# facebookresearch/NasRec

Measured on AMD Instinct MI355X. Metric: supernet samples/sec at batch 256 (Criteo-shape), 1/2/4/8 MI355X, higher is better.
Workload: dtype f32

## Files before the change

include/nasrec_hip.h:

```cpp
#ifndef NASREC_HIP_H
#define NASREC_HIP_H

#include <stdint.h>

#ifdef __cplusplus
extern "C" {
#endif

#define NASREC_MAX_SEGS 8
#define NASREC_MAX_TABLES 32
#define NASREC_EMB_DIM 16
#define NASREC_MHA_PARAMS 1696
#define NASREC_MHA_SAVED 36

enum {
  NASREC_AM_KC = 0,
  NASREC_AM_RC = 1,
  NASREC_AM_TOKR = 2,
  NASREC_AM_TOKK = 3
};
enum { NASREC_CM_PLAIN = 0,
       NASREC_CM_TOKJ = 1    };
enum { NASREC_ACT_NONE = 0, NASREC_ACT_RELU = 1, NASREC_ACT_SILU = 2, NASREC_ACT_SIGMOID = 3 };

enum {
  NASREC_OP_GEMM = 1,
  NASREC_OP_EMBED_GATHER = 2,
  NASREC_OP_DOT_TRI_FWD = 3,
  NASREC_OP_DOT_TRI_BWD = 4,
  NASREC_OP_FM_FWD = 5,
  NASREC_OP_FM_BWD = 6,
  NASREC_OP_MHA_FWD = 7,
  NASREC_OP_MHA_BWD = 8,
  NASREC_OP_REDUCE_ROWS = 9,
  NASREC_OP_COPY_SEGS = 10,
  NASREC_OP_GATE_BWD = 11,
  NASREC_OP_ROWSUM = 12,
  NASREC_OP_FINAL_FWD = 13,
  NASREC_OP_BCE = 14,
  NASREC_OP_FINAL_BWD = 15,
  NASREC_OP_EMB_DEDUP = 16,
  NASREC_OP_SUMSQ = 17,
  NASREC_OP_CLIP_COEF = 18,
  NASREC_OP_ADAGRAD_DENSE = 19,
  NASREC_OP_ADAGRAD_ROWS = 20,
  NASREC_OP_MEMSET = 21,
  NASREC_OP_LAYERNORM_FWD = 22,
  NASREC_OP_LAYERNORM_BWD = 23,
  NASREC_OP_ADD_SEGS = 24,
  NASREC_OP_SCALE = 25,
  NASREC_OP_ACT_BWD = 26,
  NASREC_OP_STAGE_INPUTS = 27,
  NASREC_OP_OPT_REDUCE = 28,
  NASREC_OP_OPT_APPLY = 29,
  NASREC_OP_WORKLIST = 30,
  NASREC_OP_CONST_I64 = 31,
  NASREC_OP_SPLITK_EPILOGUES = 32,
  NASREC_OP_DEDUP_IDS = 33,
  NASREC_OP_OPT_REDUCE2 = 34,
  NASREC_OP_FINAL_FUSED = 35,
  NASREC_OP_PERSIST = 36,
  NASREC_OP_WORKLIST_DEV = 38,
  NASREC_OP_WEIGHT_DECAY = 39,
  NASREC_OP_OPT_MOMENTS = 40,
  NASREC_OP_LAST_LAYER_STEP = 41,
  NASREC_OP_ROC_AUC = 42
};

enum { NASREC_OPTIM_ADAGRAD = 0, NASREC_OPTIM_ADAM = 1, NASREC_OPTIM_SGD = 2 };

typedef struct nasrec_gemm_seg {
  const float* A;
  const float* B;
  float* C;
  const float* Aaux;
  const float* Baux;
  float* rowsum;
  int32_t M, N, K;
  int32_t lda, ldb, ldc;
  int32_t Mvalid;
  int32_t accumulate;
  int32_t ones_col;
  int32_t _pad;
} nasrec_gemm_seg_t;

typedef struct nasrec_gemm_desc {
  int32_t kind;
  int32_t amode, bmode, cmode;
  int32_t nseg;
  int32_t zmode;
  int32_t act;
  int32_t bias_on_rows;
  int32_t mask_on_rows;
  int32_t dims_in_use;
  int32_t beta;
  int32_t splitk;
  const float* bias;
  float* save_z;
  float* save_act;
  const float* mul_ptr[NASREC_MAX_SEGS];
  int32_t mul_off[NASREC_MAX_SEGS], mul_width[NASREC_MAX_SEGS], mul_ld[NASREC_MAX_SEGS];
  int32_t mul_nseg;
  int32_t defer_second_pass;
  float* workspace;
  int32_t* counters;
  float* rowsum_out;
  const float* pre_add;
  nasrec_gemm_seg_t seg[NASREC_MAX_SEGS];
} nasrec_gemm_desc_t;

typedef struct nasrec_embed_desc {
  int32_t kind;
  int32_t B, Fs;
  int32_t _pad;
  const int64_t* idx;
  const float* table[NASREC_MAX_TABLES];
  int64_t rows[NASREC_MAX_TABLES];
  float* out;
  int32_t* oob;
} nasrec_embed_desc_t;

typedef struct nasrec_emb_dedup_desc {
  int32_t kind;
  int32_t B, Fs;
  int32_t _pad;
  const int64_t* idx;
  const float* dout;
  int32_t* leader;
  float* gsum;
  float* sumsq_partial;
  int32_t* overflow;
  int32_t rank_B;
  int32_t _pad2;
  int64_t rank_stride;
} nasrec_emb_dedup_desc_t;

typedef struct nasrec_dot_tri_desc {
  int32_t kind;
  int32_t B, k1;
  int32_t ld_out;
  const float* T;
  float* out;
  const float* dout;
  float* dT;
} nasrec_dot_tri_desc_t;

typedef struct nasrec_fm_desc {
  int32_t kind;
  int32_t B, N;
  int32_t ldx;
  int32_t ld_ix;
  int32_t accumulate;
  const float* x;
  float* ix;
  const float* dix;
  float* dx;
  const float* add;
} nasrec_fm_desc_t;

typedef struct nasrec_mha_desc {
  int32_t kind;
  int32_t B, N;
  int32_t ldx, ldo;
  int32_t dims_in_use;
  const float* x;
  float* out;
  const float* dout;
  float* dx;
  float* dparams_partial;
  const float* params[12];
  float* saved;
  int32_t partial_ld;
  int32_t bwd_form;
} nasrec_mha_desc_t;

#define NASREC_REDUCE_MAX_DST 48
typedef struct nasrec_reduce_rows_desc {
  int32_t kind;
  int32_t R, C, ld;
  const float* in;
  int32_t ndst;
  int32_t _pad;
  float* dst[NASREC_REDUCE_MAX_DST];
  int32_t dst_off[NASREC_REDUCE_MAX_DST];
  int32_t dst_len[NASREC_REDUCE_MAX_DST];
} nasrec_reduce_rows_desc_t;

typedef struct nasrec_copy_segs_desc {
  int32_t kind;
  int32_t B, nseg;
  int32_t ld_dst;
  int32_t accumulate;
  int32_t reverse;
  float* dst;
  float* seg[NASREC_MAX_SEGS];
  int32_t width[NASREC_MAX_SEGS], ld[NASREC_MAX_SEGS], off[NASREC_MAX_SEGS];
  int32_t seg_accumulate[NASREC_MAX_SEGS];
} nasrec_copy_segs_desc_t;


typedef struct nasrec_gate_bwd_desc {
  int32_t kind;
  int32_t B, D;
  int32_t ld_dout, ld_g, ld_dz;
  const float* dout;
  const float* g;
  float* dz;
  int32_t nseg;
  const float* r_ptr[NASREC_MAX_SEGS];
  float* dr_ptr[NASREC_MAX_SEGS];
  int32_t r_off[NASREC_MAX_SEGS], r_width[NASREC_MAX_SEGS], r_ld[NASREC_MAX_SEGS];
  int32_t dr_accumulate[NASREC_MAX_SEGS];
} nasrec_gate_bwd_desc_t;

typedef struct nasrec_rowsum_desc {
  int32_t kind;
  int32_t mode, R, K, ld;
  int32_t rvalid;
  const float* p;
  const float* aux;
  float* out;
} nasrec_rowsum_desc_t;

typedef struct nasrec_final_desc {
  int32_t kind;
  int32_t B, nseg;
  float grad_scale;
  const float* w;
  const float* bias;
  float* logits;
  const float* dlogits;
  float* dw;
  float* dbias;
  const float* seg[NASREC_MAX_SEGS];
  float* dseg[NASREC_MAX_SEGS];
  int32_t width[NASREC_MAX_SEGS], ld[NASREC_MAX_SEGS], off[NASREC_MAX_SEGS];
  int32_t dseg_accumulate[NASREC_MAX_SEGS];
  const float* y;
  float* loss;
  float* dlogits_out;
  int32_t nsplit;
  int32_t dseg_done;
  int32_t tok_stride[NASREC_MAX_SEGS];
} nasrec_final_desc_t;

typedef struct nasrec_bce_desc {
  int32_t kind;
  int32_t B;
  float grad_scale;
  int32_t _pad;
  const float* logits;
  const float* y;
  float* loss;
  float* dlogits;
} nasrec_bce_desc_t;

#define NASREC_SPLITK_BALANCED (-1)
#define NASREC_SK_WORKSPACE_FLOATS (512L * 3 * 128 * 128)
#define NASREC_CHUNK_ELEMS 65536
#define NASREC_CONST_I64_MAX 448

typedef struct nasrec_sumsq_desc {
  int32_t kind;
  int32_t nblocks;
  int64_t n;
  const float* x;
  float* partial;
  const int64_t* chunks;
  int64_t nchunks;
} nasrec_sumsq_desc_t;

typedef struct nasrec_clip_coef_desc {
  int32_t kind;
  int32_t n_a, n_b;
  float max_norm;
  const float* partial_a;
  const float* partial_b;
  float* out;
} nasrec_clip_coef_desc_t;

typedef struct nasrec_adagrad_dense_desc {
  int32_t kind;
  float eps;
  int64_t n;
  float* p;
  const float* g;
  float* state;
  const float* lr;
  const float* coef;
  const int64_t* chunks;
  int64_t nchunks;
} nasrec_adagrad_dense_desc_t;

typedef struct nasrec_adagrad_rows_desc {
  int32_t kind;
  int32_t B, Fs;
  float eps;
  const int64_t* idx;
  const int32_t* leader;
  const float* gsum;
  float* table[NASREC_MAX_TABLES];
  float* state[NASREC_MAX_TABLES];
  const float* lr;
  const float* coef;
  int64_t rows[NASREC_MAX_TABLES];
  int32_t rank_B;
  int32_t _pad;
  int64_t rank_stride;
} nasrec_adagrad_rows_desc_t;

typedef struct nasrec_opt_reduce_desc {
  int32_t kind;
  int32_t _pad;
  nasrec_emb_dedup_desc_t dedup;
  nasrec_sumsq_desc_t sumsq;
} nasrec_opt_reduce_desc_t;

typedef struct nasrec_opt_apply_desc {
  int32_t kind;
  int32_t dense_blocks;
  nasrec_clip_coef_desc_t clip;
  nasrec_adagrad_dense_desc_t dense;
  nasrec_adagrad_rows_desc_t rows;
} nasrec_opt_apply_desc_t;

typedef struct nasrec_weight_decay_desc {
// ... 335 lines not shown
```

nasrec_amd/_lib.py:

```python
import ctypes as C
import os

import torch

_HERE = os.path.dirname(os.path.abspath(__file__))
LIB_PATH = os.environ.get("NASREC_HIP_LIB") or os.path.join(_HERE, "lib", "libnasrec_hip.so")

MAX_SEGS = 8
MAX_TABLES = 32
EMB_DIM = 16
MHA_PARAMS = 1696
MHA_SAVED = 36
REDUCE_MAX_DST = 48

AM_KC, AM_RC, AM_TOKR, AM_TOKK = 0, 1, 2, 3
CM_PLAIN, CM_TOKJ = 0, 1
ACT_NONE, ACT_RELU, ACT_SILU, ACT_SIGMOID = 0, 1, 2, 3
TSV_OK, TSV_NEEDS_PYTHON, TSV_BAD_COLUMNS = 0, 1, 2
ACT_BY_NAME = {"identity": ACT_NONE, "relu": ACT_RELU, "silu": ACT_SILU}

(OP_GEMM, OP_EMBED_GATHER, OP_DOT_TRI_FWD, OP_DOT_TRI_BWD, OP_FM_FWD, OP_FM_BWD, OP_MHA_FWD, OP_MHA_BWD, OP_REDUCE_ROWS,
 OP_COPY_SEGS, OP_GATE_BWD, OP_ROWSUM, OP_FINAL_FWD, OP_BCE, OP_FINAL_BWD, OP_EMB_DEDUP, OP_SUMSQ, OP_CLIP_COEF,
 OP_ADAGRAD_DENSE, OP_ADAGRAD_ROWS, OP_MEMSET, OP_LAYERNORM_FWD, OP_LAYERNORM_BWD, OP_ADD_SEGS, OP_SCALE,
 OP_ACT_BWD, OP_STAGE_INPUTS, OP_OPT_REDUCE, OP_OPT_APPLY, OP_WORKLIST, OP_CONST_I64, OP_SPLITK_EPILOGUES, OP_DEDUP_IDS,
 OP_OPT_REDUCE2, OP_FINAL_FUSED, OP_PERSIST) = range(1, 37)
OP_WORKLIST_DEV = 38
OP_WEIGHT_DECAY = 39
OP_OPT_MOMENTS = 40
OP_LAST_LAYER_STEP = 41
OPTIM_ADAGRAD, OPTIM_ADAM, OPTIM_SGD = 0, 1, 2
LAST_LAYER_MAX = 8192
OP_ROC_AUC = 42
ROC_AUC_MAX_N = 1 << 30
ROC_AUC_TOO_FEW, ROC_AUC_BAD_LABEL, ROC_AUC_NOT_FINITE, ROC_AUC_ONE_CLASS = 1, 2, 4, 8

i32, i64, f32, vp = C.c_int32, C.c_int64, C.c_float, C.c_void_p


class GemmSeg(C.Structure):
    _fields_ = [("A", vp), ("B", vp), ("C", vp), ("Aaux", vp), ("Baux", vp), ("rowsum", vp), ("M", i32), ("N", i32), ("K", i32),
                ("lda", i32), ("ldb", i32), ("ldc", i32), ("Mvalid", i32), ("accumulate", i32), ("ones_col", i32), ("_pad", i32)]


class GemmDesc(C.Structure):
    _fields_ = [("kind", i32), ("amode", i32), ("bmode", i32), ("cmode", i32), ("nseg", i32), ("zmode", i32), ("act", i32),
                ("bias_on_rows", i32), ("mask_on_rows", i32), ("dims_in_use", i32), ("beta", i32), ("splitk", i32),
                ("bias", vp), ("save_z", vp), ("save_act", vp), ("mul_ptr", vp * MAX_SEGS), ("mul_off", i32 * MAX_SEGS),
                ("mul_width", i32 * MAX_SEGS), ("mul_ld", i32 * MAX_SEGS), ("mul_nseg", i32), ("defer_second_pass", i32),
                ("workspace", vp), ("counters", vp), ("rowsum_out", vp), ("pre_add", vp), ("seg", GemmSeg * MAX_SEGS)]


EPILOGUES_MAX = 3


class SplitkEpiloguesDesc(C.Structure):
    _fields_ = [("kind", i32), ("n", i32), ("g", GemmDesc * EPILOGUES_MAX)]


class EmbedDesc(C.Structure):
    _fields_ = [("kind", i32), ("B", i32), ("Fs", i32), ("_pad", i32), ("idx", vp), ("table", vp * MAX_TABLES),
                ("rows", i64 * MAX_TABLES), ("out", vp), ("oob", vp)]


class EmbDedupDesc(C.Structure):
    _fields_ = [("kind", i32), ("B", i32), ("Fs", i32), ("_pad", i32), ("idx", vp), ("dout", vp), ("leader", vp), ("gsum", vp),
                ("sumsq_partial", vp), ("overflow", vp), ("rank_B", i32), ("_pad2", i32), ("rank_stride", i64)]


class DotTriDesc(C.Structure):
    _fields_ = [("kind", i32), ("B", i32), ("k1", i32), ("ld_out", i32), ("T", vp), ("out", vp), ("dout", vp), ("dT", vp)]


class FmDesc(C.Structure):
    _fields_ = [("kind", i32), ("B", i32), ("N", i32), ("ldx", i32), ("ld_ix", i32), ("accumulate", i32), ("x", vp), ("ix", vp),
                ("dix", vp), ("dx", vp), ("add", vp)]


class MhaDesc(C.Structure):
    _fields_ = [("kind", i32), ("B", i32), ("N", i32), ("ldx", i32), ("ldo", i32), ("dims_in_use", i32), ("x", vp), ("out", vp),
                ("dout", vp), ("dx", vp), ("dparams_partial", vp), ("params", vp * 12), ("saved", vp), ("partial_ld", i32), ("bwd_form", i32)]


class ReduceRowsDesc(C.Structure):
    _fields_ = [("kind", i32), ("R", i32), ("C", i32), ("ld", i32), ("in_", vp), ("ndst", i32), ("_pad", i32), ("dst", vp * REDUCE_MAX_DST),
                ("dst_off", i32 * REDUCE_MAX_DST), ("dst_len", i32 * REDUCE_MAX_DST)]


class CopySegsDesc(C.Structure):
    _fields_ = [("kind", i32), ("B", i32), ("nseg", i32), ("ld_dst", i32), ("accumulate", i32), ("reverse", i32), ("dst", vp),
                ("seg", vp * MAX_SEGS), ("width", i32 * MAX_SEGS), ("ld", i32 * MAX_SEGS), ("off", i32 * MAX_SEGS),
                ("seg_accumulate", i32 * MAX_SEGS)]


class GateBwdDesc(C.Structure):
    _fields_ = [("kind", i32), ("B", i32), ("D", i32), ("ld_dout", i32), ("ld_g", i32), ("ld_dz", i32), ("dout", vp), ("g", vp),
                ("dz", vp), ("nseg", i32), ("r_ptr", vp * MAX_SEGS), ("dr_ptr", vp * MAX_SEGS), ("r_off", i32 * MAX_SEGS),
                ("r_width", i32 * MAX_SEGS), ("r_ld", i32 * MAX_SEGS), ("dr_accumulate", i32 * MAX_SEGS)]


class RowsumDesc(C.Structure):
    _fields_ = [("kind", i32), ("mode", i32), ("R", i32), ("K", i32), ("ld", i32), ("rvalid", i32), ("p", vp), ("aux", vp),
                ("out", vp)]


class FinalDesc(C.Structure):
    _fields_ = [("kind", i32), ("B", i32), ("nseg", i32), ("grad_scale", f32), ("w", vp), ("bias", vp), ("logits", vp), ("dlogits", vp),
                ("dw", vp), ("dbias", vp), ("seg", vp * MAX_SEGS), ("dseg", vp * MAX_SEGS), ("width", i32 * MAX_SEGS),
                ("ld", i32 * MAX_SEGS), ("off", i32 * MAX_SEGS), ("dseg_accumulate", i32 * MAX_SEGS), ("y", vp), ("loss", vp),
                ("dlogits_out", vp), ("nsplit", i32), ("dseg_done", i32), ("tok_stride", i32 * MAX_SEGS)]


class BceDesc(C.Structure):
    _fields_ = [("kind", i32), ("B", i32), ("grad_scale", f32), ("_pad", i32), ("logits", vp), ("y", vp), ("loss", vp),
                ("dlogits", vp)]


class SumsqDesc(C.Structure):
    _fields_ = [("kind", i32), ("nblocks", i32), ("n", i64), ("x", vp), ("partial", vp), ("chunks", vp), ("nchunks", i64)]


class ClipCoefDesc(C.Structure):
    _fields_ = [("kind", i32), ("n_a", i32), ("n_b", i32), ("max_norm", f32), ("partial_a", vp), ("partial_b", vp), ("out", vp)]


class AdagradDenseDesc(C.Structure):
    _fields_ = [("kind", i32), ("eps", f32), ("n", i64), ("p", vp), ("g", vp), ("state", vp), ("lr", vp), ("coef", vp),
                ("chunks", vp), ("nchunks", i64)]


class AdagradRowsDesc(C.Structure):
    _fields_ = [("kind", i32), ("B", i32), ("Fs", i32), ("eps", f32), ("idx", vp), ("leader", vp), ("gsum", vp),
                ("table", vp * MAX_TABLES), ("state", vp * MAX_TABLES), ("lr", vp), ("coef", vp), ("rows", i64 * MAX_TABLES),
                ("rank_B", i32), ("_pad", i32), ("rank_stride", i64)]


class MemsetDesc(C.Structure):
    _fields_ = [("kind", i32), ("_pad", i32), ("bytes", i64), ("ptr", vp), ("chunks", vp), ("nchunks", i64)]


SPLITK_BALANCED = -1
SK_WORKSPACE_FLOATS = 512 * 3 * 128 * 128
CHUNK_ELEMS = 65536
CONST_I64_MAX = 448


class ConstI64Desc(C.Structure):
    _fields_ = [("kind", i32), ("n", i32), ("dst", vp), ("vals", i64 * CONST_I64_MAX)]


class LayerNormDesc(C.Structure):
    _fields_ = [("kind", i32), ("mode", i32), ("R", i32), ("D", i32), ("ldx", i32), ("ldy", i32), ("act", i32),
                ("dims_in_use", i32), ("accumulate", i32), ("eps", f32), ("x", vp), ("w", vp), ("b", vp), ("y", vp), ("stats", vp),
                ("dy", vp), ("dx", vp), ("dwb_partial", vp), ("nblk", i32), ("_pad", i32)]


class ScaleDesc(C.Structure):
    _fields_ = [("kind", i32), ("_pad", i32), ("n", i64), ("s", f32), ("_pad2", i32), ("x", vp), ("y", vp)]


class ActBwdDesc(C.Structure):
    _fields_ = [("kind", i32), ("mode", i32), ("R", i32), ("D", i32), ("ld_dy", i32), ("ld_z", i32), ("ld_dz", i32), ("act", i32),
                ("dims_in_use", i32), ("dy", vp), ("z", vp), ("dz", vp)]


DEDUP_IDS_MAX_B = 2048


class DedupIdsDesc(C.Structure):
    _fields_ = [("kind", i32), ("B", i32), ("Fs", i32), ("cap", i32), ("idx", vp), ("leader", vp), ("order", vp), ("lists", vp), ("counts", vp),
                ("heads", vp)]


class OptReduce2Desc(C.Structure):
    _fields_ = [("kind", i32), ("B", i32), ("Fs", i32), ("cap", i32), ("rank_B", i32), ("row_blocks", i32), ("rank_stride", i64), ("rows", vp),
                ("leader", vp), ("order", vp), ("lists", vp), ("counts", vp), ("heads", vp), ("sumsq_partial", vp), ("sumsq", SumsqDesc)]


class StageDesc(C.Structure):
    _fields_ = [("kind", i32), ("B", i32), ("Fd", i32), ("Fs", i32), ("lr", f32), ("_pad", i32), ("int_src", vp), ("int_dst", vp),
                ("cat_src", vp), ("cat_dst", vp), ("y_src", vp), ("y_dst", vp), ("lr_dst", vp), ("gather", EmbedDesc), ("dedup_ids", DedupIdsDesc)]


class OptReduceDesc(C.Structure):
    _fields_ = [("kind", i32), ("_pad", i32), ("dedup", EmbDedupDesc), ("sumsq", SumsqDesc)]


class OptApplyDesc(C.Structure):
    _fields_ = [("kind", i32), ("dense_blocks", i32), ("clip", ClipCoefDesc), ("dense", AdagradDenseDesc), ("rows", AdagradRowsDesc)]


WL_MAX_ITEMS, WL_BLOB_BYTES, WL_REDUCE_DST = 12, 3680, 16
WL_WHOLE, WL_MAIN, WL_EPI = 0, 1, 2
# ... 146 lines not shown
```

nasrec_amd/csrc/common.h:

```cpp
#pragma once
#include <hip/hip_runtime.h>
#include <stdint.h>
#include "nasrec_hip.h"

#define NASREC_WAVE 64

typedef float f32x4 __attribute__((ext_vector_type(4)));

template <int MODE>
__device__ __forceinline__ long operand_offset(int r, int k, int ld) {
  if (MODE == NASREC_AM_KC) return (long)r * ld + k;
  if (MODE == NASREC_AM_RC) return (long)k * ld + r;
  if (MODE == NASREC_AM_TOKR) return (long)(r >> 4) * ld + (r & 15) + (long)k * 16;
  return (long)(k >> 4) * ld + (k & 15) + (long)r * 16;
}

template <int CMODE>
__device__ __forceinline__ long c_offset(int i, int j, int ldc) {
  if (CMODE == NASREC_CM_PLAIN) return (long)i * ldc + j;
  return (long)(j >> 4) * ldc + (j & 15) + (long)i * 16;
}

__device__ __forceinline__ float act_apply(float z, int act) {
  switch (act) {
    case NASREC_ACT_RELU: return z > 0.f ? z : 0.f;
    case NASREC_ACT_SILU: return z / (1.f + __expf(-z));
    case NASREC_ACT_SIGMOID: return 1.f / (1.f + __expf(-z));
    default: return z;
  }
}

template <int BYTES>
__device__ __forceinline__ void warm_kernarg() {
  static_assert(BYTES % 64 == 0 && BYTES >= 64 && BYTES <= 4096, "whole 64-byte lines");
  if (threadIdx.x >= 64) return;
  const unsigned long long p = (unsigned long long)__builtin_amdgcn_kernarg_segment_ptr();
  int sink;
  if (BYTES <= 1024) {
    asm volatile(
        ".set nasrec_wk_off, 0\n"
        ".rept %c2\n"
        "s_load_dword %0, %1, nasrec_wk_off\n"
        ".set nasrec_wk_off, nasrec_wk_off + 64\n"
        ".endr\n"
        "s_waitcnt lgkmcnt(0)"
        : "=&s"(sink)
        : "s"(p), "n"(BYTES / 64)
        : "memory");
  } else {
    asm volatile(
        ".set nasrec_wk_off, 0\n"
        ".rept %c2\n"
        ".rept 16\n"
        "s_load_dword %0, %1, nasrec_wk_off\n"
        ".set nasrec_wk_off, nasrec_wk_off + 64\n"
        ".endr\n"
        "s_waitcnt lgkmcnt(0)\n"
        ".endr"
        : "=&s"(sink)
        : "s"(p), "n"(BYTES / 1024)
        : "memory");
  }
}

template <int CTRL>
__device__ __forceinline__ float dpp_mov(float v) {
  return __builtin_bit_cast(float, __builtin_amdgcn_mov_dpp(__builtin_bit_cast(int, v), CTRL, 0xf, 0xf, false));
}
__device__ __forceinline__ float wave_sum(float v) {
  v += dpp_mov<0xb1>(v);
  v += dpp_mov<0x4e>(v);
  v += dpp_mov<0x124>(v);
  v += dpp_mov<0x128>(v);
  v += dpp_mov<0x142>(v);
  v += dpp_mov<0x143>(v);
  return __builtin_bit_cast(float, __builtin_amdgcn_readlane(__builtin_bit_cast(int, v), 63));
}

int nasrec_set_error(int code, const char* fmt, ...);
int nasrec_check_launch(const char* what);

static inline bool nasrec_lds_attr_needed(unsigned long long& mask) {
  int dev = 0;
  (void)hipGetDevice(&dev);
  const unsigned long long bit = 1ull << (dev & 63);
  if (mask & bit) return false;
  mask |= bit;
  return true;
}

int launch_gemm(hipStream_t s, const nasrec_gemm_desc_t* d);
int launch_embed_gather(hipStream_t s, const nasrec_embed_desc_t* d);
int launch_emb_dedup(hipStream_t s, const nasrec_emb_dedup_desc_t* d);
int launch_dot_tri(hipStream_t s, const nasrec_dot_tri_desc_t* d);
int launch_fm(hipStream_t s, const nasrec_fm_desc_t* d);
int launch_mha(hipStream_t s, const nasrec_mha_desc_t* d);
int launch_reduce_rows(hipStream_t s, const nasrec_reduce_rows_desc_t* d);
int launch_copy_segs(hipStream_t s, const nasrec_copy_segs_desc_t* d);
int launch_gate_bwd(hipStream_t s, const nasrec_gate_bwd_desc_t* d);
int launch_rowsum(hipStream_t s, const nasrec_rowsum_desc_t* d);
int launch_final(hipStream_t s, const nasrec_final_desc_t* d);
int final_fused_check(const nasrec_final_desc_t* d);
int launch_bce(hipStream_t s, const nasrec_bce_desc_t* d);
int launch_sumsq(hipStream_t s, const nasrec_sumsq_desc_t* d);
int launch_clip_coef(hipStream_t s, const nasrec_clip_coef_desc_t* d);
int launch_adagrad_dense(hipStream_t s, const nasrec_adagrad_dense_desc_t* d);
int launch_adagrad_rows(hipStream_t s, const nasrec_adagrad_rows_desc_t* d);
int launch_layernorm(hipStream_t s, const nasrec_layernorm_desc_t* d);
int launch_scale(hipStream_t s, const nasrec_scale_desc_t* d);
int launch_act_bwd(hipStream_t s, const nasrec_act_bwd_desc_t* d);
int launch_stage(hipStream_t s, const nasrec_stage_desc_t* d);
int launch_opt_reduce(hipStream_t s, const nasrec_opt_reduce_desc_t* d);
int launch_opt_apply(hipStream_t s, const nasrec_opt_apply_desc_t* d);
int launch_memset_chunks(hipStream_t s, const nasrec_memset_desc_t* d);
int launch_memset_flat(hipStream_t s, const nasrec_memset_desc_t* d);
int launch_const_i64(hipStream_t s, const nasrec_const_i64_desc_t* d);
int launch_splitk_epilogues(hipStream_t s, const nasrec_splitk_epilogues_desc_t* d);
int launch_worklist(hipStream_t s, const nasrec_worklist_desc_t* d);
int launch_worklist_dev(hipStream_t s, const nasrec_worklist_dev_desc_t* d);
int launch_dedup_ids(hipStream_t s, const nasrec_dedup_ids_desc_t* d);
int launch_opt_reduce2(hipStream_t s, const nasrec_opt_reduce2_desc_t* d);
int launch_persist(hipStream_t s, const nasrec_persist_desc_t* d);
int launch_weight_decay(hipStream_t s, const nasrec_weight_decay_desc_t* d);
int launch_opt_moments(hipStream_t s, const nasrec_opt_moments_desc_t* d);
int launch_last_layer_step(hipStream_t s, const nasrec_last_layer_step_desc_t* d);
int launch_roc_auc(hipStream_t s, const nasrec_roc_auc_desc_t* d);
```

nasrec_amd/csrc/final_bodies.h:

```cpp
#pragma once
#include "common.h"

__device__ __forceinline__ int final_wcol(const nasrec_final_desc_t& d, int q, int j) {
  const int ts = d.tok_stride[q];
  return d.off[q] + (ts ? (j >> 4) * ts + (j & 15) : j);
}
__device__ __forceinline__ int final_feat(const nasrec_final_desc_t& d, int q, int k) {
  const int r = k - d.off[q], ts = d.tok_stride[q];
  if (r < 0) return -1;
  if (!ts) return r < d.width[q] ? r : -1;
  const int t = r / ts, e = r - t * ts;
  const int j = t * 16 + e;
  return (e < 16 && j < d.width[q]) ? j : -1;
}
__host__ __device__ inline int final_seg_extent(const nasrec_final_desc_t& d, int q) {
  const int ts = d.tok_stride[q], W = d.width[q];
  return (ts && W > 0) ? ((W - 1) >> 4) * ts + ((W - 1) & 15) + 1 : W;
}

__device__ __forceinline__ float final_logit(const nasrec_final_desc_t& d, int b, float* red) {
  const int wave = threadIdx.x >> 6, lane = threadIdx.x & 63;
  float s = 0.f;
  for (int q = 0; q < d.nseg; ++q) {
    if (!d.seg[q]) continue;
    const float* x = d.seg[q] + (long)b * d.ld[q];
    const float* w = d.w + d.off[q];
    const int W = d.width[q], ts = d.tok_stride[q];
    for (int j0 = lane + 64 * wave; j0 < W; j0 += 256 * 4) {
      float xv[4], wv[4];
#pragma unroll
      for (int u = 0; u < 4; ++u) {
        const int j = min(j0 + 256 * u, W - 1);
        xv[u] = x[j];
        wv[u] = w[ts ? (j >> 4) * ts + (j & 15) : j];
      }
#pragma unroll
      for (int u = 0; u < 4; ++u)
        if (j0 + 256 * u < W) s = fmaf(xv[u], wv[u], s);
    }
  }
  s = wave_sum(s);
  __syncthreads();
  if (lane == 0) red[wave] = s;
  __syncthreads();
  return ((red[0] + red[1]) + (red[2] + red[3])) + d.bias[0];
}

__device__ __forceinline__ void final_fwd_block(const nasrec_final_desc_t& d, int vb, float* red) {
  if (vb >= d.B) return;
  const float z = final_logit(d, vb, red);
  if (threadIdx.x == 0) d.logits[vb] = z;
}

__device__ __forceinline__ float bce_grad(float z, float y, float scale) { return (1.f / (1.f + expf(-z)) - y) * scale; }
__device__ __forceinline__ float bce_term(float z, float y) { return fmaxf(z, 0.f) - z * y + log1pf(expf(-fabsf(z))); }

__device__ __forceinline__ void final_fused_block(const nasrec_final_desc_t& d, int vb, float* red) {
  const int b = vb;
  if (b >= d.B) return;
  const float yb = d.y[b];
  const float z = final_logit(d, b, red);
  if (threadIdx.x == 0) d.logits[b] = z;
  const float g = bce_grad(z, yb, d.grad_scale);
  const int tid = threadIdx.x;
  for (int q = 0; q < d.nseg; ++q) {
    float* p = d.dseg[q];
    if (!p || !d.seg[q]) continue;
    p += (long)b * d.ld[q];
    const float* w = d.w + d.off[q];
    const int W = d.width[q], ts = d.tok_stride[q];
    const bool acc = d.dseg_accumulate[q] != 0;
    for (int j0 = tid; j0 < W; j0 += 256 * 4) {
      float wv[4], cv[4];
#pragma unroll
      for (int u = 0; u < 4; ++u) {
        const int j = min(j0 + 256 * u, W - 1);
        wv[u] = w[ts ? (j >> 4) * ts + (j & 15) : j];
        cv[u] = acc ? p[j] : 0.f;
      }
#pragma unroll
      for (int u = 0; u < 4; ++u) {
        const float v = g * wv[u];
        if (j0 + 256 * u < W) p[j0 + 256 * u] = acc ? cv[u] + v : v;
      }
    }
  }
}

#define FINAL_BWD_LDS_FLOATS 272
#define FINAL_BWD_ROWS 16
__host__ __device__ inline int final_bwd_rows(int B) { return B >= 1024 ? FINAL_BWD_ROWS : 1; }
__device__ __forceinline__ void final_bwd_block(const nasrec_final_desc_t& d, int K, int nA, int nB, int vb_, float* lds) {
  const int nC = d.y != nullptr ? 1 : 0;
  const int vb = vb_ < nB + nC ? nA + vb_ : vb_ - (nB + nC);
  const bool fused = d.y != nullptr;
  const float* const dl_a = fused ? d.logits : d.dlogits;
  const float* const dl_b = fused ? d.y : d.dlogits;
  const float dl_scale = d.grad_scale;
  auto dl = [&](int b) {
    const float z = dl_a[b], y = dl_b[b];
    return fused ? bce_grad(z, y, dl_scale) : z;
  };
  if (vb < nA && final_bwd_rows(d.B) > 1) {
    constexpr int RB = FINAL_BWD_ROWS;
    const int kblocks = (K + 255) / 256;
    const int rblk = vb / kblocks, k = (vb - rblk * kblocks) * 256 + (int)threadIdx.x;
    if (k >= K) return;
    float* p0 = nullptr;
    long ldq = 0;
    bool accq = false;
    for (int q = 0; q < d.nseg; ++q) {
      const int jj = final_feat(d, q, k);
      if (jj >= 0) {
        if (d.dseg[q]) {
          p0 = d.dseg[q] + jj;
          ldq = d.ld[q];
          accq = d.dseg_accumulate[q] != 0;
        }
        break;
      }
    }
    if (!p0) return;
    const float wk = d.w[k];
    const int r0 = rblk * RB;
    float z[RB], y[RB], c[RB], g[RB];
#pragma unroll
    for (int u = 0; u < RB; ++u) {
      const int b = min(r0 + u, d.B - 1);
      z[u] = dl_a[b];
      y[u] = dl_b[b];
      c[u] = 0.f;
    }
    if (accq) {
#pragma unroll
      for (int u = 0; u < RB; ++u) c[u] = p0[(long)min(r0 + u, d.B - 1) * ldq];
    }
    if (fused) {
#pragma unroll
      for (int u = 0; u < RB; ++u) g[u] = bce_grad(z[u], y[u], dl_scale);
    } else {
#pragma unroll
      for (int u = 0; u < RB; ++u) g[u] = z[u];
    }
    __builtin_amdgcn_s_waitcnt(0x0F70);
#pragma unroll
    for (int u = 0; u < RB; ++u) {
      if (r0 + u >= d.B) break;
      const float v = g[u] * wk;
      p0[(long)(r0 + u) * ldq] = accq ? c[u] + v : v;
    }
    return;
  }
  if (vb < nA) {
    const long t = (long)vb * 256 + threadIdx.x;
    if (t >= (long)d.B * K) return;
    const int b = (int)(t / K), k = (int)(t % K);
    for (int q = 0; q < d.nseg; ++q) {
      const int jj = final_feat(d, q, k);
      if (jj >= 0) {
        if (d.dseg[q]) {
          float* p = d.dseg[q] + (long)b * d.ld[q] + jj;
          const float v = dl(b) * d.w[k];
          *p = d.dseg_accumulate[q] ? *p + v : v;
        }
        break;
      }
    }
    return;
  }
  if (vb >= nA + nB) {
    float* redl = lds;
    float s = 0.f;
    for (int b = threadIdx.x; b < d.B; b += 256) {
      const float z = d.logits[b], y = d.y[b];
      s += bce_term(z, y);
      if (d.dlogits_out) d.dlogits_out[b] = bce_grad(z, y, d.grad_scale);
    }
    redl[threadIdx.x] = s;
    __syncthreads();
    for (int o = 128; o > 0; o >>= 1) {
      if ((int)threadIdx.x < o) redl[threadIdx.x] += redl[threadIdx.x + o];
      __syncthreads();
    }
    if (threadIdx.x == 0 && d.loss) d.loss[0] = redl[0] / (float)d.B;
    return;
  }
  if (d.nsplit > 1) {
    float(*reds)[64] = reinterpret_cast<float(*)[64]>(lds);
    const int nBk = nB / d.nsplit;
    const int blk = vb - nA, slice = blk / nBk, kl = threadIdx.x & 63, w = threadIdx.x >> 6;
    const int k = (blk - slice * nBk) * 64 + kl;
    const int b0 = (int)((long)d.B * slice / d.nsplit), b1 = (int)((long)d.B * (slice + 1) / d.nsplit);
    float s0 = 0.f, s1 = 0.f;
    if (k <= K) {
      const float* src = nullptr;
      int ld = 0, jj = 0;
      if (k < K) {
        for (int q = 0; q < d.nseg; ++q) {
          jj = final_feat(d, q, k);
          if (jj >= 0) {
            src = d.seg[q];
            ld = d.ld[q];
            break;
          }
        }
      }
      const bool has = k < K && src != nullptr;
      const float* sp = has ? src + jj : d.w;
      const long sld = has ? ld : 0;
      int b = b0 + w;
      for (; b + 28 < b1; b += 32) {
        float f[8], z[8], y[8], g[8];
#pragma unroll
        for (int u = 0; u < 8; ++u) {
          f[u] = sp[(long)(b + 4 * u) * sld];
          z[u] = dl_a[b + 4 * u];
          y[u] = dl_b[b + 4 * u];
        }
        if (fused) {
#pragma unroll
          for (int u = 0; u < 8; ++u) g[u] = bce_grad(z[u], y[u], dl_scale);
        } else {
#pragma unroll
          for (int u = 0; u < 8; ++u) g[u] = z[u];
        }
#pragma unroll
        for (int u = 0; u < 8; u += 2) {
          s0 = fmaf(g[u], (k == K) ? 1.f : (has ? f[u] : 0.f), s0);
          s1 = fmaf(g[u + 1], (k == K) ? 1.f : (has ? f[u + 1] : 0.f), s1);
        }
      }
      for (; b + 4 < b1; b += 8) {
        const float f0 = (k == K) ? 1.f : (src ? src[(long)b * ld + jj] : 0.f);
        const float f1 = (k == K) ? 1.f : (src ? src[(long)(b + 4) * ld + jj] : 0.f);
        s0 = fmaf(dl(b), f0, s0);
        s1 = fmaf(dl(b + 4), f1, s1);
      }
      for (; b < b1; b += 4) s0 = fmaf(dl(b), (k == K) ? 1.f : (src ? src[(long)b * ld + jj] : 0.f), s0);
    }
    reds[w][kl] = s0 + s1;
    __syncthreads();
    if (w == 0 && k <= K) d.dw[(long)slice * (K + 1) + k] = (reds[0][kl] + reds[1][kl]) + (reds[2][kl] + reds[3][kl]);
    return;
  }
  float(*red)[17] = reinterpret_cast<float(*)[17]>(lds);
  const int kl = threadIdx.x & 15, bq = threadIdx.x >> 4;
// ... 65 lines not shown
```

nasrec_amd/csrc/gemm_fast.hip:

```cpp
#include <stdlib.h>
#include "gemm_tile.h"

typedef float f32x16 __attribute__((ext_vector_type(16)));
typedef int i32x4 __attribute__((ext_vector_type(4)));

#define FT_BM 128
#define FT_BN 128
#define FT_BK 32
#define FT_KC_LD 36
#define FT_TILE_FLOATS (FT_BM * FT_KC_LD)
#define FT_FENCE() __builtin_amdgcn_sched_barrier(0)

template <int MODE>
__device__ __forceinline__ void ft_slot(int tid, int it, int& row, int& k) {
  const int idx = tid + 256 * it;
  if (MODE == NASREC_AM_KC) {
    row = idx >> 3;
    k = (idx & 7) << 2;
  } else {
    k = idx >> 5;
    row = (idx & 31) << 2;
  }
}

// ... 544 lines not shown
  const int fr = lane & 31, fg = lane >> 5;
  const int t = blockIdx.x;
  const long W = (long)sk_tiles * sk_T, lo = (long)t * sk_T, hi = lo + sk_T;
  int w = (int)(lo * FT_SK_WGS / W);
  while (w > 0 && ft_share_begin(W, w) > lo) --w;
  while (ft_share_begin(W, w + 1) <= lo) ++w;
  if (ft_share_begin(W, w) <= lo && ft_share_begin(W, w + 1) >= hi) return;
  int z, ks, by, bx;
  if (!ft_decode(d, t, 1, tiles_m, tiles_n, z, ks, by, bx)) return;
  const nasrec_gemm_seg_t& s0 = d.seg[z];
  const int m0 = by * FT_BM, n0 = bx * FT_BN;
  if (m0 >= s0.M || n0 >= s0.N) return;
  f32x16 acc[2][2];
#pragma unroll
  for (int a = 0; a < 2; ++a)
#pragma unroll
    for (int b = 0; b < 2; ++b)
#pragma unroll
      for (int r = 0; r < 16; ++r) acc[a][b][r] = 0.f;
  for (; w < FT_SK_WGS && ft_share_begin(W, w) < hi; ++w) {
    const int piece = t - (int)(ft_share_begin(W, w) / sk_T);
    const float* slot = d.workspace + ((long)w * FT_SK_PIECES + piece) * FT_PIECE_FLOATS;
#pragma unroll
    for (int a = 0; a < 2; ++a)
#pragma unroll
      for (int b = 0; b < 2; ++b)
#pragma unroll
        for (int r = 0; r < 16; ++r) acc[a][b][r] += slot[((a * 2 + b) * 16 + r) * 256 + tid];
  }
  ft_epilogue(d, s0, m0, n0, wm, wn, fr, fg, acc, false);
}

template <int AM, int BMODE>
static int launch_fast_t(hipStream_t st, const nasrec_gemm_desc_t* d, int Mmax, int Nmax, int zdim, bool ones) {
  const int tm = (Mmax + FT_BM - 1) / FT_BM, tn = (Nmax + FT_BN - 1) / FT_BN;
  long blocks = (long)tm * tn * zdim;
  if (d->zmode) {
    const int S = d->splitk > 1 ? d->splitk : 1;
    blocks = 0;
    for (int q = 0; q < d->nseg; ++q)
      blocks += (long)((d->seg[q].M + FT_BM - 1) / FT_BM) * ((d->seg[q].N + FT_BN - 1) / FT_BN) * S;
  }
  int sk_tiles = 0, sk_T = 0;
  if (d->splitk == NASREC_SPLITK_BALANCED) {
    int T = 0;
    if (d->zmode) {
      for (int q = 0; q < d->nseg; ++q) {
        const int tq = d->seg[q].A ? (d->seg[q].K + FT_BK - 1) / FT_BK : 0;
        if (q > 0 && tq != T) return nasrec_set_error(-2, "gemm: balanced schedule needs equal K over the batch (problem %d)", q);
        T = tq;
      }
    } else {
      for (int q = 0; q < d->nseg; ++q)
        if (d->seg[q].A) T += (d->seg[q].K + FT_BK - 1) / FT_BK;
    }
    if (T < 1) return nasrec_set_error(-2, "gemm: balanced schedule on an empty product");
    if (!d->workspace) return nasrec_set_error(-3, "gemm: balanced schedule needs a workspace of NASREC_SK_WORKSPACE_FLOATS floats");
    const long tiles = blocks;
    if (tiles % FT_SK_WGS != 0) {
      sk_tiles = (int)(tiles >= FT_SK_WGS ? FT_SK_WGS + tiles % FT_SK_WGS : tiles);
      sk_T = T;
      blocks = FT_SK_WGS + (tiles - sk_tiles);
    }
  }
  const dim3 grid((unsigned)blocks);
  if (ones)
    hipLaunchKernelGGL((gemm_fast_kernel<AM, BMODE, true>), grid, dim3(256), 0, st, *d, Mmax, Nmax, tm, tn, sk_tiles, sk_T);
  else
    hipLaunchKernelGGL((gemm_fast_kernel<AM, BMODE, false>), grid, dim3(256), 0, st, *d, Mmax, Nmax, tm, tn, sk_tiles, sk_T);
  if (sk_tiles > 0) hipLaunchKernelGGL(gemm_fast_fixup_kernel, dim3((unsigned)sk_tiles), dim3(256), 0, st, *d, tm, tn, sk_tiles, sk_T);
  return 0;
}

bool gemm_fast_eligible(const nasrec_gemm_desc_t* d, int Mmax, int Nmax) {
  if (d->cmode != NASREC_CM_PLAIN) return false;
  if (d->bias && d->bias_on_rows) return false;
  if ((d->amode != NASREC_AM_KC && d->amode != NASREC_AM_RC) || (d->bmode != NASREC_AM_KC && d->bmode != NASREC_AM_RC)) return false;
  if (d->amode == NASREC_AM_RC && d->bmode == NASREC_AM_KC) return false;
  const int nprob = d->zmode ? d->nseg : 1;
  const int S = d->splitk > 1 ? d->splitk : 1;
  long tiles = 0, kmax = 0;
  for (int q = 0; q < d->nseg; ++q) {
    const nasrec_gemm_seg_t& s = d->seg[q];
    if (s.Aaux || s.Baux) return false;
    if (s.A && s.K > kmax) kmax = s.K;
    const long r = s.M > s.N ? s.M : s.N, ld = s.lda > s.ldb ? s.lda : s.ldb;
    if (s.A && (r * ld + s.K >= (1L << 29) || (long)s.K * ld + r >= (1L << 29))) return false;
  }
  long useful = 0, padded = 0;
  for (int q = 0; q < nprob; ++q) {
    const nasrec_gemm_seg_t& s = d->seg[q];
    const long t = (long)((s.M + FT_BM - 1) / FT_BM) * ((s.N + FT_BN - 1) / FT_BN);
    tiles += t * S;
    useful += (long)s.M * s.N;
    padded += t * FT_BM * FT_BN;
  }
  (void)Mmax;
  (void)Nmax;
  if (2 * useful < padded) return false;
  static const long min_k = getenv("NASREC_FAST_MIN_K") ? atol(getenv("NASREC_FAST_MIN_K")) : 1;
  return tiles >= NASREC_GEMM_FAST_MIN_TILES && kmax >= min_k;
}

int launch_gemm_fast(hipStream_t st, const nasrec_gemm_desc_t* d, int Mmax, int Nmax, int zdim) {
  bool ones = false;
  for (int q = 0; q < d->nseg; ++q) ones = ones || d->seg[q].ones_col != 0;
  if (d->amode == NASREC_AM_KC && d->bmode == NASREC_AM_KC) return launch_fast_t<NASREC_AM_KC, NASREC_AM_KC>(st, d, Mmax, Nmax, zdim, ones);
  if (d->amode == NASREC_AM_KC && d->bmode == NASREC_AM_RC) return launch_fast_t<NASREC_AM_KC, NASREC_AM_RC>(st, d, Mmax, Nmax, zdim, ones);
  return launch_fast_t<NASREC_AM_RC, NASREC_AM_RC>(st, d, Mmax, Nmax, zdim, ones);
}
```

nasrec_amd/csrc/gemm_kslice.hip:

```cpp
#include <cstdlib>
#include <cstring>
#include "gemm_tile.h"

#define KS_TM 32
#define KS_TN 32
#define KS_DC 128
#define KS_NB 4
#define KS_CH ((KS_TM + KS_TN) * KS_DC)
#define KS_SEGS 4
#ifdef KS_STAMPS
#define KS_STAMP(i) \
  if (tid == 0 && d.workspace) d.workspace[blockIdx.x * 64 + (i)] = __builtin_bit_cast(float, (unsigned)__builtin_readcyclecounter())
#define KS_LOOP_STAMP_A const unsigned ks_ta = (unsigned)__builtin_readcyclecounter()
#define KS_LOOP_STAMP_B ks_wait += (unsigned)__builtin_readcyclecounter() - ks_ta
#else
#define KS_STAMP(i)
#define KS_LOOP_STAMP_A
#define KS_LOOP_STAMP_B
#endif

__device__ __forceinline__ __amdgpu_buffer_rsrc_t ks_rsrc(const float* p, long floats) {
  return __builtin_amdgcn_make_buffer_rsrc(const_cast<float*>(p), 0, (int)(floats <= 0 ? 0 : (floats > 0x1fffffffL ? 0x7fffffffL : 4 * floats)), 0x00020000);
}

// ... 221 lines not shown
      if (ck >= cK) {
        do {
          ++cseg;
        } while (cseg < KS_SEGS && seg_k(cseg) == 0);
        ck = 0;
        cK = seg_k(cseg);
      }
    };
    auto multiply = [&](int set) {
      const int lim = flim[set];
      if (lim < KS_DC) {
#pragma unroll
        for (int kb = 0; kb < 4; ++kb)
#pragma unroll
          for (int e = 0; e < 4; ++e) {
            const bool in = 4 * (16 * half + 4 * kb + fg) + e < lim;
            fa[set][kb][e] = in ? fa[set][kb][e] : 0.f;
            fb[set][kb][e] = in ? fb[set][kb][e] : 0.f;
          }
      }
#pragma unroll
      for (int kb = 0; kb < 4; kb += 2)
#pragma unroll
        for (int j = 0; j < 4; ++j) {
          acc0 = __builtin_amdgcn_mfma_f32_16x16x4f32(fa[set][kb][j], fb[set][kb][j], acc0, 0, 0, 0);
          acc1 = __builtin_amdgcn_mfma_f32_16x16x4f32(fa[set][kb + 1][j], fb[set][kb + 1][j], acc1, 0, 0, 0);
        }
    };
    for (int t = 0; t < nchunks + 1; t += 2) {
#pragma unroll
      for (int h = 0; h < 2; ++h) {
        const int c = t + h;
        if (c < nchunks) {
          asm volatile("s_waitcnt lgkmcnt(0)" ::: "memory");
          KS_LOOP_STAMP_A;
          __builtin_amdgcn_s_barrier();
          KS_LOOP_STAMP_B;
          readfrag(h);
        }
        if (c >= 1 && c <= nchunks) multiply(h ^ 1);
      }
    }
    KS_STAMP(4);
    asm volatile("s_waitcnt lgkmcnt(0)" ::: "memory");
    __builtin_amdgcn_s_barrier();
    if (tK > 0) {
#pragma unroll
      for (int e = 0; e < 4; ++e) {
        const bool in = 4 * fg + e < tK;
        ta[e] = in ? ta[e] : 0.f;
        tb[e] = in ? tb[e] : 0.f;
      }
#pragma unroll
      for (int j = 0; j < 4; ++j) acc0 = __builtin_amdgcn_mfma_f32_16x16x4f32(ta[j], tb[j], acc0, 0, 0, 0);
    }
    const f32x4 acc = acc0 + acc1;
#ifdef KS_STAMPS
    if (lane == 0 && d.workspace) {
      d.workspace[blockIdx.x * 64 + 16 + wave * 3 + 1] = __builtin_bit_cast(float, ks_wait);
      d.workspace[blockIdx.x * 64 + 16 + wave * 3 + 2] = __builtin_bit_cast(float, (unsigned)__builtin_readcyclecounter() - ks_t0);
    }
#endif
    *reinterpret_cast<f32x4*>(&red[((half * 4 + tile) * 64 + lane) * 4]) = acc;
  }
  __syncthreads();
  KS_STAMP(5);
  {
    const int e = wave;
    const int etile = e >> 2, r = e & 3;
    const float v = red[((0 * 4 + etile) * 64 + lane) * 4 + r] + red[((1 * 4 + etile) * 64 + lane) * 4 + r];
    const int i = m0 + (etile >> 1) * 16 + 4 * fg + r, j = n0 + (etile & 1) * 16 + fr;
    if (i < M && j < N) epilogue_store<NASREC_CM_PLAIN>(d, s0, i, j, v);
  }
  KS_STAMP(6);
}

bool gemm_kslice_eligible(const nasrec_gemm_desc_t* d) {
  if (d->amode != NASREC_AM_KC || d->bmode != NASREC_AM_KC || d->cmode != NASREC_CM_PLAIN || d->zmode || d->splitk > 1) return false;
  if (d->nseg > KS_SEGS) return false;
  const nasrec_gemm_seg_t& s0 = d->seg[0];
  long K = 0;
  for (int q = 0; q < d->nseg; ++q) {
    const nasrec_gemm_seg_t& s = d->seg[q];
    if (s.Aaux || s.Baux || s.ones_col || (s.Mvalid > 0 && s.Mvalid < s0.M)) return false;
    if (s.A && s.K > 0) {
      K += s.K;
      if ((long)s0.M * s.lda >= (1L << 29) || (long)s0.N * s.ldb >= (1L << 29)) return false;
    }
  }
  const long tiles = (long)((s0.M + KS_TM - 1) / KS_TM) * ((s0.N + KS_TN - 1) / KS_TN);
  return s0.M <= 512 && tiles >= 128 && tiles <= 512 && K >= 512;
}

int launch_gemm_kslice(hipStream_t st, const nasrec_gemm_desc_t* d) {
  const nasrec_gemm_seg_t& s0 = d->seg[0];
  const int tiles_m = (s0.M + KS_TM - 1) / KS_TM, tiles_n = (s0.N + KS_TN - 1) / KS_TN;
  static unsigned long long attr_devices = 0;
  const size_t lds = sizeof(float) * KS_NB * KS_CH;
  if (nasrec_lds_attr_needed(attr_devices))
    (void)hipFuncSetAttribute(reinterpret_cast<const void*>(&gemm_kslice_kernel), hipFuncAttributeMaxDynamicSharedMemorySize, (int)lds);
  hipLaunchKernelGGL(gemm_kslice_kernel, dim3((unsigned)(tiles_m * tiles_n)), dim3(1024), lds, st, *d, tiles_m, tiles_n);
  return nasrec_check_launch("gemm_kslice");
}
```

nasrec_amd/csrc/gemm_skinny.hip:

```cpp
#include <stdlib.h>

#include "gemm_tile.h"

#define SKN_STEPS 8

template <int NW, bool BRC>
__global__ __launch_bounds__(64 * NW) void gemm_skinny_n_kernel(const nasrec_gemm_desc_t d) {
  __shared__ float red[NW][256];
  const int lane = threadIdx.x & 63, wave = __builtin_amdgcn_readfirstlane(threadIdx.x >> 6);
  const int r = lane & 15, g = lane >> 4;
  const nasrec_gemm_seg_t& s0 = d.seg[0];
  const int M = s0.M, N = s0.N;
  const int m0 = (int)blockIdx.x * 16;
  const int row = min(m0 + r, M - 1), col = min(r, N - 1);
  const int nsegk = d.zmode ? 1 : d.nseg;
  int T = 0;
  for (int q = 0; q < nsegk; ++q) T += (d.seg[q].A && d.seg[q].K > 0) ? (d.seg[q].K + 15) >> 4 : 0;
  const int t0 = (int)((long)T * wave / NW), t1 = (int)((long)T * (wave + 1) / NW);
  int fq = 0, fk = 0;
  {
    int skip = t0;
    for (; fq < nsegk; ++fq) {
      const int nt = (d.seg[fq].A && d.seg[fq].K > 0) ? (d.seg[fq].K + 15) >> 4 : 0;
      if (skip < nt) break;
      skip -= nt;
    }
    fk = 16 * skip;
  }
  f32x4 acc = {0.f, 0.f, 0.f, 0.f};
  for (int t = t0; t < t1; t += SKN_STEPS) {
    f32x4 fa[SKN_STEPS], fb[SKN_STEPS];
    int lim[SKN_STEPS];
#pragma unroll
    for (int s = 0; s < SKN_STEPS; ++s) {
      const bool in = t + s < t1 && fq < nsegk;
      const nasrec_gemm_seg_t& sg = d.seg[in ? fq : 0];
      const bool live = in && sg.A != nullptr && sg.K > 0;
      const int K = live ? sg.K : 0, kk = fk + 4 * g;
      lim[s] = K - fk;
      const __amdgpu_buffer_rsrc_t ra = __builtin_amdgcn_make_buffer_rsrc(
          const_cast<float*>(sg.A), 0, live ? (int)min(4L * ((long)(M - 1) * sg.lda + K), 0x7fffffffL) : 0, 0x00020000);
      const __amdgpu_buffer_rsrc_t rb = __builtin_amdgcn_make_buffer_rsrc(
          const_cast<float*>(sg.B), 0, live ? (int)(4 * (BRC ? (long)(K - 1) * sg.ldb + N : (long)(N - 1) * sg.ldb + K)) : 0, 0x00020000);
      fa[s] = __builtin_bit_cast(f32x4, __builtin_amdgcn_raw_buffer_load_b128(ra, (int)(4 * ((long)row * sg.lda + kk)), 0, 0));
      if (BRC) {
#pragma unroll
        for (int j = 0; j < 4; ++j)
          fb[s][j] = __builtin_bit_cast(float, __builtin_amdgcn_raw_buffer_load_b32(rb, 4 * ((kk + j) * sg.ldb + col), 0, 0));
      } else {
        fb[s] = __builtin_bit_cast(f32x4, __builtin_amdgcn_raw_buffer_load_b128(rb, 4 * (col * sg.ldb + kk), 0, 0));
      }
      fk += 16;
      bool next = in && fk >= K;
      if (next) {
        ++fq;
        while (fq < nsegk && !(d.seg[fq].A && d.seg[fq].K > 0)) ++fq;
        fk = 0;
      }
    }
#pragma unroll
    for (int s = 0; s < SKN_STEPS; ++s) {
      const int l = lim[s];
      if (l > 0) {
        f32x4 a = fa[s], b = fb[s];
        if (l < 16) {
#pragma unroll
          for (int j = 0; j < 4; ++j) {
            const bool ok = 4 * g + j < l;
            a[j] = ok ? a[j] : 0.f;
            b[j] = ok ? b[j] : 0.f;
          }
        }
#pragma unroll
        for (int j = 0; j < 4; ++j) acc = __builtin_amdgcn_mfma_f32_16x16x4f32(a[j], b[j], acc, 0, 0, 0);
      }
    }
  }
#pragma unroll
  for (int q = 0; q < 4; ++q) red[wave][q * 64 + lane] = acc[q];
  __syncthreads();
  if (wave == 0) {
    float v4[4];
#pragma unroll
    for (int q = 0; q < 4; ++q) {
      float p[NW];
#pragma unroll
      for (int w = 0; w < NW; ++w) p[w] = red[w][q * 64 + lane];
#pragma unroll
      for (int span = 1; span < NW; span *= 2)
#pragma unroll
        for (int w = 0; w + span < NW; w += 2 * span) p[w] += p[w + span];
      v4[q] = p[0];
    }
    if (m0 + 4 * g < M && r < N) epilogue_store_col4<NASREC_CM_PLAIN>(d, s0, m0 + 4 * g, r, M, v4);
  }
}

bool gemm_skinny_n_eligible(const nasrec_gemm_desc_t* d) {
  if (d->amode != NASREC_AM_KC || (d->bmode != NASREC_AM_KC && d->bmode != NASREC_AM_RC) || d->cmode != NASREC_CM_PLAIN || d->splitk > 1) return false;
  if (d->zmode && d->nseg != 1) return false;
  const nasrec_gemm_seg_t& s0 = d->seg[0];
  if (s0.N < 1 || s0.N > 16 || s0.M < 1024) return false;
  long K = 0;
  for (int q = 0; q < d->nseg; ++q) {
    const nasrec_gemm_seg_t& s = d->seg[q];
    if (s.Aaux || s.Baux || s.ones_col || (s.Mvalid > 0 && s.Mvalid < s0.M)) return false;
    if (s.A && s.K > 0) {
      K += s.K;
      if ((long)s0.M * s.lda >= (1L << 29) || (long)(d->bmode == NASREC_AM_RC ? s.K : s0.N) * s.ldb >= (1L << 29)) return false;
    }
  }
  return K >= 256;
}

int launch_gemm_skinny_n(hipStream_t st, const nasrec_gemm_desc_t* d) {
  const int M = d->seg[0].M;
  const int tiles = (M + 15) / 16;
  const bool brc = d->bmode == NASREC_AM_RC;
  if (tiles >= 512) {
    if (brc) hipLaunchKernelGGL((gemm_skinny_n_kernel<4, true>), dim3((unsigned)tiles), dim3(256), 0, st, *d);
    else hipLaunchKernelGGL((gemm_skinny_n_kernel<4, false>), dim3((unsigned)tiles), dim3(256), 0, st, *d);
  } else {
    if (brc) hipLaunchKernelGGL((gemm_skinny_n_kernel<8, true>), dim3((unsigned)tiles), dim3(512), 0, st, *d);
    else hipLaunchKernelGGL((gemm_skinny_n_kernel<8, false>), dim3((unsigned)tiles), dim3(512), 0, st, *d);
  }
  return nasrec_check_launch("gemm_skinny_n");
}

#define TK_MAXK 16
#define TK_GROUPS 2
#define TK_ROWS (8 * TK_GROUPS)
template <bool BRC>
__global__ __launch_bounds__(256) void gemm_tinyk_kernel(const nasrec_gemm_desc_t d) {
  const int q = d.zmode ? (int)blockIdx.z : 0;
  const nasrec_gemm_seg_t& sg = d.seg[q];
  const int M = sg.M, N = sg.N, K = sg.K;
  const int j = (int)blockIdx.x * 256 + (int)threadIdx.x;
  const int i0 = (int)blockIdx.y * TK_ROWS;
  if (i0 >= M) return;
  const int jc = min(j, N - 1);
  float w[TK_MAXK];
  if (sg.A != nullptr && K > 0) {
#pragma unroll
    for (int k = 0; k < TK_MAXK; ++k) w[k] = k < K ? (BRC ? sg.B[(long)k * sg.ldb + jc] : sg.B[(long)jc * sg.ldb + k]) : 0.f;
  } else {
#pragma unroll
    for (int k = 0; k < TK_MAXK; ++k) w[k] = 0.f;
  }
  const bool simple = !d.pre_add && d.mul_nseg == 0 && !(d.zmode ? sg.accumulate : d.beta) && d.dims_in_use < 0 && !(d.bias && d.bias_on_rows);
  const float bj = (simple && d.bias) ? d.bias[jc] : 0.f;
  float* const zp = d.save_z;
  float* const ap = d.save_act;
  const int act = d.act;
  const int lane = (int)threadIdx.x & 63;
  float xa[TK_GROUPS], xb[TK_GROUPS];
#pragma unroll
  for (int gr = 0; gr < TK_GROUPS; ++gr) {
    xa[gr] = xb[gr] = 0.f;
    if (sg.A != nullptr && K > 0) {
      const int ri = min(i0 + 8 * gr + (lane >> 3), M - 1), kc = 2 * (lane & 7);
      const float* xr = sg.A + (long)ri * sg.lda;
      if (kc < K) xa[gr] = xr[kc];
      if (kc + 1 < K) xb[gr] = xr[kc + 1];
    }
  }
#pragma unroll
  for (int gr = 0; gr < TK_GROUPS; ++gr) {
    const int ib = i0 + 8 * gr;
    if (ib >= M) break;
    const float x0 = xa[gr], x1 = xb[gr];
    float acc[8];
#pragma unroll
    for (int r = 0; r < 8; ++r) {
      float s = 0.f;
#pragma unroll
      for (int k = 0; k < TK_MAXK; ++k) {
        const float xv = __builtin_bit_cast(float, __builtin_amdgcn_readlane(__builtin_bit_cast(int, (k & 1) ? x1 : x0), r * 8 + (k >> 1)));
        s = fmaf(xv, w[k], s);
      }
      acc[r] = s;
    }
    if (j < N) {
      if (simple) {
#pragma unroll
        for (int r = 0; r < 8; ++r) {
          if (ib + r < M) {
            const long o = (long)(ib + r) * sg.ldc + j;
            float v = acc[r] + bj;
            if (zp) zp[o] = v;
            v = act_apply(v, act);
            if (ap) ap[o] = v;
            sg.C[o] = v;
          }
        }
      } else {
        const float va[4] = {acc[0], acc[1], acc[2], acc[3]}, vb[4] = {acc[4], acc[5], acc[6], acc[7]};
        epilogue_store_col4<NASREC_CM_PLAIN>(d, sg, ib, j, M, va);
        if (ib + 4 < M) epilogue_store_col4<NASREC_CM_PLAIN>(d, sg, ib + 4, j, M, vb);
      }
    }
  }
}

bool gemm_tinyk_eligible(const nasrec_gemm_desc_t* d) {
  static const bool on = getenv("NASREC_TINYK") == nullptr || atoi(getenv("NASREC_TINYK")) != 0;
  if (!on || d->amode != NASREC_AM_KC || (d->bmode != NASREC_AM_KC && d->bmode != NASREC_AM_RC) || d->cmode != NASREC_CM_PLAIN || d->splitk > 1) return false;
  static const bool rc_too = getenv("NASREC_TINYK") != nullptr && atoi(getenv("NASREC_TINYK")) == 2;
  if (d->bmode == NASREC_AM_RC && !rc_too) return false;
  if (!d->zmode && d->nseg != 1) return false;
  for (int q = 0; q < d->nseg; ++q) {
    const nasrec_gemm_seg_t& s = d->seg[q];
    if (s.Aaux || s.Baux || s.ones_col || (s.Mvalid > 0 && s.Mvalid < s.M)) return false;
    if (s.M < 1024 || s.N < 256 || s.K < 0 || s.K > TK_MAXK) return false;
  }
  return true;
}

int launch_gemm_tinyk(hipStream_t st, const nasrec_gemm_desc_t* d) {
  int Mmax = 0, Nmax = 0;
  const int nprob = d->zmode ? d->nseg : 1;
  for (int q = 0; q < nprob; ++q) {
    Mmax = max(Mmax, d->seg[q].M);
    Nmax = max(Nmax, d->seg[q].N);
  }
  const dim3 grid((unsigned)((Nmax + 255) / 256), (unsigned)((Mmax + TK_ROWS - 1) / TK_ROWS), (unsigned)nprob);
  if (d->bmode == NASREC_AM_RC) hipLaunchKernelGGL((gemm_tinyk_kernel<true>), grid, dim3(256), 0, st, *d);
  else hipLaunchKernelGGL((gemm_tinyk_kernel<false>), grid, dim3(256), 0, st, *d);
  return nasrec_check_launch("gemm_tinyk");
}
```

nasrec_amd/csrc/norm_loss_opt.hip:

```cpp
#include "common.h"
#include "optimizer_bodies.h"

#include "final_bodies.h"

__global__ __launch_bounds__(256) void final_fwd_kernel(const nasrec_final_desc_t d) {
  __shared__ float red[4];
  final_fwd_block(d, blockIdx.x, red);
}

__global__ __launch_bounds__(256) void final_bwd_kernel(const nasrec_final_desc_t d, int K, int nA, int nB) {
  __shared__ float lds[FINAL_BWD_LDS_FLOATS];
  final_bwd_block(d, K, nA, nB, blockIdx.x, lds);
}

__global__ __launch_bounds__(256) void final_fused_kernel(const nasrec_final_desc_t d) {
  __shared__ float red[4];
  final_fused_block(d, blockIdx.x, red);
}

int final_fused_check(const nasrec_final_desc_t* d) {
  if (!d->y || !d->logits || !d->bias || !d->w) return nasrec_set_error(-2, "final_fused: needs y, logits, bias and w");
  if (d->nsplit > 1) return nasrec_set_error(-2, "final_fused: nsplit=%d (the batch-sliced backward keeps its own launch)", d->nsplit);
  for (int q = 0; q < d->nseg; ++q)
    if (d->dseg[q] && !d->seg[q]) return nasrec_set_error(-2, "final_fused: segment %d has a gradient destination and no input", q);
  return 0;
}

int launch_final(hipStream_t st, const nasrec_final_desc_t* d) {
  if (d->B == 0) return 0;
  if (d->kind == NASREC_OP_FINAL_FUSED) {
    const int rc = final_fused_check(d);
    if (rc) return rc;
    hipLaunchKernelGGL(final_fused_kernel, dim3(d->B), dim3(256), 0, st, *d);
  } else if (d->kind == NASREC_OP_FINAL_FWD) {
    hipLaunchKernelGGL(final_fwd_kernel, dim3(d->B), dim3(256), 0, st, *d);
  } else {
    int K, nA, nB;
    final_bwd_geometry(*d, K, nA, nB);
    if (d->y != nullptr && d->logits == nullptr) return nasrec_set_error(-2, "final_bwd: fused BCE needs desc.logits");
    hipLaunchKernelGGL(final_bwd_kernel, dim3(nA + nB + (d->y != nullptr ? 1 : 0)), dim3(256), 0, st, *d, K, nA, nB);
  }
  return nasrec_check_launch("final");
}

__global__ __launch_bounds__(1024) void bce_kernel(const nasrec_bce_desc_t d) {
  __shared__ float red[1024];
  float s = 0.f;
  for (int b = threadIdx.x; b < d.B; b += 1024) {
    const float z = d.logits[b], y = d.y[b];
    s += bce_term(z, y);
    d.dlogits[b] = bce_grad(z, y, d.grad_scale);
  }
  red[threadIdx.x] = s;
  __syncthreads();
  for (int o = 512; o > 0; o >>= 1) {
    if ((int)threadIdx.x < o) red[threadIdx.x] += red[threadIdx.x + o];
    __syncthreads();
  }
  if (threadIdx.x == 0) d.loss[0] = red[0] / (float)d.B;
}

int launch_bce(hipStream_t st, const nasrec_bce_desc_t* d) {
  if (d->B == 0) return 0;
  hipLaunchKernelGGL(bce_kernel, dim3(1), dim3(1024), 0, st, *d);
  return nasrec_check_launch("bce");
}

__global__ __launch_bounds__(256) void sumsq_kernel(const nasrec_sumsq_desc_t d) {
  __shared__ float red[256];
  sumsq_body(d, blockIdx.x, gridDim.x, red);
}

int launch_sumsq(hipStream_t st, const nasrec_sumsq_desc_t* d) {
  if (d->nblocks < 1) return nasrec_set_error(-2, "sumsq: nblocks=%d", d->nblocks);
  hipLaunchKernelGGL(sumsq_kernel, dim3(d->nblocks), dim3(256), 0, st, *d);
  return nasrec_check_launch("sumsq");
}

__global__ __launch_bounds__(64) void clip_coef_kernel(const nasrec_clip_coef_desc_t d) {
  float total;
  const float coef = clip_coef_wave(d, threadIdx.x, &total);
  if (threadIdx.x == 0) {
    d.out[0] = coef;
    d.out[1] = total;
  }
}

int launch_clip_coef(hipStream_t st, const nasrec_clip_coef_desc_t* d) {
  hipLaunchKernelGGL(clip_coef_kernel, dim3(1), dim3(64), 0, st, *d);
  return nasrec_check_launch("clip_coef");
}

__global__ __launch_bounds__(256) void adagrad_dense_kernel(const nasrec_adagrad_dense_desc_t d) {
  adagrad_dense_body(d, blockIdx.x, gridDim.x, *d.lr, *d.coef);
}

int launch_adagrad_dense(hipStream_t st, const nasrec_adagrad_dense_desc_t* d) {
  if (d->n == 0 || (d->chunks && d->nchunks < 1)) return 0;
  const long blocks = d->chunks ? (d->nchunks > 2048 ? 2048 : d->nchunks) : adagrad_dense_blocks(d->n);
  hipLaunchKernelGGL(adagrad_dense_kernel, dim3((unsigned)blocks), dim3(256), 0, st, *d);
  return nasrec_check_launch("adagrad_dense");
}

__global__ __launch_bounds__(256) void memset_chunks_kernel(const nasrec_memset_desc_t d) {
  for (long c = blockIdx.x; c < d.nchunks; c += gridDim.x) {
    float* x = reinterpret_cast<float*>(d.ptr) + d.chunks[2 * c];
    const long n = d.chunks[2 * c + 1], n4 = n >> 2;
    for (long i = threadIdx.x; i < n4; i += 256) *reinterpret_cast<f32x4*>(x + 4 * i) = (f32x4){0.f, 0.f, 0.f, 0.f};
    for (long j = 4 * n4 + threadIdx.x; j < n; j += 256) x[j] = 0.f;
  }
}

// ... 626 lines not shown
```

nasrec_amd/csrc/token_linear.hip:

```cpp
#include "gemm_tile.h"

#define TL_WAVES 16
#define TL_CHUNK 8
#define TL_MAX_LDS 147456
#define TL_BIAS_FLOATS 80

template <int RB>
struct TlPad {
  static constexpr int v = RB == 1 ? 16 : (RB <= 3 ? 48 : 80);
};

template <int AM, int RB>
__global__ __launch_bounds__(1024) void token_linear_kernel(const nasrec_gemm_desc_t d, int wgs) {
  extern __shared__ __attribute__((aligned(16))) float lds_all[];
  float* const Bl = lds_all;
  float* const Wl = lds_all + TL_BIAS_FLOATS;
  constexpr int MP = TlPad<RB>::v;
  const int tid = threadIdx.x, lane = tid & 63, wave = __builtin_amdgcn_readfirstlane(tid >> 6);
  const int z = d.zmode ? (int)blockIdx.x / wgs : 0;
  const int wg = (int)blockIdx.x - z * wgs;
  const int s_lo = d.zmode ? z : 0, s_hi = d.zmode ? z + 1 : d.nseg;
  const nasrec_gemm_seg_t& s0 = d.seg[s_lo];
  const int M = s0.M, Bs = s0.N >> 4;

// ... 19 lines not shown
    kbase += Kp;
  }
  if (tid < TL_BIAS_FLOATS) Bl[tid] = (d.bias && d.bias_on_rows && tid < M) ? d.bias[tid] : 0.f;
  __syncthreads();

  const int g = lane >> 4, e = lane & 15;
  const bool acc_c = d.zmode ? s0.accumulate != 0 : d.beta != 0;
  const bool has_bias = d.bias != nullptr, bias_rows = d.bias_on_rows != 0, mask_rows = d.mask_on_rows != 0;
  const int dims = d.dims_in_use, act = d.act;
  float* const zbase = d.save_z;
  for (int b = wg * TL_WAVES + wave; b < Bs; b += wgs * TL_WAVES) {
    f32x4 acc[RB];
#pragma unroll
    for (int rb = 0; rb < RB; ++rb) acc[rb] = (f32x4){0.f, 0.f, 0.f, 0.f};
    int kb = 0;
    for (int s = s_lo; s < s_hi; ++s) {
      const nasrec_gemm_seg_t& sg = d.seg[s];
      if (!sg.A || sg.K <= 0) continue;
      const int K4 = (sg.K + 3) >> 2;
      const __amdgpu_buffer_rsrc_t rs =
          __builtin_amdgcn_make_buffer_rsrc(const_cast<float*>(sg.B) + (long)b * sg.ldb, 0, sg.K * 64, 0x00020000);
      for (int c0 = 0; c0 < K4; c0 += TL_CHUNK) {
        float xv[TL_CHUNK];
#pragma unroll
        for (int u = 0; u < TL_CHUNK; ++u)
          xv[u] = __builtin_bit_cast(float, __builtin_amdgcn_raw_buffer_load_b32(rs, (c0 + u) * 256 + lane * 4, 0, 0));
#pragma unroll
        for (int u = 0; u < TL_CHUNK; ++u) {
          if (c0 + u < K4) {
            const float* wrow = Wl + (kb + 4 * (c0 + u) + g) * MP + e;
#pragma unroll
            for (int rb = 0; rb < RB; ++rb) acc[rb] = __builtin_amdgcn_mfma_f32_16x16x4f32(wrow[rb * 16], xv[u], acc[rb], 0, 0, 0);
          }
        }
      }
      kb += 4 * K4;
    }
    float* C = s0.C + (long)b * s0.ldc + e;
    float* Z = zbase ? zbase + (long)b * s0.ldc + e : nullptr;
    float cv[RB][4];
#pragma unroll
    for (int rb = 0; rb < RB; ++rb)
#pragma unroll
      for (int r = 0; r < 4; ++r) cv[rb][r] = 0.f;
    if (acc_c) {
#pragma unroll
      for (int rb = 0; rb < RB; ++rb)
#pragma unroll
        for (int r = 0; r < 4; ++r) cv[rb][r] = C[min(rb * 16 + 4 * g + r, M - 1) * 16];
    }
    const float bcol = (has_bias && !bias_rows) ? d.bias[b * 16 + e] : 0.f;
    __builtin_amdgcn_s_waitcnt(0x0F70);
    const bool dead_col = dims >= 0 && !mask_rows && b * 16 + e >= dims;
#pragma unroll
    for (int rb = 0; rb < RB; ++rb)
#pragma unroll
      for (int r = 0; r < 4; ++r) {
        const int i = rb * 16 + 4 * g + r;
        if (i >= M) continue;
        float v = acc[rb][r];
        if (has_bias) v += bias_rows ? Bl[i] : bcol;
        if (Z) Z[i * 16] = v;
        v = act_apply(v, act);
        if (dead_col || (dims >= 0 && mask_rows && i >= dims)) v = 0.f;
        if (acc_c) v += cv[rb][r];
        C[i * 16] = v;
      }
  }
}

bool token_linear_eligible(const nasrec_gemm_desc_t* d) {
  if (d->cmode != NASREC_CM_TOKJ || d->bmode != NASREC_AM_TOKR) return false;
  if (d->amode != NASREC_AM_KC && d->amode != NASREC_AM_RC) return false;
  if (d->splitk > 1 || d->pre_add || d->save_act || d->mul_nseg > 0) return false;
  const int nprob = d->zmode ? d->nseg : 1;
  for (int p = 0; p < nprob; ++p) {
    const nasrec_gemm_seg_t& s0 = d->seg[p];
    if (s0.M < 1 || s0.M > 80 || (s0.N & 15) || (s0.N >> 4) < 1024 || s0.ones_col) return false;
    if (s0.Mvalid > 0 && s0.Mvalid < s0.M) return false;
    const int mp = s0.M <= 16 ? 16 : (s0.M <= 48 ? 48 : 80);
    long kp = 0;
    for (int q = d->zmode ? p : 0; q < (d->zmode ? p + 1 : d->nseg); ++q) {
      const nasrec_gemm_seg_t& s = d->seg[q];
      if (s.Aaux || s.Baux) return false;
      if (!d->zmode && (s.M != s0.M || s.N != s0.N)) return false;
      if (s.A && s.K > 0) kp += (s.K + 3) & ~3;
      if ((long)s.K * 64 > 0x7fffffffL) return false;
    }
    if (kp * mp * 4 + TL_BIAS_FLOATS * 4 > TL_MAX_LDS) return false;
    if (d->zmode && p > 0 && (s0.N != d->seg[0].N || (s0.M + 15) / 16 != (d->seg[0].M + 15) / 16)) return false;
  }
  return true;
}

template <int AM, int RB>
static void launch_token_linear_rb(hipStream_t st, const nasrec_gemm_desc_t* d, int grid, int wgs, size_t lds) {
  static unsigned long long big_lds_devices = 0;
  if (lds > 65536 && nasrec_lds_attr_needed(big_lds_devices))
    (void)hipFuncSetAttribute(reinterpret_cast<const void*>(&token_linear_kernel<AM, RB>), hipFuncAttributeMaxDynamicSharedMemorySize, TL_MAX_LDS);
  hipLaunchKernelGGL((token_linear_kernel<AM, RB>), dim3(grid), dim3(1024), lds, st, *d, wgs);
}

template <int AM>
static void launch_token_linear_t(hipStream_t st, const nasrec_gemm_desc_t* d, int rb, int grid, int wgs, size_t lds) {
  switch (rb) {
    case 1: launch_token_linear_rb<AM, 1>(st, d, grid, wgs, lds); break;
    case 2: launch_token_linear_rb<AM, 2>(st, d, grid, wgs, lds); break;
    case 3: launch_token_linear_rb<AM, 3>(st, d, grid, wgs, lds); break;
    case 4: launch_token_linear_rb<AM, 4>(st, d, grid, wgs, lds); break;
    default: launch_token_linear_rb<AM, 5>(st, d, grid, wgs, lds); break;
  }
}

int launch_token_linear(hipStream_t st, const nasrec_gemm_desc_t* d) {
  const int nprob = d->zmode ? d->nseg : 1;
  const int Bs = d->seg[0].N >> 4;
  const int rb = (d->seg[0].M + 15) / 16;
  const int mp = rb == 1 ? 16 : (rb <= 3 ? 48 : 80);
  long kp_max = 0;
  for (int p = 0; p < nprob; ++p) {
    long kp = 0;
    for (int q = d->zmode ? p : 0; q < (d->zmode ? p + 1 : d->nseg); ++q)
      if (d->seg[q].A && d->seg[q].K > 0) kp += (d->seg[q].K + 3) & ~3;
    if (kp > kp_max) kp_max = kp;
  }
  int wgs = 256 / nprob;
  if (wgs < 64) wgs = 64;
  const int need = (Bs + TL_WAVES - 1) / TL_WAVES;
  if (wgs > need) wgs = need;
  const size_t lds = (size_t)(kp_max > 0 ? kp_max : 4) * mp * 4 + TL_BIAS_FLOATS * 4;
  if (d->amode == NASREC_AM_KC)
    launch_token_linear_t<NASREC_AM_KC>(st, d, rb, wgs * nprob, wgs, lds);
  else
    launch_token_linear_t<NASREC_AM_RC>(st, d, rb, wgs * nprob, wgs, lds);
  return nasrec_check_launch("token_linear");
}

#define TDW_WAVES 16

template <int RB, int CB>
__global__ __launch_bounds__(64 * TDW_WAVES) void token_dw_kernel(const nasrec_gemm_desc_t d, int Mmax, int Nmax) {
  __shared__ __attribute__((aligned(16))) float red[4 * RB * CB * 4 * 64];
  const int tid = threadIdx.x, lane = tid & 63, wave = __builtin_amdgcn_readfirstlane(tid >> 6);
  const int S = d.splitk;
  const int z = (int)blockIdx.x / S, ks = (int)blockIdx.x - z * S;
  const nasrec_gemm_seg_t& sg = d.seg[z];
  const int M = sg.M, N = sg.N, Nr = sg.ones_col ? N - 1 : N;
  const int Bs = sg.K >> 4;
  const int i16 = lane & 15, g = lane >> 4;
  f32x4 acc[RB][CB];
#pragma unroll
  for (int rb = 0; rb < RB; ++rb)
#pragma unroll
    for (int cb = 0; cb < CB; ++cb) acc[rb][cb] = (f32x4){0.f, 0.f, 0.f, 0.f};
  const int ones_cb = sg.ones_col ? (N - 1) >> 4 : -1, ones_j = (N - 1) & 15;
  if (sg.A) {
    for (int b = ks * TDW_WAVES + wave; b < Bs; b += S * TDW_WAVES) {
      const __amdgpu_buffer_rsrc_t ra = __builtin_amdgcn_make_buffer_rsrc(const_cast<float*>(sg.A) + (long)b * sg.lda, 0, M * 64, 0x00020000);
      const __amdgpu_buffer_rsrc_t rx = __builtin_amdgcn_make_buffer_rsrc(const_cast<float*>(sg.B) + (long)b * sg.ldb, 0, Nr * 64, 0x00020000);
      f32x4 a[RB], x[CB];
#pragma unroll
      for (int rb = 0; rb < RB; ++rb)
        a[rb] = __builtin_bit_cast(f32x4, __builtin_amdgcn_raw_buffer_load_b128(ra, ((rb * 16 + i16) * 16 + 4 * g) * 4, 0, 0));
#pragma unroll
      for (int cb = 0; cb < CB; ++cb) {
        x[cb] = __builtin_bit_cast(f32x4, __builtin_amdgcn_raw_buffer_load_b128(rx, ((cb * 16 + i16) * 16 + 4 * g) * 4, 0, 0));
        if (cb == ones_cb && i16 == ones_j) x[cb] = (f32x4){1.f, 1.f, 1.f, 1.f};
      }
#pragma unroll
      for (int st = 0; st < 4; ++st)
#pragma unroll
        for (int rb = 0; rb < RB; ++rb)
#pragma unroll
          for (int cb = 0; cb < CB; ++cb) acc[rb][cb] = __builtin_amdgcn_mfma_f32_16x16x4f32(a[rb][st], x[cb][st], acc[rb][cb], 0, 0, 0);
    }
  }
  for (int round = 0; round < TDW_WAVES / 4; ++round) {
    if ((wave >> 2) == round) {
      float* mine = red + (wave & 3) * (RB * CB * 256);
#pragma unroll
      for (int rb = 0; rb < RB; ++rb)
#pragma unroll
        for (int cb = 0; cb < CB; ++cb)
#pragma unroll
          for (int r = 0; r < 4; ++r) {
            float* p = &mine[((rb * CB + cb) * 4 + r) * 64 + lane];
            *p = round == 0 ? acc[rb][cb][r] : *p + acc[rb][cb][r];
          }
    }
    __syncthreads();
  }
  const int Mv = (sg.Mvalid > 0 && sg.Mvalid < M) ? sg.Mvalid : M;
  float* slab = d.workspace + ((long)(z * S + ks)) * Mmax * Nmax;
  for (int idx = tid; idx < RB * CB * 256; idx += 64 * TDW_WAVES) {
    const int blk = idx >> 8, r = (idx >> 6) & 3, l = idx & 63;
    const int rb = blk / CB, cb = blk - rb * CB;
    const int i = rb * 16 + 4 * (l >> 4) + r, j = cb * 16 + (l & 15);
    const int o = (blk * 4 + r) * 64 + l;
    const float v = (red[o] + red[RB * CB * 256 + o]) + (red[2 * RB * CB * 256 + o] + red[3 * RB * CB * 256 + o]);
    if (i < M && j < N) slab[(long)i * N + j] = i < Mv ? v : 0.f;
  }
}

bool token_dw_eligible(const nasrec_gemm_desc_t* d) {
  if (d->amode != NASREC_AM_TOKK || d->bmode != NASREC_AM_TOKK || d->cmode != NASREC_CM_PLAIN || !d->zmode) return false;
  if (d->splitk < 2 || !d->workspace) return false;
  for (int q = 0; q < d->nseg; ++q) {
    const nasrec_gemm_seg_t& s = d->seg[q];
    if (s.Aaux || s.Baux) return false;
    if (s.M < 1 || s.M > 80 || s.N < 1 || s.N > 80) return false;
    if ((s.K & 15) || (s.K >> 4) < 1024) return false;
  }
  return true;
}

template <int RB>
static void launch_token_dw_rb(hipStream_t st, const nasrec_gemm_desc_t* d, int cb, int grid, int Mmax, int Nmax) {
  switch (cb) {
    case 1: hipLaunchKernelGGL((token_dw_kernel<RB, 1>), dim3(grid), dim3(64 * TDW_WAVES), 0, st, *d, Mmax, Nmax); break;
    case 2: hipLaunchKernelGGL((token_dw_kernel<RB, 2>), dim3(grid), dim3(64 * TDW_WAVES), 0, st, *d, Mmax, Nmax); break;
    case 3: hipLaunchKernelGGL((token_dw_kernel<RB, 3>), dim3(grid), dim3(64 * TDW_WAVES), 0, st, *d, Mmax, Nmax); break;
    case 4: hipLaunchKernelGGL((token_dw_kernel<RB, 4>), dim3(grid), dim3(64 * TDW_WAVES), 0, st, *d, Mmax, Nmax); break;
    default: hipLaunchKernelGGL((token_dw_kernel<RB, 5>), dim3(grid), dim3(64 * TDW_WAVES), 0, st, *d, Mmax, Nmax); break;
  }
}

int launch_token_dw(hipStream_t st, const nasrec_gemm_desc_t* d, int Mmax, int Nmax) {
  const int rb = (Mmax + 15) / 16, cb = (Nmax + 15) / 16;
  const int grid = d->nseg * d->splitk;
  switch (rb) {
    case 1: launch_token_dw_rb<1>(st, d, cb, grid, Mmax, Nmax); break;
    case 2: launch_token_dw_rb<2>(st, d, cb, grid, Mmax, Nmax); break;
    case 3: launch_token_dw_rb<3>(st, d, cb, grid, Mmax, Nmax); break;
    case 4: launch_token_dw_rb<4>(st, d, cb, grid, Mmax, Nmax); break;
    default: launch_token_dw_rb<5>(st, d, cb, grid, Mmax, Nmax); break;
  }
  return 0;
}
```

nasrec_amd/csrc/worklist.hip:

```cpp
#include <stdlib.h>
#include <string.h>

#include <vector>

#include "worklist_body.h"

static int wl_gemm_geometry(const nasrec_gemm_desc_t* g, nasrec_wl_item_t& it, int blob_left) {
  if (g->nseg < 1 || g->nseg > NASREC_MAX_SEGS) return nasrec_set_error(-2, "worklist: gemm nseg=%d", g->nseg);
  const int need = (int)offsetof(nasrec_gemm_desc_t, seg) + g->nseg * (int)sizeof(nasrec_gemm_seg_t);
  if (need > blob_left) return nasrec_set_error(-2, "worklist: truncated gemm descriptor (%d bytes) runs past the blob", need);
  const int nprob = g->zmode ? g->nseg : 1;
  const int S = g->splitk > 1 ? g->splitk : 1;
  if (g->splitk == NASREC_SPLITK_BALANCED) return nasrec_set_error(-2, "worklist: the balanced schedule is a throughput-regime launch");
  if ((it.part == 0) != (S == 1)) return nasrec_set_error(-2, "worklist: gemm part %d with splitk %d", it.part, g->splitk);
  if (S > 1 && !g->workspace) return nasrec_set_error(-3, "worklist: splitk=%d needs a workspace", S);
  int Mmax = 0, Nmax = 0, Kmax = 0;
  long wgs = 0;
  bool aux = false, uniform = true;
  for (int q = 0; q < nprob; ++q) {
    Mmax = g->seg[q].M > Mmax ? g->seg[q].M : Mmax;
    Nmax = g->seg[q].N > Nmax ? g->seg[q].N : Nmax;
    wgs += (long)((g->seg[q].M + 63) / 64) * ((g->seg[q].N + 63) / 64) * S;
  }
  for (int q = 0; q < g->nseg; ++q) {
// ... 80 lines not shown
      TU += (s.M + 15) / 16;
    }
    if (plain) {
      it.geom[0] = TU;
      it.geom[1] = 0;
      it.geom[2] = WL_TOKS | (2 << 2);
      it.nblk = std::min(((Nmax >> 4) * TU + 3) / 4, WL_TOK_MAX_WG);
      return 0;
    }
  }
  int tile, tbm, tbn;
  if (wgs >= GEMM_SKINNY_BELOW) {
    tile = WL_T32x32, tbm = 32, tbn = 32;
  } else {
    long pad64x16 = 0, pad16x64 = 0;
    for (int q = 0; q < nprob; ++q) {
      pad64x16 += (long)((g->seg[q].M + 63) / 64) * 64 * ((g->seg[q].N + 15) / 16) * 16;
      pad16x64 += (long)((g->seg[q].M + 15) / 16) * 16 * ((g->seg[q].N + 63) / 64) * 64;
    }
    static const bool by_padding = getenv("NASREC_WL_TILE_BY_PADDING") == nullptr || atoi(getenv("NASREC_WL_TILE_BY_PADDING")) != 0;
    const bool wide = by_padding && pad64x16 != pad16x64 ? pad64x16 < pad16x64 : Nmax >= Mmax;
    if (wide) {
      tile = WL_T64x16, tbm = 64, tbn = 16;
    } else {
      tile = WL_T16x64, tbm = 16, tbn = 64;
    }
  }
  it.geom[0] = (Nmax + tbn - 1) / tbn;
  it.geom[1] = (Mmax + tbm - 1) / tbm;
  const bool kca_ = g->amode == NASREC_AM_KC || g->amode == NASREC_AM_TOKK, kcb_ = g->bmode == NASREC_AM_KC || g->bmode == NASREC_AM_TOKK;
  it.geom[2] = tile | ((kca_ && kcb_ ? 0 : (kca_ ? 1 : 2)) << 2) | ((aux ? 1 : 0) << 4);
  it.nblk = it.geom[0] * it.geom[1] * nprob * S;
  return 0;
}

static int wl_item_geometry(nasrec_wl_item_t& it, const char* blob, int left, int k, bool& big) {
    it.nblk = 0;
    it.geom[0] = it.geom[1] = it.geom[2] = 0;
#define WL_NEED(T) if ((int)sizeof(T) > left) return nasrec_set_error(-2, "worklist: item %d runs past the blob", k)
    switch (it.kind) {
      case NASREC_OP_GEMM: {
        const int rc = wl_gemm_geometry(reinterpret_cast<const nasrec_gemm_desc_t*>(blob), it, left);
        if (rc) return rc;
        break;
      }
      case NASREC_OP_MHA_FWD:
      case NASREC_OP_MHA_BWD: {
        WL_NEED(nasrec_mha_desc_t);
        const nasrec_mha_desc_t* d = reinterpret_cast<const nasrec_mha_desc_t*>(blob);
        if (d->N < 1 || d->N > MHA_N) return nasrec_set_error(-2, "worklist: mha N=%d out of range [1,%d]", d->N, MHA_N);
        if (it.kind == NASREC_OP_MHA_BWD) {
          if (!d->saved) return nasrec_set_error(-2, "worklist: mha backward needs the state saved by the forward launch");
          big = true;
        }
        it.nblk = d->B;
        break;
      }
      case NASREC_OP_FM_FWD:
      case NASREC_OP_FM_BWD:
        WL_NEED(nasrec_fm_desc_t);
        it.nblk = (reinterpret_cast<const nasrec_fm_desc_t*>(blob)->B + 3) / 4;
        break;
      case NASREC_OP_DOT_TRI_FWD:
      case NASREC_OP_DOT_TRI_BWD: {
        WL_NEED(nasrec_dot_tri_desc_t);
        const nasrec_dot_tri_desc_t* d = reinterpret_cast<const nasrec_dot_tri_desc_t*>(blob);
        const int P4 = (d->k1 * (d->k1 - 1) / 2 + 3) & ~3;
        if (d->k1 < 2 || 4 * (d->k1 * TRI_LD + P4) > WL_LDS_FLOATS)
          return nasrec_set_error(-2, "worklist: dot_tri k1=%d does not fit the shared LDS buffer", d->k1);
        it.nblk = (d->B + 3) / 4;
        break;
      }
      case NASREC_OP_COPY_SEGS: {
        WL_NEED(nasrec_copy_segs_desc_t);
        const nasrec_copy_segs_desc_t* d = reinterpret_cast<const nasrec_copy_segs_desc_t*>(blob);
        int W = 0;
        for (int q = 0; q < d->nseg; ++q) W = max(W, d->off[q] + d->width[q]);
        it.geom[0] = W;
        it.nblk = (int)(((long)d->B * W + 255) / 256);
        break;
      }
      case NASREC_OP_FINAL_FWD:
        WL_NEED(nasrec_final_desc_t);
        it.nblk = reinterpret_cast<const nasrec_final_desc_t*>(blob)->B;
        break;
      case NASREC_OP_FINAL_FUSED: {
        WL_NEED(nasrec_final_desc_t);
        const int rc = final_fused_check(reinterpret_cast<const nasrec_final_desc_t*>(blob));
        if (rc) return rc;
        it.nblk = reinterpret_cast<const nasrec_final_desc_t*>(blob)->B;
        break;
      }
      case NASREC_OP_FINAL_BWD: {
        WL_NEED(nasrec_final_desc_t);
        const nasrec_final_desc_t* d = reinterpret_cast<const nasrec_final_desc_t*>(blob);
        if (d->y != nullptr && d->logits == nullptr) return nasrec_set_error(-2, "worklist: final_bwd with the fused loss needs desc.logits");
        int K, nA, nB;
        final_bwd_geometry(*d, K, nA, nB);
        it.geom[0] = K, it.geom[1] = nA, it.geom[2] = nB;
        it.nblk = nA + nB + (d->y != nullptr ? 1 : 0);
        break;
      }
      case NASREC_OP_GATE_BWD: {
        WL_NEED(nasrec_gate_bwd_desc_t);
        const nasrec_gate_bwd_desc_t* d = reinterpret_cast<const nasrec_gate_bwd_desc_t*>(blob);
        it.nblk = (int)(((long)d->B * d->D + 255) / 256);
        break;
      }
      case NASREC_OP_DEDUP_IDS: {
        WL_NEED(nasrec_dedup_ids_desc_t);
        const nasrec_dedup_ids_desc_t* d = reinterpret_cast<const nasrec_dedup_ids_desc_t*>(blob);
        if (d->B < 1 || d->B > 256 || d->cap != 256 || d->Fs < 1 || d->Fs > NASREC_MAX_TABLES || !d->idx || !d->leader || !d->order || !d->lists || !d->counts)
          return nasrec_set_error(-2, "worklist: dedup_ids item needs B <= 256, cap 256 and every output (B=%d cap=%d)", d->B, d->cap);
        it.nblk = d->Fs;
        break;
      }
      case NASREC_OP_REDUCE_ROWS: {
        WL_NEED(nasrec_wl_reduce_t);
        const nasrec_wl_reduce_t* d = reinterpret_cast<const nasrec_wl_reduce_t*>(blob);
        if (d->ndst < 1 || d->ndst > NASREC_WL_REDUCE_DST) return nasrec_set_error(-2, "worklist: reduce_rows ndst=%d", d->ndst);
        it.nblk = (d->C + 15) / 16;
        break;
      }
      default:
        return nasrec_set_error(-2, "worklist: item %d has kind %d, which has no body in the worklist kernel", k, it.kind);
    }
#undef WL_NEED
  return 0;
}

static int wl_finalize(nasrec_worklist_desc_t& wl, bool& big, unsigned (&pf)[6], unsigned (&pm)[6]) {
  if (wl.n < 1 || wl.n > NASREC_WL_MAX_ITEMS) return nasrec_set_error(-2, "worklist: n=%d outside [1,%d]", wl.n, NASREC_WL_MAX_ITEMS);
  static const bool force_big = getenv("NASREC_WL_BIG") != nullptr && atoi(getenv("NASREC_WL_BIG")) != 0;
  big = force_big;
  int first = 0;
  for (int k = 0; k < wl.n; ++k) {
    nasrec_wl_item_t& it = wl.item[k];
    if (it.off < 0 || (it.off & 15) || it.off >= NASREC_WL_BLOB_BYTES) return nasrec_set_error(-2, "worklist: item %d offset %d", k, it.off);
    const char* blob = wl.blob + it.off;
    const int left = NASREC_WL_BLOB_BYTES - it.off;
    it.first = first;
    {
      const int rc = wl_item_geometry(it, blob, left, k, big);
      if (rc) return rc;
    }
    first += it.nblk;
  }
  wl.total_blocks = first;
  static_assert(NASREC_WL_MAX_ITEMS == 12 && NASREC_WL_BLOB_BYTES <= 256 * 16 && offsetof(nasrec_worklist_desc_t, blob) % 16 == 0, "packed item table");
  bool packed = first < 0xffff;
  for (int q = 0; q < 6; ++q) {
    unsigned f2[2], m2[2];
    for (int h = 0; h < 2; ++h) {
      const int k = 2 * q + h;
      if (k < wl.n) {
        f2[h] = (unsigned)wl.item[k].first;
        m2[h] = (unsigned)wl.item[k].kind | ((unsigned)wl.item[k].part << 6) | ((unsigned)(wl.item[k].off >> 4) << 8);
        packed = packed && wl.item[k].kind < 64 && wl.item[k].part < 4;
      } else {
        f2[h] = 0xffffu;
        m2[h] = 0;
      }
    }
    pf[q] = f2[0] | (f2[1] << 16);
    pm[q] = m2[0] | (m2[1] << 16);
  }
  if (!packed) pf[0] = WL_PACKED_NONE;
  return 0;
}

int launch_worklist(hipStream_t st, const nasrec_worklist_desc_t* w) {
  nasrec_worklist_desc_t wl = *w;
  bool big;
  unsigned pf[6], pm[6];
  const int rc = wl_finalize(wl, big, pf, pm);
  if (rc) return rc;
  const int first = wl.total_blocks;
  if (first < 1) return 0;
  if (big) {
// ... 287 lines not shown
```

nasrec_amd/engine.py:

```python
import ctypes as C
import json
import os
from typing import Dict, List, Optional

import torch

from . import _lib as L
from . import plan as P
from . import schedule as S

E = 16
DEDUP_SPLIT_MAX_B = min(int(os.environ.get("NASREC_DEDUP_SPLIT_MAX_B", "2048")), L.DEDUP_IDS_MAX_B)
_IDS_AS_ITEM = os.environ.get("NASREC_IDS_AS_ITEM", "1") != "0"
_WL_TUNE = os.environ.get("NASREC_WL_TUNE", "0") == "1"
_WL_TUNE_MARGIN = float(os.environ.get("NASREC_WL_TUNE_MARGIN", "0.004"))
_WL_RESIDENT = os.environ.get("NASREC_WL_RESIDENT", "1") != "0"
_FUSE_FINAL = os.environ.get("NASREC_FUSE_FINAL", "1") != "0"
_FIXED_OPT_TABLE = os.environ.get("NASREC_FIXED_OPT_TABLE", "1") != "0"


def _ptr_array(descs):
    arr = (C.c_void_p * len(descs))()
    for i, d in enumerate(descs):
        arr[i] = C.addressof(getattr(d, "launch_as", d))
# ... 368 lines not shown
            fsegs, K = P.final_segments(d_last, s_last)
            w = ctx.param("_final.weight", (1, K))
            bptr = ctx.param("_final.bias", (1,))
            fd = L.FinalDesc()
            fd.kind = L.OP_FINAL_FWD
            fd.B, fd.nseg = B, len(fsegs)
            fd.w, fd.bias, fd.logits = w, bptr, cp.logits.data_ptr()
            for q, (s, ts) in enumerate(fsegs):
                fd.seg[q], fd.width[q], fd.ld[q], fd.off[q], fd.tok_stride[q] = s.view.ptr, s.width, s.view.ld, s.koff, ts
            ctx.emit(fd)
            if cfg.use_final_sigmoid:
                raise NotImplementedError("use_final_sigmoid is never enabled by the reference CLIs")
            scheduled = self.level_schedule and cfg.fixed and B <= 256
            cp.fwd_levels = cp.bwd_levels = None
            cp.dead_forward = []
            if train:
                if optim is None:
                    self._ensure_table_state()
                self._build_training_tail(cp, ctx, w, bptr, fsegs, B, K, grad_scale)
            fwd_list = list(ctx.fwd)
            if self.dead_code_elimination and cfg.fixed:
                fwd_list, cp.dead_forward = S.eliminate_dead_forward(fwd_list, ctx.bwd if train else [])
            if scheduled:
                fwd_descs, cp.fwd_levels = S.pack(fwd_list)
                self._resident_worklists(cp, fwd_descs)
            else:
                fwd_descs = fwd_list
            cp.fwd = Program(fwd_descs)
            cp.used_params = list(ctx.used_params)
            if train:
                bd, pre = cp.bce, cp._pre
                fi = next(i for i, dsc in enumerate(ctx.bwd) if isinstance(dsc, L.FinalDesc))
                plain = ctx.bwd[fi]
                assert plain.kind == L.OP_FINAL_BWD
                fused = L.FinalDesc.from_buffer_copy(plain)
                fused.logits, fused.y, fused.loss, fused.dlogits_out = cp.logits.data_ptr(), cp.y.data_ptr(), cp.loss.data_ptr(), cp.dlogits.data_ptr()
                fused.grad_scale = bd.grad_scale
                cp.bce = bd
                bwd_descs = pre[1:] + ctx.bwd[:fi] + [fused] + ctx.bwd[fi + 1:]
                odescs = []
                cp.dedup_ids, cp.ids_on_stage = None, False
                if local_optimizer:
                    odescs = self._optimizer_descs(cp, B, cp.cat_x, sbuf.grad_tensor() if (sbuf.grad_written and not self.host_embedding)
                                                   else None, clip, eps)
                ids_in_program = []
                if cp.dedup_ids is not None:
                    if scheduled and _IDS_AS_ITEM:
                        ids_in_program = [cp.dedup_ids]
                    elif B <= 256:
                        cp.stage.dedup_ids = cp.dedup_ids
                        cp.ids_on_stage = True
                    else:
                        odescs = [cp.dedup_ids] + odescs
                cp.fb = None
                if scheduled:
                    jf, jb = self._fuse_final(fwd_list, bwd_descs, fused) if _FUSE_FINAL else (fwd_list, bwd_descs)
                    fb_descs = None
                    cp.persistent = False
                    cp.level_tuning = None
                    if persist:
                        try:
                            fb_descs, cp.fb_levels = S.pack_persistent(
                                ids_in_program + jf + jb, lambda nb: torch.empty(max(int(nb), 16), dtype=torch.uint8, device=self.device),
                                arena.ranges, alloc=ctx.alloc)
                            cp.persistent = True
                            self._persist_errs += [d.err_tensor for d in fb_descs if isinstance(d, L.PersistDesc)]
                        except S.PersistRefused as e:
                            import warnings
                            warnings.warn("persistent step refused (%s): one launch per level instead" % (e,))
                    if fb_descs is None:
                        fb_descs, cp.fb_levels = S.pack(ids_in_program + jf + jb, alloc=ctx.alloc)
                        if _WL_TUNE and S.BALANCE:
                            fb_descs, cp.level_tuning = self._tune_levels(ids_in_program + jf + jb, ctx.alloc, fb_descs)
                    self._resident_worklists(cp, fb_descs)
                    cp.fb = Program(fb_descs)
                    bwd_descs, cp.bwd_levels = S.pack(bwd_descs)
                    self._resident_worklists(cp, bwd_descs)
                cp.bwd = Program(bwd_descs)
                cp.bwd_tail_start = len(pre) - 1 + ctx.bwd_tail_start
                cp.bwd_marks = [(b, len(pre) - 1 + idx) for b, idx in ctx.block_marks]
                cp.bwd_core = Program(pre[1:] + ctx.bwd)
                last = L.FinalDesc.from_buffer_copy(plain)
                for q in range(L.MAX_SEGS):
                    last.dseg[q] = None
                tail = [ctx.bwd[fi + 1]] if plain.nsplit > 1 else []
                cp.bwd_final_only = Program(pre[1:] + [last] + tail)
                cp.opt = Program(odescs)
                if graph:
                    cp.step = Program((cp.fb.descs if cp.fb is not None else cp.fwd.descs + cp.bwd.descs) + cp.opt.descs)
                    cp.step.capture(self.stream.cuda_stream)
            elif graph:
                cp.fwd.capture(self.stream.cuda_stream)
        if graph or arena is None or cfg.fixed:
            self.stream.synchronize()
        self._plans[key] = cp
        self._last_plan = (fast, choice, cp)
        return cp

    def _resident_worklists(self, cp, descs):
        if not _WL_RESIDENT:
            return
        lists = [d for d in descs if isinstance(d, L.WorklistDesc) and not hasattr(d, "launch_as")]
        if not lists:
            return
        lib = L.load()
        sz = (C.sizeof(L.WorklistDesc) + 255) & ~255
        buf = torch.empty(sz * len(lists), dtype=torch.uint8, device=self.device)
        if not hasattr(cp, "_wl_resident"):
            cp._wl_resident = []
        cp._wl_resident.append(buf)
        self.stream.synchronize()
        for i, d in enumerate(lists):
            dv = L.WorklistDevDesc()
            L.check(lib.nasrec_worklist_prepare(C.addressof(d), buf.data_ptr() + i * sz, C.addressof(dv)))
            d.launch_as = dv

    def _tune_levels(self, prog_in, alloc, default_descs):
        sp = self.stream.cuda_stream

        def sig(descs):
            return hash(b"".join(bytes(d) for d in descs))

        def run_ms(prog, reps):
            e0, e1 = torch.cuda.Event(enable_timing=True), torch.cuda.Event(enable_timing=True)
            e0.record(self.stream)
            for _ in range(reps):
                prog.run(sp)
            e1.record(self.stream)
            e1.synchronize()
            return e0.elapsed_time(e1) / reps

        keep = list(S._MHA_NS)
        cands = [("default", default_descs)]
        seen = {sig(default_descs)}
        try:
            for ns in S.TUNE_MHA_NS:
                S._MHA_NS[:] = list(ns) + keep[len(ns):]
                descs, _ = S.pack(prog_in, alloc=alloc)
                h = sig(descs)
                if h not in seen:
                    seen.add(h)
                    cands.append((",".join(str(v) for v in ns), descs))
        finally:
            S._MHA_NS[:] = keep
        if len(cands) == 1:
            return default_descs, {"candidates": 1, "chosen": "default"}
        progs = [(name, descs, Program(descs)) for name, descs in cands]
        for _, _, pg in progs:
            run_ms(pg, 5)
        times = {name: [] for name, _, _ in progs}
        for _ in range(5):
            for name, _, pg in progs:
                times[name].append(run_ms(pg, 20))
        med = {name: sorted(v)[len(v) // 2] for name, v in times.items()}
        best = min(med, key=med.get)
        if med[best] > med["default"] * (1.0 - _WL_TUNE_MARGIN):
            best = "default"
        chosen = next(descs for name, descs, _ in progs if name == best)
        return chosen, {"candidates": len(progs), "chosen": best, "ms": {k: round(v, 5) for k, v in med.items()}}

    def _build_training_tail(self, cp, ctx, w, bptr, fsegs, B, K, grad_scale):
        cfg, arena = self.cfg, cp.arena
        bd = L.BceDesc()
        bd.kind = L.OP_BCE
        bd.B = B
        bd.grad_scale = grad_scale if grad_scale is not None else 1.0 / B
        bd.logits, bd.y, bd.loss, bd.dlogits = cp.logits.data_ptr(), cp.y.data_ptr(), cp.loss.data_ptr(), cp.dlogits.data_ptr()
        pre = [bd]

        def final_bwd():
            e = L.FinalDesc()
            e.kind = L.OP_FINAL_BWD
            e.B, e.nseg = B, len(fsegs)
            e.w, e.bias, e.dlogits = w, bptr, cp.dlogits.data_ptr()
            e.dw, e.dbias = self.grads["_final.weight"].data_ptr(), self.grads["_final.bias"].data_ptr()
            for q, (s, ts) in enumerate(fsegs):
                gp, acc = ctx.gtarget(s.view)
                e.seg[q], e.dseg[q], e.width[q], e.ld[q], e.off[q], e.dseg_accumulate[q] = s.view.ptr, gp, s.width, s.view.ld, s.koff, acc
                e.tok_stride[q] = ts
            if B > 256:
                e.nsplit = max(2, min(32, B // 128))
                part = ctx.alloc(e.nsplit * (K + 1))
                e.dw = part.data_ptr()
                r = L.ReduceRowsDesc()
                r.kind = L.OP_REDUCE_ROWS
                r.R, r.C, r.ld, r.in_ = e.nsplit, K + 1, K + 1, part.data_ptr()
                r.ndst = 2
                r.dst[0], r.dst_off[0], r.dst_len[0] = self.grads["_final.weight"].data_ptr(), 0, K
                r.dst[1], r.dst_off[1], r.dst_len[1] = self.grads["_final.bias"].data_ptr(), K, 1
                ctx.emit(e)
                ctx.emit(r)
                return
            ctx.emit(e)

        ctx.on_backward(final_bwd)
        ctx.build_backward()
        cp.chunk_tab, cp.nchunks, cp.path_spans = None, 0, None
        if not cfg.fixed:
            names = [n for n in list(ctx.grad_params) + ["_final.weight", "_final.bias"] if not n.startswith("_embedding.")]
            cp.path_spans = [(self.offsets[n], self.params[n].numel()) for n in dict.fromkeys(names)]
            flat = P.path_chunks(cp.path_spans)
            cp.nchunks = len(flat) // 2
            cp.chunk_tab = (arena.alloc(len(flat), torch.int64).tensor() if arena is not None
                            else torch.empty(len(flat), dtype=torch.int64, device=self.device))
            pre += P.const_i64_descs(cp.chunk_tab.data_ptr(), flat)
            ms = P.memset_desc(self.flat_g)
            ms.chunks, ms.nchunks = cp.chunk_tab.data_ptr(), cp.nchunks
            pre.append(ms)
        elif _FIXED_OPT_TABLE:
            names = [n for n in list(ctx.grad_params) + ["_final.weight", "_final.bias"] if not n.startswith("_embedding.")]
            spans = [(self.offsets[n], self.params[n].numel()) for n in dict.fromkeys(names)]
            if sum(n for _, n in spans) < 0.9 * self.flat_numel:
                flat = P.path_chunks(spans, chunk=1024)
                cp.nchunks = len(flat) // 2
                cp.chunk_tab = torch.empty(len(flat), dtype=torch.int64, device=self.device)
                lib = L.load()
                for dsc in P.const_i64_descs(cp.chunk_tab.data_ptr(), flat):
                    L.check(lib.nasrec_launch(self.stream.cuda_stream, C.addressof(dsc)))
                self.stream.synchronize()
        if cp.wd:
            self._weight_decay_tables(cp, ctx, arena, pre)
        if cp.mom is not None:
            self._moments_tables(cp, ctx, arena, pre)
        cp.bce, cp._pre = bd, pre

    WD_BLOCKS = 2048

    def _weight_decay_tables(self, cp, ctx, arena, pre):
        names = [n for n in list(ctx.grad_params) + ["_final.weight", "_final.bias"] if not n.startswith("_embedding.")]
        reached = list(dict.fromkeys(names))
        reg, cp.wd_tables = P.regularised(self.shapes, cp.no_reg)
        on = set(reached)

        def chunks(ns):
            return P.path_chunks([(self.offsets[n], self.params[n].numel()) for n in ns], chunk=1024)
        parts = [chunks([n for n in reg if n in on]), chunks([n for n in reg if n not in on]), chunks(list(dict.fromkeys(reached + reg)))]
        if cp.chunk_tab is None:
            parts.append(chunks(reached))
        flat = [v for part in parts for v in part]
        tab = (arena.alloc(max(1, len(flat)), torch.int64).tensor() if (arena is not None and not self.cfg.fixed)
               else torch.empty(max(1, len(flat)), dtype=torch.int64, device=self.device))
        if not self.cfg.fixed:
            pre += P.const_i64_descs(tab.data_ptr(), flat)
        else:
            lib = L.load()
            for dsc in P.const_i64_descs(tab.data_ptr(), flat):
                L.check(lib.nasrec_launch(self.stream.cuda_stream, C.addressof(dsc)))
            self.stream.synchronize()
        ptrs, off = [], 0
        for part in parts:
            ptrs.append((tab.data_ptr() + 8 * off, len(part) // 2))
            off += len(part)
        cp.wd_add, cp.wd_set, cp.wd_union = ptrs[:3]
        if cp.chunk_tab is None:
            cp.chunk_tab, cp.nchunks = tab[off - len(parts[3]):off], ptrs[3][1]
        cp.wd_tab = tab
        self._row_bitmap()
        if getattr(self, "_wd_part", None) is None:
            with torch.cuda.stream(self.stream):
                self._wd_part = torch.zeros(2 * self.WD_BLOCKS, dtype=torch.float64, device=self.device)
                self._wd_counter = torch.zeros(1, dtype=torch.int32, device=self.device)
                self.wd_l2_sumsq = torch.zeros(1, dtype=torch.float64, device=self.device)
# ... 586 lines not shown
```

nasrec_amd/plan.py:

```python
import ctypes as C
import math
from typing import Dict, List, Optional

import torch

from . import _lib as L

NUM_MHA_HEADS = 8
DS_INTERACT_NUM_SPLITS = 8
E = 16

DENSE_UNARY = ("linear-2d", "zeros-2d")
DENSE_BINARY = ("sum", "sigmoid-gating")
DENSE_SPARSE = ("dot-product",)
SPARSE_NODES = ("zeros-3d", "transformer", "linear-3d")

MHA_LEAVES = ["_mha.in_proj_weight", "_mha.in_proj_bias", "_mha.out_proj.weight", "_mha.out_proj.bias", "_attn_ln.weight",
              "_attn_ln.bias", "attn_fc1.weight", "attn_fc1.bias", "attn_fc2.weight", "attn_fc2.bias", "_attn_fc_ln.weight",
              "_attn_fc_ln.bias"]
MHA_SHAPES = [(48, 16), (48,), (16, 16), (16,), (16,), (16,), (16, 16), (16,), (16, 16), (16,), (16,), (16,)]
MHA_OFFS = [0, 768, 816, 1072, 1088, 1104, 1120, 1376, 1392, 1648, 1664, 1680]


class NetConfig:

    def __init__(self, num_blocks, ops_config, use_layernorm, activation="relu", embedding_dim=16, fixed=False,
                 last_n_blocks_out=1, use_final_sigmoid=False):
        assert embedding_dim == E, "the engine is specialised for embedding_dim == 16 (supernet.py:224)"
        if not 1 <= int(last_n_blocks_out) <= L.MAX_SEGS // 2:
            raise NotImplementedError("last_n_blocks_out = %s: the final-logit descriptor holds %d segments (dense + sparse of at most %d blocks)"
                                      % (last_n_blocks_out, L.MAX_SEGS, L.MAX_SEGS // 2))
        self.last_n_blocks_out = int(last_n_blocks_out)
        self.num_blocks = num_blocks
        self.ops_config = ops_config
        self.use_layernorm = bool(use_layernorm)
        self.activation = activation
        self.fixed = fixed
        self.use_final_sigmoid = use_final_sigmoid

    def block_ops(self, i):
        return self.ops_config[i] if isinstance(self.ops_config, list) else self.ops_config


class Buf:
    def __init__(self, ctx, numel, need_grad=True, tensor=None):
        self.ctx = ctx
        self.numel = numel
        self.t = tensor if tensor is not None else ctx.alloc(numel)
        self.g = None
        self.need_grad = need_grad
        self.written = []

    @property
    def grad_written(self):
        return bool(self.written)

    def mark(self, c0=0, c1=1 << 30):
        self.written.append((c0, c1))

    def overlaps(self, c0, c1):
        return any(a < c1 and c0 < b for a, b in self.written)

    def grad_tensor(self):
        if self.g is None:
            self.g = self.ctx.alloc(self.numel)
        return self.g


class DV:

    def __init__(self, buf, off, width, ld, padded=False):
        self.buf, self.off, self.width, self.ld = buf, off, width, ld
        self.padded = padded

    @property
    def ptr(self):
        return self.buf.t.data_ptr() + 4 * self.off

    @property
    def gptr(self):
        return self.buf.grad_tensor().data_ptr() + 4 * self.off

    def full(self, B):
        if self.padded:
            return self.off == 0 and self.ld * B == self.buf.numel
        return self.off == 0 and self.width == self.ld and self.width * B == self.buf.numel

    def cols(self):
        c0 = self.off % self.ld
        return c0, c0 + self.width


class SV:

    def __init__(self, buf, off, N, ld):
        self.buf, self.off, self.N, self.ld = buf, off, N, ld

    @property
    def ptr(self):
        return self.buf.t.data_ptr() + 4 * self.off

    @property
    def gptr(self):
        return self.buf.grad_tensor().data_ptr() + 4 * self.off

    def dense(self):
        return DV(self.buf, self.off, self.N * E, self.ld)

    def rows(self, n0, n):
        return SV(self.buf, self.off + n0 * E, n, self.ld)

    def full(self, B):
        return self.off == 0 and self.N * E == self.ld and self.N * E * B == self.buf.numel

    def cols(self):
        c0 = self.off % self.ld
        return c0, c0 + self.N * E


class Seg:

    def __init__(self, view, koff, width):
        self.view, self.koff, self.width = view, koff, width


class Ctx:
    def __init__(self, B, device, params: Optional[Dict[str, torch.Tensor]], grads: Optional[Dict[str, torch.Tensor]],
                 shape_only=False, train=True):
        self.B = B
        self.device = device
        self.params = params
        self.grads = grads
        self.shape_only = shape_only
        self.train = train
        self.shapes: Dict[str, tuple] = {}
        self.fwd: List = []
        self.bwd: List = []
        self.closures: List = []
        self.keep: List = []
        self.used_params: List[str] = []
        self._used_set = set()
        self._pcache: Dict[str, tuple] = {}
        self.grad_params: List[str] = []
        self._grad_set = set()
        self.out = self.fwd
        self.deferred: List = []
        self.bwd_tail_start = 0
        self.mha_reduce: List = []
        self.ln_reduce: List = []
        self.defer_dw = True
        self.arena = None
        self.raw_sparse = None
        self.deferred_raw: List = []
        self.sk_workspace = None
        self.mha_bwd_form = 0
        self.block_marks: List = []

    def alloc(self, numel):
        if self.shape_only:
            return _FakeTensor()
        if self.arena is not None:
            return self.arena.alloc(int(numel))
        t = torch.empty(int(numel), dtype=torch.float32, device=self.device)
        self.keep.append(t)
        return t

    def zeros_i32(self, n):
        if self.shape_only:
            return _FakeTensor()
        t = torch.zeros(int(n), dtype=torch.int32, device=self.device)
        self.keep.append(t)
        return t

    def buf(self, numel, need_grad=True):
        return Buf(self, int(numel), need_grad)

    def param(self, name, shape, used=True):
        hit = self._pcache.get(name)
        if hit is not None and hit[0] == shape:
            if used and name not in self._used_set:
                self._used_set.add(name)
                self.used_params.append(name)
            return hit[1]
        shape = tuple(int(s) for s in shape)
        if name in self.shapes:
            assert self.shapes[name] == shape, (name, self.shapes[name], shape)
        self.shapes[name] = shape
        if self.shape_only:
            return 0
        p = self.params[name]
        assert tuple(p.shape) == shape, "parameter %s has shape %s, the path needs %s" % (name, tuple(p.shape), shape)
        if used and name not in self._used_set:
            self._used_set.add(name)
            self.used_params.append(name)
        ptr = p.data_ptr()
        self._pcache[name] = (shape, ptr)
        return ptr

    def gparam(self, name):
        if name not in self._grad_set:
            self._grad_set.add(name)
            self.grad_params.append(name)
        return self.grads[name].data_ptr()

    def emit(self, desc):
        if not self.shape_only:
            self.out.append(desc)

    def on_backward(self, fn):
        if self.train and not self.shape_only:
            self.closures.append(fn)

    def build_backward(self):
        self.out = self.bwd
        for fn in reversed(self.closures):
            fn()
        _flush_raw_dx(self)
        _flush_mha_reduce(self)
        _flush_ln_reduce(self)
        self.bwd_tail_start = len(self.bwd)
        _flush_deferred(self)
        self.out = self.fwd

    def gtarget(self, view):
        buf = view.buf
        if not buf.need_grad:
            return None, 0
        if (self.deferred or self.deferred_raw) and buf.g is not None and not self.shape_only:
            lo = buf.g.data_ptr()
            hi = lo + 4 * buf.numel
            hit = [e for e in self.deferred if lo <= e[4]["A"] < hi]
            if hit:
                self.deferred = [e for e in self.deferred if not (lo <= e[4]["A"] < hi)]
                _flush_deferred(self, hit)
            if any(lo <= e["B"] < hi for e in self.deferred_raw):
                _flush_raw_dx(self)
        acc = buf.grad_written
        if not acc and not view.full(self.B):
            self.emit(memset_desc(buf.grad_tensor()))
            acc = True
        buf.mark(*view.cols())
        return view.gptr, int(acc)

    def live(self, view):
        return view.buf.overlaps(*view.cols())


class _FakeTensor:
    def data_ptr(self):
        return 0


def memset_desc(t):
    d = L.MemsetDesc()
    d.kind = L.OP_MEMSET
    d.bytes = t.numel() * 4
    d.ptr = t.data_ptr()
    return d


def path_chunks(ranges, chunk=None):
    chunk = chunk or L.CHUNK_ELEMS
    merged = []
    for off, n in sorted(ranges):
        if n <= 0:
            continue
        if merged and off <= merged[-1][0] + merged[-1][1]:
            merged[-1][1] = max(merged[-1][1], off + n - merged[-1][0])
        else:
            merged.append([off, n])
    flat = []
    for off, n in merged:
        for o in range(0, n, chunk):
            flat += [off + o, min(chunk, n - o)]
    return flat


def regularised(shapes: Dict[str, tuple], no_reg_param_name=None):
    dense, tables = [], []
    for n, shp in shapes.items():
        if len(shp) < 2 or (no_reg_param_name is not None and n.startswith(no_reg_param_name)):
            continue
        if n.startswith("_embedding."):
            tables.append(int(n.split(".")[1]))
        else:
            dense.append(n)
    return dense, sorted(tables)


def const_i64_descs(dst_ptr, values):
    out = []
    for i in range(0, len(values), L.CONST_I64_MAX):
        part = values[i:i + L.CONST_I64_MAX]
        d = L.ConstI64Desc()
        d.kind = L.OP_CONST_I64
        d.n = len(part)
        d.dst = dst_ptr + 8 * i
        d.vals[:len(part)] = part
        out.append(d)
    return out


import os as _os
_SPLITK_CAP = int(_os.environ["NASREC_SPLITK_CAP"]) if _os.environ.get("NASREC_SPLITK_CAP") else None


def _splitk_for(tiles_mn, ktiles, nprob=1):
    if tiles_mn * nprob >= 192 or ktiles < 8:
        return 1
    if _SPLITK_CAP is not None:
        return max(1, min(_SPLITK_CAP, ktiles // 2, max(1, 256 // max(1, tiles_mn * nprob))))
    s = min(ktiles // 2, max(1, 256 // max(1, tiles_mn * nprob)))
    return max(1, min(s, 32))


GEMM_FAST_MIN_TILES = 120
_FAST_MIN_K = int(_os.environ.get("NASREC_FAST_MIN_K", "1"))
_LN_NBLK = int(_os.environ.get("NASREC_LN_NBLK", "512"))
_TOKDW_CAP = int(_os.environ.get("NASREC_TOKDW_CAP", "128"))
_FAST_MIN_KT = int(_os.environ.get("NASREC_FAST_MIN_KT", "4"))


def _fast_gemm_splitk(amode, bmode, cmode, segs, zmode):
    if cmode != L.CM_PLAIN or (amode, bmode) not in _FAST_BINDINGS:
        return None
    kmax = 0
    kt_max = kt_sum = 0
    any_live = False
    for sd in segs:
        if sd.get("Aaux") or sd.get("Baux"):
            return None
        if not sd.get("A"):
            continue
        any_live = True
        K = sd["K"]
        if K > kmax:
            kmax = K
        r, ld = max(sd["M"], sd["N"]), max(sd.get("lda", 0), sd.get("ldb", 0))
        if r * ld + K >= (1 << 29) or K * ld + r >= (1 << 29):
            return None
        kt = (K + 31) // 32
        kt_sum += kt
        if kt > kt_max:
            kt_max = kt
    if not any_live or kmax < _FAST_MIN_K:
        return None
    tiles = area = 0
    for sd in (segs if zmode else segs[:1]):
        tiles += ((sd["M"] + 127) // 128) * ((sd["N"] + 127) // 128)
        area += sd["M"] * sd["N"]
    if 2 * area < tiles * 128 * 128:
        return None
    kt = kt_max if zmode else kt_sum
    S = 1
    if tiles < 256:
        S = max(1, min(-(-256 // tiles), kt // _FAST_MIN_KT, 32))
    return S if tiles * S >= GEMM_FAST_MIN_TILES else None


_FAST_BINDINGS = ((L.AM_KC, L.AM_KC), (L.AM_KC, L.AM_RC), (L.AM_RC, L.AM_RC))
def kslice_eligible(amode, bmode, cmode, segs, zmode):
    if (amode, bmode, cmode) != (L.AM_KC, L.AM_KC, L.CM_PLAIN) or zmode:
        return False
    M, N = segs[0]["M"], segs[0]["N"]
    K = 0
    for sd in segs:
        if sd.get("Aaux") or sd.get("Baux") or sd.get("ones_col") or (0 < sd.get("Mvalid", M) < M):
            return False
        if sd.get("A") and sd["K"] > 0:
            K += sd["K"]
            if M * sd["lda"] >= (1 << 29) or N * sd["ldb"] >= (1 << 29):
                return False
    if len(segs) > 4:
        return False
    tiles = ((M + 31) // 32) * ((N + 31) // 32)
    return M <= 512 and 128 <= tiles <= 512 and K >= 512


def skinny_n_eligible(amode, bmode, cmode, segs, zmode):
    if amode != L.AM_KC or bmode not in (L.AM_KC, L.AM_RC) or cmode != L.CM_PLAIN or (zmode and len(segs) != 1):
        return False
    M, N = segs[0]["M"], segs[0]["N"]
    if N < 1 or N > 16 or M < 1024:
        return False
    K = 0
    for sd in segs:
        if sd.get("Aaux") or sd.get("Baux") or sd.get("ones_col") or (0 < sd.get("Mvalid", M) < M):
            return False
        if sd.get("A") and sd["K"] > 0:
            K += sd["K"]
            if M * sd.get("lda", 0) >= (1 << 29) or (sd["K"] if bmode == L.AM_RC else N) * sd.get("ldb", 0) >= (1 << 29):
                return False
    return K >= 256 and _SKINNY_N


_SKINNY_N = _os.environ.get("NASREC_SKINNY_N", "1") != "0"
BALANCED_MIN_SAVING_US = float(_os.environ.get("NASREC_BALANCED_MIN_US", "80.0"))


def _balanced_schedule_pays(segs, zmode):
    live = [sd for sd in segs if sd.get("A")]
    if not live or len(live) != len(segs):
        return False
    if zmode:
        kts = {(sd["K"] + 31) // 32 for sd in segs}
        if len(kts) != 1:
            return False
        T = kts.pop()
        probs = segs
    else:
        T = sum((sd["K"] + 31) // 32 for sd in segs)
        probs = segs[:1]
    tiles = sum(((sd["M"] + 127) // 128) * ((sd["N"] + 127) // 128) for sd in probs)
    left = tiles % 512
    if left == 0:
        return False
    rounds = tiles // 512 + (1.0 if left > 64 else 0.55)
    return (rounds - tiles / 512.0) * T * 3.8 >= BALANCED_MIN_SAVING_US


_TINYK = _os.environ.get("NASREC_TINYK", "1") != "0"
_TINYK_RC = _os.environ.get("NASREC_TINYK", "1") == "2"


def tinyk_eligible(d) -> bool:
    if not _TINYK or d.amode != L.AM_KC or d.bmode not in (L.AM_KC, L.AM_RC) or d.cmode != L.CM_PLAIN or d.splitk > 1:
        return False
    if d.bmode == L.AM_RC and not _TINYK_RC:
        return False
    if not d.zmode and d.nseg != 1:
        return False
    for q in range(d.nseg):
        s = d.seg[q]
        if s.Aaux or s.Baux or s.ones_col or (0 < s.Mvalid < s.M):
            return False
        if s.M < 1024 or s.N < 256 or s.K < 0 or s.K > 16:
            return False
    return True


def gemm_kernel_name(d) -> str:
    segs = [dict(A=d.seg[q].A, Aaux=d.seg[q].Aaux, Baux=d.seg[q].Baux, M=d.seg[q].M, N=d.seg[q].N, K=d.seg[q].K) for q in range(d.nseg)]
    live = [sd for sd in segs if sd["A"]]
    if d.splitk <= 1 and kslice_eligible(d.amode, d.bmode, d.cmode, [dict(sd, ones_col=d.seg[q].ones_col, Mvalid=d.seg[q].Mvalid, lda=d.seg[q].lda,
                                                                          ldb=d.seg[q].ldb) for q, sd in enumerate(segs)], d.zmode):
        return "gemm_kslice_kernel"
    if d.splitk <= 1 and skinny_n_eligible(d.amode, d.bmode, d.cmode, [dict(sd, ones_col=d.seg[q].ones_col, Mvalid=d.seg[q].Mvalid, lda=d.seg[q].lda,
                                                                            ldb=d.seg[q].ldb) for q, sd in enumerate(segs)], d.zmode):
        return "gemm_skinny_n_kernel"
    if tinyk_eligible(d):
        return "gemm_tinyk_kernel"
    if (d.cmode == L.CM_TOKJ and d.bmode == L.AM_TOKR and d.amode in (L.AM_KC, L.AM_RC) and d.splitk <= 1 and not d.pre_add
            and not d.save_act and d.mul_nseg == 0 and all(sd["M"] <= 80 and sd["N"] >= 16 * 1024 and not sd["Aaux"] and not sd["Baux"] for sd in segs)):
        return "token_linear_kernel"
    if d.cmode != L.CM_PLAIN or (d.amode, d.bmode) not in ((L.AM_KC, L.AM_KC), (L.AM_KC, L.AM_RC), (L.AM_RC, L.AM_RC)) or not live:
        return "gemm_kernel"
    if any(sd["Aaux"] or sd["Baux"] for sd in segs) or max(sd["K"] for sd in live) < _FAST_MIN_K:
        return "gemm_kernel"
    probs = segs if d.zmode else segs[:1]
    tiles = sum(((sd["M"] + 127) // 128) * ((sd["N"] + 127) // 128) for sd in probs)
    if 2 * sum(sd["M"] * sd["N"] for sd in probs) < tiles * 128 * 128:
        return "gemm_kernel"
    return "gemm_fast_kernel" if tiles * max(1, d.splitk) >= GEMM_FAST_MIN_TILES else "gemm_kernel"


def gemm_descs(ctx, amode, bmode, cmode, segs, zmode, act=0, bias_on_rows=0, mask_on_rows=0, dims=-1, beta=0, bias=None, save_z=None,
               save_act=None, pre_add=None, mul=None, splitk=None, rowsum_out=None):
    if not segs:
        return []
    nseg = len(segs)
    assert nseg <= L.MAX_SEGS
    d = L.GemmDesc()
    d.kind = L.OP_GEMM
    d.amode, d.bmode, d.cmode = amode, bmode, cmode
    d.nseg = nseg
    d.zmode = zmode
    if act:
        d.act = act
    if bias_on_rows:
        d.bias_on_rows = bias_on_rows
    if mask_on_rows:
        d.mask_on_rows = mask_on_rows
    d.dims_in_use = dims
    if beta:
        d.beta = beta
    if bias:
        d.bias = bias
    if save_z:
        d.save_z = save_z
    if save_act:
        d.save_act = save_act
    if pre_add:
        d.pre_add = pre_add
    if mul:
        assert len(mul) <= L.MAX_SEGS
        d.mul_nseg = len(mul)
        for q, (ptr, off, width, ld) in enumerate(mul):
            d.mul_ptr[q], d.mul_off[q], d.mul_width[q], d.mul_ld[q] = ptr, off, width, ld
    M = N = 0
    kt_max = kt_sum = live_tiles = 0
    dseg = d.seg
    for q in range(nseg):
        sdict = segs[q]
        s = dseg[q]
        for k, v in sdict.items():
            setattr(s, k, v)
        m, n = sdict["M"], sdict["N"]
        if "Mvalid" not in sdict:
            s.Mvalid = m
        if m > M:
            M = m
        if n > N:
            N = n
        kt = (sdict["K"] + 31) // 32
        kt_sum += kt
        if kt > kt_max:
            kt_max = kt
        live_tiles += ((m + 63) // 64) * ((n + 63) // 64)
    B = ctx.B
    if zmode:
        S = _splitk_for(live_tiles, kt_max)
    else:
        S = _splitk_for(((M + 63) // 64) * ((N + 63) // 64), kt_sum)
    fast = _fast_gemm_splitk(amode, bmode, cmode, segs, zmode) if B > 128 else None
    if fast is not None:
        S = fast
    if amode == L.AM_TOKK and zmode and B >= 1024:
        ok = True
        for sd in segs:
            if sd["M"] > 80 or sd["N"] > 80 or sd.get("Aaux") or sd.get("Baux"):
                ok = False
                break
        if ok:
            S = max(4, min(_TOKDW_CAP, 256 // nseg, B // 64))
    if splitk is not None:
        S = splitk
    elif B <= 512 and S > 1 and kslice_eligible(amode, bmode, cmode, segs, zmode):
        S = 1
    elif B >= 1024 and skinny_n_eligible(amode, bmode, cmode, segs, zmode):
        S = 1
    d.splitk = 1
    if fast == 1 and S == 1 and B > 256 and ctx.sk_workspace is not None and _balanced_schedule_pays(segs, zmode):
        d.splitk = L.SPLITK_BALANCED
        d.workspace = ctx.sk_workspace().data_ptr()
    if S > 1:
        d.splitk = S
        ws = ctx.alloc(S * M * N * (nseg if zmode else 1))
        d.workspace = ws.data_ptr()
    if rowsum_out is not None:
        d.rowsum_out = rowsum_out
    return [d]


def _live_segs(segs: List[Seg]):
    return [s for s in segs if s.view is not None]


def _cover_pieces(live: List[Seg]):
    cuts = sorted({s.koff for s in live} | {s.koff + s.width for s in live})
    out = []
    for a, b in zip(cuts[:-1], cuts[1:]):
        rank = 0
        for s in live:
            if s.koff <= a and b <= s.koff + s.width:
                if out and out[-1][0] is s and out[-1][2] == a and out[-1][3] == rank:
                    out[-1] = (s, out[-1][1], b, rank)
                else:
                    out.append((s, a, b, rank))
                rank += 1
    return out


def _split_column_remainder(ctx, bm, cm, d):
    if ctx.B <= 256 or cm != L.CM_PLAIN or bm not in (L.AM_KC, L.AM_RC) or not d.get("A"):
        return [d]
    N, ones = d["N"], int(bool(d.get("ones_col")))
    r = N % 128
    if N <= 128 or r == 0 or r > 16 or r - ones < 1 or d["M"] < 128:
        return [d]
    Nm = N - r
    step = 4 * Nm * (d["ldb"] if bm == L.AM_KC else 1)
    main = dict(d, N=Nm, ones_col=0, rowsum=None)
    rem = dict(d, N=r, B=d["B"] + step, C=d["C"] + 4 * Nm)
    if d.get("Baux"):
        rem["Baux"] = d["Baux"] + step
    return [main, rem]


def _emit_z_groups(ctx, am, bm, cm, items, rowsum_out=None):
    items = [(g, p) for g, d in _with_rowsum(items, rowsum_out) for p in _split_column_remainder(ctx, bm, cm, d)]
    for gi in sorted({g for g, _ in items}):
        grp = [d for g, d in items if g == gi]
        for cls in sorted({_shape_class(ctx, d) for d in grp}):
            part = [d for d in grp if _shape_class(ctx, d) == cls]
            for i in range(0, len(part), L.MAX_SEGS):
                for d in gemm_descs(ctx, am, bm, cm, part[i:i + L.MAX_SEGS], 1):
                    ctx.emit(d)


def _shape_class(ctx, d):
    return (d["M"] < 64, d["N"] < 64) if ctx.B > 256 else (False, False)


def _with_rowsum(items, rowsum_out):
    if rowsum_out is None or not items:
        return list(items)
    items = list(items)
    g0 = min(g for g, _ in items)
    i0 = next(i for i, (g, _) in enumerate(items) if g == g0)
    g, d = items[i0]
    items[i0] = (g, dict(d, N=d["N"] + 1, ones_col=1, rowsum=rowsum_out))
    return items

# ... 112 lines not shown


def _flush_raw_dx(ctx):
    items, ctx.deferred_raw = ctx.deferred_raw, []
    if not items:
        return
    view = items[0]["view"]
    gp, acc = ctx.gtarget(view)
    if gp is None:
        return
    for i in range(0, len(items), L.MAX_SEGS):
        segs = [dict(A=e["A"], B=e["B"], Baux=e["Baux"], C=gp, M=e["M"], N=e["N"], K=e["K"], lda=e["lda"], ldb=e["ldb"], ldc=view.ld)
                for e in items[i:i + L.MAX_SEGS]]
        for d in gemm_descs(ctx, L.AM_RC, L.AM_TOKR, L.CM_TOKJ, segs, 0, beta=int(acc or i > 0)):
            ctx.emit(d)


def _is_whole_raw(ctx, s):
    v = s.view
    return ctx.defer_dw and ctx.raw_sparse is not None and v.buf is ctx.raw_sparse and v.off == 0 and v.N * E == v.ld and s.width == v.N


def _dx_groups(ctx, live, mk):
    items, seen = [], {}
    for s in live:
        gp, acc = ctx.gtarget(s.view)
        if gp is None:
            continue
        g = seen.get(id(s.view.buf), 0)
        seen[id(s.view.buf)] = g + 1
        items.append((g, mk(s, gp, acc)))
    return items


def emit_layernorm(ctx, mode, x_ptr, ldx, R, D, wname, out_ptr, ldy, act, dims, accumulate, out_view, x_grad_cb):
    w = ctx.param(wname + ".weight", (D,))
    b = ctx.param(wname + ".bias", (D,))
    if ctx.shape_only:
        return
    stats = ctx.alloc(R * 2)
    d = L.LayerNormDesc()
    d.kind = L.OP_LAYERNORM_FWD
    d.mode, d.R, d.D, d.ldx, d.ldy = mode, R, D, ldx, ldy
    d.act, d.dims_in_use, d.accumulate, d.eps = act, dims, accumulate, 1e-5
    d.x, d.w, d.b, d.y, d.stats = x_ptr, w, b, out_ptr, stats.data_ptr()
    ctx.emit(d)

    def bwd():
        if not ctx.live(out_view):
            return
        nblk = min((R + 3) // 4, _LN_NBLK) if mode == L.AM_KC else (R + 255) // 256
        part = ctx.alloc(nblk * 2 * D)
        dx = ctx.alloc(_ln_numel(mode, R, D, ldx))
        e = L.LayerNormDesc()
        e.kind = L.OP_LAYERNORM_BWD
        e.mode, e.R, e.D, e.ldx, e.ldy = mode, R, D, ldx, ldy
        e.act, e.dims_in_use, e.accumulate, e.eps = act, dims, 0, 1e-5
        e.x, e.w, e.b, e.stats = x_ptr, w, b, stats.data_ptr()
        e.dy = out_view.gptr
        e.dx = dx.data_ptr()
        e.dwb_partial = part.data_ptr()
        e.nblk = nblk
        ctx.emit(e)
        r = L.ReduceRowsDesc()
        r.kind = L.OP_REDUCE_ROWS
        r.R, r.C, r.ld = nblk, 2 * D, 2 * D
        r.in_ = part.data_ptr()
        r.ndst = 2
        r.dst[0], r.dst_off[0], r.dst_len[0] = ctx.gparam(wname + ".weight"), 0, D
        r.dst[1], r.dst_off[1], r.dst_len[1] = ctx.gparam(wname + ".bias"), D, D
        if ctx.B > 256 and _LN_REDUCE_BATCH:
            ctx.ln_reduce.append(r)
        else:
            ctx.emit(r)
        x_grad_cb(dx)

    ctx.on_backward(bwd)


def _ln_numel(mode, R, D, ld):
    if mode == L.AM_KC:
        return R * ld
    return (R // 16) * ld


def linear_dense(ctx, segs: List[Seg], Ktot, wname, nout, bias: bool, out: DV, act=L.ACT_NONE, dims=-1, beta=0, ln=None,
                 mul=None, save_act: Optional[DV] = None, pre_dz_cb=None, pre_add: Optional[DV] = None):
    B = ctx.B
    W = ctx.param(wname + ".weight", (nout, Ktot))
    bptr = ctx.param(wname + ".bias", (nout,)) if bias else None
    if ctx.shape_only:
        if ln:
            ctx.param(ln + ".weight", (nout,))
            ctx.param(ln + ".bias", (nout,))
        return
    live = _live_segs(segs)
    if pre_add is not None:
        assert not ln and act == L.ACT_NONE and dims < 0 and beta == 0 and pre_add.ld == out.ld and pre_add.width == nout
    if len(live) > L.MAX_SEGS and not ln and (act != L.ACT_NONE or mul is not None):
        raise NotImplementedError("more than %d live input segments for the activated product %s" % (L.MAX_SEGS, wname))
    need_z = act == L.ACT_SILU and not ln
    zbuf = None
    if ln:
        zbuf = ctx.alloc(B * nout)
        tgt_ptr, tgt_ld = zbuf.data_ptr(), nout
        g_act, g_dims, g_beta = L.ACT_NONE, -1, 0
    else:
        tgt_ptr, tgt_ld = out.ptr, out.ld
        g_act, g_dims, g_beta = act, dims, beta
    savez = ctx.alloc(B * nout) if need_z else None
    sd = [dict(A=s.view.ptr, B=W + 4 * s.koff, C=tgt_ptr, M=B, N=nout, K=s.width, lda=s.view.ld, ldb=Ktot, ldc=tgt_ld) for s in live]
    if not sd:
        sd = [dict(A=None, B=W, C=tgt_ptr, M=B, N=nout, K=0, lda=1, ldb=Ktot, ldc=tgt_ld)]
    mul_list = None
    if mul is not None:
        mul_list = [(m.view.ptr, m.koff, m.width, m.view.ld) for m in mul if m.view is not None]
        if not mul_list:
            mul_list = [(None, 0, 1, 1)]
    for c0 in range(0, len(sd), L.MAX_SEGS):
        for d in gemm_descs(ctx, L.AM_KC, L.AM_KC, L.CM_PLAIN, sd[c0:c0 + L.MAX_SEGS], 0, act=g_act, dims=g_dims,
                            beta=g_beta if c0 == 0 else 1, bias=bptr if c0 == 0 else None,
                            save_z=savez.data_ptr() if need_z else None, save_act=save_act.ptr if save_act is not None else None,
                            mul=mul_list, pre_add=pre_add.ptr if (pre_add is not None and c0 == 0) else None):
            ctx.emit(d)

    def backward_products(dz_ptr, dz_ld, aux_ptr, kdims):
        kd = nout if kdims < 0 else min(kdims, nout)
        _emit_z_groups(ctx, L.AM_KC, L.AM_RC, L.CM_PLAIN, _dx_groups(ctx, live, lambda s, gp, acc: dict(
            A=dz_ptr, Aaux=aux_ptr, B=W + 4 * s.koff, C=gp, M=B, N=s.width, K=kd, lda=dz_ld, ldb=Ktot, ldc=s.view.ld, accumulate=acc)))
        gW = ctx.gparam(wname + ".weight")
        _weight_grad_products(ctx, L.AM_RC, L.AM_RC, L.CM_PLAIN, [(rank, dict(
            A=dz_ptr, Aaux=aux_ptr, B=s.view.ptr + 4 * (a - s.koff), C=gW + 4 * a, M=nout, N=b - a, K=B, lda=dz_ld, ldb=s.view.ld, ldc=Ktot,
            Mvalid=kd, accumulate=int(rank > 0))) for s, a, b, rank in _cover_pieces(live)],
            rowsum_out=ctx.gparam(wname + ".bias") if (bias and live) else None)
        if bias and not live:
            r = L.RowsumDesc()
            r.kind = L.OP_ROWSUM
            r.mode, r.R, r.K, r.ld, r.rvalid = L.AM_RC, nout, B, dz_ld, kd
            r.p, r.aux, r.out = dz_ptr, aux_ptr, ctx.gparam(wname + ".bias")
            ctx.emit(r)

    if ln:
        emit_layernorm(ctx, L.AM_KC, zbuf.data_ptr(), nout, B, nout, ln, out.ptr, out.ld, act, dims, beta, out,
                       lambda dx: backward_products(dx.data_ptr(), nout, None, -1))
        return

    def bwd():
        if pre_dz_cb is not None:
            r = pre_dz_cb()
            if r is None:
                return
            dz_ptr, dz_ld = r
            backward_products(dz_ptr, dz_ld, None, -1)
            return
        if not ctx.live(out):
            return
        if act == L.ACT_RELU:
            backward_products(out.gptr, out.ld, out.ptr, dims)
        elif act == L.ACT_SILU:
            dz = ctx.alloc(B * nout)
            a = L.ActBwdDesc()
            a.kind = L.OP_ACT_BWD
            a.mode, a.R, a.D = L.AM_KC, B, nout
            a.ld_dy, a.ld_z, a.ld_dz = out.ld, nout, nout
            a.act, a.dims_in_use = act, dims
            a.dy, a.z, a.dz = out.gptr, savez.data_ptr(), dz.data_ptr()
            ctx.emit(a)
            backward_products(dz.data_ptr(), nout, None, -1)
        else:
            backward_products(out.gptr, out.ld, None, dims)

    ctx.on_backward(bwd)


def linear_tokens(ctx, segs: List[Seg], Ntot, wname, nout, bias: bool, out: SV, act=L.ACT_NONE, dims=-1, ln=None):
    B = ctx.B
    W = ctx.param(wname + ".weight", (nout, Ntot))
    bptr = ctx.param(wname + ".bias", (nout,)) if bias else None
    if ctx.shape_only:
        if ln:
            ctx.param(ln + ".weight", (nout,))
            ctx.param(ln + ".bias", (nout,))
        return
    live = _live_segs(segs)
    if len(live) > L.MAX_SEGS:
        raise NotImplementedError("more than %d live input segments for %s" % (L.MAX_SEGS, wname))
    need_z = act == L.ACT_SILU and not ln
    if ln:
        zbuf = ctx.alloc(B * nout * E)
        tgt_ptr, tgt_ld = zbuf.data_ptr(), nout * E
        g_act, g_dims = L.ACT_NONE, -1
    else:
        tgt_ptr, tgt_ld = out.ptr, out.ld
        g_act, g_dims = act, dims
    savez = ctx.alloc(B * nout * E) if need_z else None
    sd = [dict(A=W + 4 * s.koff, B=s.view.ptr, C=tgt_ptr, M=nout, N=B * E, K=s.width, lda=Ntot, ldb=s.view.ld, ldc=tgt_ld) for s in live]
    if not sd:
        sd = [dict(A=None, B=W, C=tgt_ptr, M=nout, N=B * E, K=0, lda=Ntot, ldb=1, ldc=tgt_ld)]
    for d in gemm_descs(ctx, L.AM_KC, L.AM_TOKR, L.CM_TOKJ, sd, 0, act=g_act, dims=g_dims, bias=bptr, bias_on_rows=1, mask_on_rows=1,
                        save_z=savez.data_ptr() if need_z else None):
        ctx.emit(d)

    def backward_products(dz_ptr, dz_ld, aux_ptr, kdims):
        kd = nout if kdims < 0 else min(kdims, nout)
        for s in live:
            if _is_whole_raw(ctx, s) and s.view.buf.need_grad:
                ctx.deferred_raw.append(dict(A=W + 4 * s.koff, B=dz_ptr, Baux=aux_ptr, M=s.width, N=B * E, K=kd, lda=Ntot, ldb=dz_ld, view=s.view))
        rest = [s for s in live if not (_is_whole_raw(ctx, s) and s.view.buf.need_grad)]
        _emit_z_groups(ctx, L.AM_RC, L.AM_TOKR, L.CM_TOKJ, _dx_groups(ctx, rest, lambda s, gp, acc: dict(
            A=W + 4 * s.koff, B=dz_ptr, Baux=aux_ptr, C=gp, M=s.width, N=B * E, K=kd, lda=Ntot, ldb=dz_ld, ldc=s.view.ld, accumulate=acc)))
        gW = ctx.gparam(wname + ".weight")
        _weight_grad_products(ctx, L.AM_TOKK, L.AM_TOKK, L.CM_PLAIN, [(rank, dict(
            A=dz_ptr, Aaux=aux_ptr, B=s.view.ptr + 4 * (a - s.koff) * E, C=gW + 4 * a, M=nout, N=b - a, K=B * E, lda=dz_ld, ldb=s.view.ld,
            ldc=Ntot, Mvalid=kd, accumulate=int(rank > 0))) for s, a, b, rank in _cover_pieces(live)],
            rowsum_out=ctx.gparam(wname + ".bias") if (bias and live) else None)
        if bias and not live:
            r = L.RowsumDesc()
            r.kind = L.OP_ROWSUM
            r.mode, r.R, r.K, r.ld, r.rvalid = L.AM_TOKK, nout, B * E, dz_ld, kd
            r.p, r.aux, r.out = dz_ptr, aux_ptr, ctx.gparam(wname + ".bias")
            ctx.emit(r)

    if ln:
        emit_layernorm(ctx, L.AM_TOKR, zbuf.data_ptr(), nout * E, B * E, nout, ln, out.ptr, out.ld, act, dims, 0, out,
                       lambda dx: backward_products(dx.data_ptr(), nout * E, None, -1))
        return

    def bwd():
        if not ctx.live(out):
            return
        if act == L.ACT_RELU:
            backward_products(out.gptr, out.ld, out.ptr, dims)
        elif act == L.ACT_SILU:
            dz = ctx.alloc(B * nout * E)
            a = L.ActBwdDesc()
            a.kind = L.OP_ACT_BWD
            a.mode, a.R, a.D = L.AM_TOKR, B * E, nout
            a.ld_dy, a.ld_z, a.ld_dz = out.ld, nout * E, nout * E
            a.act, a.dims_in_use = act, dims
            a.dy, a.z, a.dz = out.gptr, savez.data_ptr(), dz.data_ptr()
            ctx.emit(a)
# ... 194 lines not shown
    emit_layernorm(ctx, L.AM_KC, x.ptr, x.ld, ctx.B, D, lnname, tgt.view.ptr, tgt.view.ld, act, mask, tgt.accumulate, tgt.view, xgrad)


def op_sigmoid_gating(ctx, cfg, pre, lsegs, Ltot, rsegs, Rtot, max_dims, dims, tgt: Target):
    B = ctx.B
    D = _pad_width(lsegs, Ltot, rsegs, Rtot)
    use_ln = cfg.use_layernorm
    mask = -1 if cfg.fixed else dims
    sl = pre + "._left_self_linear._linear"
    need_proj = D != max_dims
    masked_plain = (not need_proj) and (not use_ln) and 0 <= mask < D
    own = need_proj or use_ln or masked_plain
    Dp = (D + 31) // 32 * 32 if (own and B > 256) else D
    gbuf = ctx.buf(B * Dp, need_grad=False)
    g = DV(gbuf, 0, D, Dp, padded=True)
    if own:
        pbuf = ctx.buf(B * Dp)
        prod = DV(pbuf, 0, D, Dp, padded=True)
        ptgt = Target(prod, 0)
    else:
        prod = tgt.view
        ptgt = tgt
    dzbuf = {}

    def pre_dz():
        if not ctx.live(prod):
            return None
        dz = ctx.alloc(B * Dp)
        e = L.GateBwdDesc()
        e.kind = L.OP_GATE_BWD
        e.B, e.D = B, D
        e.ld_dout, e.ld_g, e.ld_dz = prod.ld, Dp, Dp
        e.dout, e.g, e.dz = prod.gptr, g.ptr, dz.data_ptr()
        n = 0
        for s in _live_segs(rsegs):
            gp, acc = ctx.gtarget(s.view)
            e.r_ptr[n], e.dr_ptr[n] = s.view.ptr, gp
            e.r_off[n], e.r_width[n], e.r_ld[n], e.dr_accumulate[n] = s.koff, s.width, s.view.ld, acc
            n += 1
        e.nseg = n
        ctx.emit(e)
        return dz.data_ptr(), Dp

    linear_dense(ctx, lsegs, D, sl, D, True, prod, L.ACT_SIGMOID, -1, ptgt.accumulate, mul=rsegs, save_act=g, pre_dz_cb=pre_dz)
    if need_proj:
        linear_dense(ctx, [Seg(prod, 0, D)], D, pre + "._linear_proj", max_dims, True, tgt.view, L.ACT_NONE, mask, tgt.accumulate,
                     ln=(pre + "._layernorm") if use_ln else None)
    elif use_ln:
        emit_ln_dense(ctx, prod, D, pre + "._layernorm", tgt, L.ACT_NONE, mask)
    elif masked_plain and not ctx.shape_only:
        masked_copy(ctx, prod, mask, tgt)


def op_transformer(ctx, cfg, pre, ssegs, Ntot, max_dims, dims, out: SV):
    B = ctx.B
    use_ln = cfg.use_layernorm
    mask = -1 if cfg.fixed else dims
    xbuf = ctx.buf(B * max_dims * E)
    x = SV(xbuf, 0, max_dims, max_dims * E)
    linear_tokens(ctx, ssegs, Ntot, pre + "._linear_proj", max_dims, not use_ln, x, L.ACT_NONE, mask,
                  ln=(pre + "._proj_ln") if use_ln else None)
    pp = [ctx.param(pre + "." + leaf, shp) for leaf, shp in zip(MHA_LEAVES, MHA_SHAPES)]
    if ctx.shape_only:
        return
    saved = ctx.alloc(B * max_dims * L.MHA_SAVED) if ctx.train else None
    d = L.MhaDesc()
    d.kind = L.OP_MHA_FWD
    d.B, d.N, d.ldx, d.ldo, d.dims_in_use = B, max_dims, x.ld, out.ld, mask
    d.x, d.out = x.ptr, out.ptr
    d.saved = saved.data_ptr() if saved is not None else None
    for q in range(12):
        d.params[q] = pp[q]
    ctx.emit(d)

    def bwd():
        if not ctx.live(out):
            return
        e = L.MhaDesc()
        e.kind = L.OP_MHA_BWD
        e.B, e.N, e.ldx, e.ldo, e.dims_in_use = B, max_dims, x.ld, out.ld, mask
        e.x, e.dout = x.ptr, out.gptr
        e.dx = xbuf.grad_tensor().data_ptr()
        xbuf.mark()
        e.saved = saved.data_ptr() if saved is not None else None
        e.bwd_form = ctx.mha_bwd_form
        for q in range(12):
            e.params[q] = pp[q]
        ctx.emit(e)
        ctx.mha_reduce.append((e, [(ctx.gparam(pre + "." + leaf), MHA_OFFS[q], int(torch.Size(MHA_SHAPES[q]).numel()))
                                   for q, leaf in enumerate(MHA_LEAVES)]))

    ctx.on_backward(bwd)


def op_fm(ctx, cfg, pre, x: SV, fm_dims, dims, dense_out: DV, pre_add: Optional[DV] = None):
    B = ctx.B
    use_ln = cfg.use_layernorm
    mask = -1 if cfg.fixed else dims
    masked_direct = fm_dims == E and 0 <= mask < E
    direct = fm_dims == E and not masked_direct
    if masked_direct:
        assert pre_add is None
    if direct:
        ix = dense_out
        if use_ln:
            ctx.param(pre + "._linear_layernorm.weight", (fm_dims,), used=False)
            ctx.param(pre + "._linear_layernorm.bias", (fm_dims,), used=False)
    else:
        ixbuf = ctx.buf(B * E)
        ix = DV(ixbuf, 0, E, E)
    if not ctx.shape_only:
        d = L.FmDesc()
        d.kind = L.OP_FM_FWD
        d.B, d.N, d.ldx, d.ld_ix, d.accumulate = B, x.N, x.ld, ix.ld, 1 if (direct and pre_add is None) else 0
        d.x, d.ix = x.ptr, ix.ptr
        if direct and pre_add is not None:
            assert pre_add.ld == ix.ld and pre_add.width == E
            d.add = pre_add.ptr
        ctx.emit(d)

        def bwd():
            if not ctx.live(ix):
                return
            gp, acc = ctx.gtarget(x)
            if gp is None:
                return
            e = L.FmDesc()
            e.kind = L.OP_FM_BWD
            e.B, e.N, e.ldx, e.ld_ix, e.accumulate = B, x.N, x.ld, ix.ld, acc
            e.x, e.dix, e.dx = x.ptr, ix.gptr, gp
            ctx.emit(e)

        ctx.on_backward(bwd)
    if masked_direct:
        if use_ln:
            ctx.param(pre + "._linear_layernorm.weight", (fm_dims,), used=False)
            ctx.param(pre + "._linear_layernorm.bias", (fm_dims,), used=False)
        if not ctx.shape_only:
            masked_copy(ctx, ix, mask, Target(dense_out, 1))
    elif not direct:
        linear_dense(ctx, [Seg(ix, 0, E)], E, pre + "._linear_proj", fm_dims, not use_ln, dense_out, L.ACT_NONE, mask,
                     0 if pre_add is not None else 1, ln=(pre + "._linear_layernorm") if use_ln else None, pre_add=pre_add)


def _as_set(v):
    return set(int(x) for x in (v.tolist() if hasattr(v, "tolist") else v))


def _mk_segs(views, widths, selected, fixed):
    segs, off = [], 0
    for j, (v, w) in enumerate(zip(views, widths)):
        if j in selected:
            segs.append(Seg(v, off, w))
            off += w
        elif not fixed:
            segs.append(Seg(None, off, w))
            off += w
    return segs, off


def block_walk(ctx, cfg, pre, ops, choice, d_in, Dtot, s_in, Ntot, l_in, Ltot, r_in, Rtot):
    B = ctx.B
    fixed = cfg.fixed
    dd, sdm = int(choice["dense_in_dims"]), int(choice["sparse_in_dims"])
    max_dense = dd if fixed else int(max(ops["dense_node_dims"]))
    max_sparse = sdm if fixed else int(max(ops["sparse_node_dims"]))
# ... 226 lines not shown
```

nasrec_amd/schedule.py:

```python
import ctypes as C
import os
from typing import List, Tuple

from . import _lib as L

E = 16
MHA_PARAM_FLOATS = [768, 48, 256, 16, 16, 16, 256, 16, 256, 16, 16, 16]


class Acc:
    __slots__ = ("ptr", "width", "stride", "rows", "end")

    def __init__(self, ptr, rows, width_f, ld_f):
        self.ptr = int(ptr)
        self.rows = max(int(rows), 1)
        self.width = int(width_f) * 4
        self.stride = int(ld_f) * 4 if self.rows > 1 else self.width
        if self.stride < self.width:
            self.stride = self.width
        self.end = self.ptr + (self.rows - 1) * self.stride + self.width


def _flat(ptr, n_floats):
    return Acc(ptr, 1, n_floats, n_floats)
# ... 107 lines not shown
                R.append(Acc(d.add, d.B, E, d.ld_ix))
        else:
            R.append(Acc(d.dix, d.B, E, d.ld_ix))
            dx = Acc(d.dx, d.B, d.N * E, d.ldx)
            W.append(dx)
            if d.accumulate:
                R.append(dx)
    elif k in (L.OP_MHA_FWD, L.OP_MHA_BWD):
        R.append(Acc(d.x, d.B, d.N * E, d.ldx))
        for q in range(12):
            R.append(_flat(d.params[q], MHA_PARAM_FLOATS[q]))
        sv = _flat(d.saved, d.B * d.N * L.MHA_SAVED) if d.saved else None
        if k == L.OP_MHA_FWD:
            W.append(Acc(d.out, d.B, d.N * E, d.ldo))
            if sv:
                W.append(sv)
        else:
            R.append(Acc(d.dout, d.B, d.N * E, d.ldo))
            if sv:
                R.append(sv)
            W.append(Acc(d.dx, d.B, d.N * E, d.ldx))
            W.append(Acc(d.dparams_partial, d.B, L.MHA_PARAMS, d.partial_ld if d.partial_ld > 0 else L.MHA_PARAMS))
    elif k == L.OP_REDUCE_ROWS:
        R.append(Acc(d.in_, d.R, d.C, d.ld))
        for q in range(d.ndst):
            if d.dst[q]:
                W.append(_flat(d.dst[q], d.dst_len[q]))
    elif k == L.OP_COPY_SEGS:
        for q in range(d.nseg):
            win = Acc(d.dst + 4 * d.off[q], d.B, d.width[q], d.ld_dst)
            seg = Acc(d.seg[q], d.B, d.width[q], d.ld[q]) if d.seg[q] else None
            if not d.reverse:
                W.append(win)
                if d.accumulate:
                    R.append(win)
                if seg:
                    R.append(seg)
            elif seg:
                R.append(win)
                W.append(seg)
                if d.seg_accumulate[q]:
                    R.append(seg)
    elif k == L.OP_GATE_BWD:
        R += [Acc(d.dout, d.B, d.D, d.ld_dout), Acc(d.g, d.B, d.D, d.ld_g)]
        W.append(Acc(d.dz, d.B, d.D, d.ld_dz))
        for q in range(d.nseg):
            if d.r_ptr[q]:
                R.append(Acc(d.r_ptr[q], d.B, d.r_width[q], d.r_ld[q]))
            if d.dr_ptr[q]:
                a = Acc(d.dr_ptr[q], d.B, d.r_width[q], d.r_ld[q])
                W.append(a)
                if d.dr_accumulate[q]:
                    R.append(a)
    elif k == L.OP_ROWSUM:
        R.append(_operand(d.p, d.mode, d.R, d.K, d.ld))
        if d.aux:
            R.append(_operand(d.aux, d.mode, d.R, d.K, d.ld))
        W.append(_flat(d.out, d.R))
    elif k in (L.OP_FINAL_FWD, L.OP_FINAL_BWD, L.OP_FINAL_FUSED):
        def extent(q):
            ts, Wq = d.tok_stride[q], d.width[q]
            return ((Wq - 1) // 16) * ts + (Wq - 1) % 16 + 1 if (ts and Wq > 0) else Wq
        K = max([d.off[q] + extent(q) for q in range(d.nseg)] + [0])
        for q in range(d.nseg):
            if d.seg[q]:
                R.append(Acc(d.seg[q], d.B, d.width[q], d.ld[q]))
        R.append(_flat(d.w, K))
        if k in (L.OP_FINAL_FWD, L.OP_FINAL_FUSED):
            R.append(_flat(d.bias, 1))
            W.append(_flat(d.logits, d.B))
        if k == L.OP_FINAL_FUSED:
            R.append(_flat(d.y, d.B))
        if k == L.OP_FINAL_BWD:
            for ptr in (d.dlogits, d.logits, d.y):
                if ptr:
                    R.append(_flat(ptr, d.B))
        if k == L.OP_FINAL_FUSED or (k == L.OP_FINAL_BWD and not d.dseg_done):
            for q in range(d.nseg):
                if d.dseg[q]:
                    a = Acc(d.dseg[q], d.B, d.width[q], d.ld[q])
                    W.append(a)
                    if d.dseg_accumulate[q]:
                        R.append(a)
        if k == L.OP_FINAL_BWD:
            W.append(_flat(d.dw, (K + 1) * max(d.nsplit, 1)))
            for ptr, n in ((d.dbias, 1), (d.loss, 1), (d.dlogits_out, d.B)):
                if ptr:
                    W.append(_flat(ptr, n))
    elif k == L.OP_BCE:
        R += [_flat(d.logits, d.B), _flat(d.y, d.B)]
        W += [_flat(d.loss, 1), _flat(d.dlogits, d.B)]
    elif k in (L.OP_LAYERNORM_FWD, L.OP_LAYERNORM_BWD):
        if d.mode == L.AM_KC:
            vx = lambda p, ld: Acc(p, d.R, d.D, ld)
            ndx = d.R * d.ldx
        else:
            vx = lambda p, ld: Acc(p, d.R // 16, d.D * E, ld)
            ndx = (d.R // 16) * d.ldx
        R += [vx(d.x, d.ldx), _flat(d.w, d.D), _flat(d.b, d.D)]
        st = _flat(d.stats, d.R * 2)
        if k == L.OP_LAYERNORM_FWD:
            y = vx(d.y, d.ldy)
            W += [y, st]
            if d.accumulate:
                R.append(y)
        else:
            R += [st, vx(d.dy, d.ldy)]
            W += [_flat(d.dx, ndx), _flat(d.dwb_partial, d.nblk * 2 * d.D)]
    elif k == L.OP_ACT_BWD:
        if d.mode == L.AM_KC:
            v = lambda p, ld: Acc(p, d.R, d.D, ld)
        else:
            v = lambda p, ld: Acc(p, d.R // 16, d.D * E, ld)
        R += [v(d.dy, d.ld_dy), v(d.z, d.ld_z)]
        W.append(v(d.dz, d.ld_dz))
    elif k == L.OP_DEDUP_IDS:
        R.append(_flat(d.idx, d.B * d.Fs * 2))
        W += [_flat(d.leader, d.B * d.Fs), _flat(d.order, d.Fs * d.cap), _flat(d.lists, d.Fs * d.cap), _flat(d.counts, d.Fs * 2)]
        if d.heads:
            W.append(_flat(d.heads, d.Fs * d.cap))
    elif k == L.OP_MEMSET and not d.chunks:
        W.append(_flat(d.ptr, (d.bytes + 3) // 4))
    else:
        return None
    return [a for a in R if a is not None and a.ptr], [a for a in W if a is not None and a.ptr]


class Node:
    __slots__ = ("desc", "part", "reads", "writes", "level", "index")

    def __init__(self, desc, part="whole"):
        self.desc, self.part = desc, part
        io = desc_io(desc, part)
        self.reads, self.writes = io if io is not None else (None, None)
        self.level = 0
        self.index = 0


def expand(descs) -> List[Node]:
    nodes = []
    for d in descs:
        if isinstance(d, L.GemmDesc) and d.splitk > 1 and not d.defer_second_pass:
            nodes.append(Node(d, "main"))
            nodes.append(Node(d, "epi"))
        else:
            nodes.append(Node(d))
    for i, n in enumerate(nodes):
        n.index = i
    return nodes


def _depends(later: Node, earlier: Node) -> bool:
    if later.reads is None or earlier.reads is None:
        return True
    for w in earlier.writes:
        for a in later.reads:
            if overlap(w, a):
                return True
        for a in later.writes:
            if overlap(w, a):
                return True
    for r in earlier.reads:
        for a in later.writes:
            if overlap(r, a):
                return True
    return False
# ... 113 lines not shown
                d = delta(moves)
                if d is not None and d < best:
                    best, best_moves = d, moves
            if best_moves:
                for k, lv in best_moves.items():
                    m = nodes[k]
                    if lv != m.level:
                        levels[m.level] = [x for x in levels[m.level] if x is not m]
                        levels[lv].append(m)
                        m.level = lv
                moved = True
        if not moved:
            break


RESPLIT = os.environ.get("NASREC_WL_RESPLIT", "0") == "1"
RESPLIT_MIN_SLACK = 3


def resplit_slack_solos(descs, alloc, min_slack=None):
    from . import plan as P
    nodes = expand_for_worklists(descs)
    nl = assign_levels(nodes)
    n = len(nodes)
    alap = [nl - 1] * n
    for i in range(n - 1, -1, -1):
        for j in range(i + 1, n):
            if alap[j] - 1 < alap[i] and _depends(nodes[j], nodes[i]):
                alap[i] = alap[j] - 1
    out, changed = list(descs), False
    for i, nd in enumerate(nodes):
        d = nd.desc
        if nd.part != "whole" or not isinstance(d, L.GemmDesc) or d.splitk > 1 or alap[i] - nd.level < (RESPLIT_MIN_SLACK if min_slack is None else min_slack):
            continue
        if P.gemm_kernel_name(d) != "gemm_kslice_kernel":
            continue
        s0 = d.seg[0]
        kt = sum((d.seg[q].K + 31) // 32 for q in range(d.nseg) if d.seg[q].A)
        S = P._splitk_for(((s0.M + 63) // 64) * ((s0.N + 63) // 64), kt)
        if S <= 1:
            continue
        d2 = L.GemmDesc.from_buffer_copy(d)
        d2.splitk = S
        ws = alloc(S * s0.M * s0.N)
        d2.workspace = ws.data_ptr()
        d2._wl_force, d2._keep = True, ws
        out[next(k for k, x in enumerate(out) if x is d)] = d2
        changed = True
    return out if changed else descs


def levels_of(descs):
    nodes = expand(descs)
    nl = assign_levels(nodes)
    out = [[] for _ in range(nl)]
    for n in nodes:
        out[n.level].append(n)
    return out


_GEMM_HEAD = L.GemmDesc.seg.offset
_SEG_BYTES = C.sizeof(L.GemmSeg)
_PLAIN_KINDS = (L.OP_MHA_FWD, L.OP_MHA_BWD, L.OP_FM_FWD, L.OP_FM_BWD, L.OP_DOT_TRI_FWD, L.OP_DOT_TRI_BWD, L.OP_COPY_SEGS, L.OP_GATE_BWD,
                L.OP_FINAL_FWD, L.OP_FINAL_BWD, L.OP_DEDUP_IDS, L.OP_FINAL_FUSED)
WL_LDS_FLOATS = 1696 + 5 * 1024 + 1024


SOLO_TILES = int(os.environ.get("NASREC_WL_SOLO_TILES", "256"))


def gemm_capable(d) -> bool:
    if d.splitk == L.SPLITK_BALANCED or d.defer_second_pass:
        return False
    kca, kcb = d.amode in (L.AM_KC, L.AM_TOKK), d.bmode in (L.AM_KC, L.AM_TOKK)
    if not kca and kcb:
        return False
    if d.splitk > 1 and not d.workspace:
        return False
    nprob = d.nseg if d.zmode else 1
    S = d.splitk if d.splitk > 1 else 1
    if nprob == 1 and ((d.seg[0].M + 63) // 64) * ((d.seg[0].N + 63) // 64) * S >= SOLO_TILES:
        return False
    from . import plan as P
    if not getattr(d, "_wl_force", False) and P.kslice_eligible(d.amode, d.bmode, d.cmode, [dict(A=d.seg[q].A, Aaux=d.seg[q].Aaux, Baux=d.seg[q].Baux, ones_col=d.seg[q].ones_col,
                                                           Mvalid=d.seg[q].Mvalid, M=d.seg[q].M, N=d.seg[q].N, K=d.seg[q].K, lda=d.seg[q].lda,
                                                           ldb=d.seg[q].ldb) for q in range(d.nseg)], d.zmode):
        return False
    s0 = d.seg[0]
    if not d.zmode:
        for q in range(d.nseg):
            s = d.seg[q]
            if s.ones_col != s0.ones_col or s.Mvalid != s0.Mvalid:
                return False
            if s.A and (bool(s.Aaux) != bool(s0.Aaux) or bool(s.Baux) != bool(s0.Baux)):
                return False
    return True


def item_bytes(node):
    d = node.desc
    k = d.kind
    if isinstance(d, L.GemmDesc):
        if not gemm_capable(d):
            return None
        return C.string_at(C.addressof(d), _GEMM_HEAD + d.nseg * _SEG_BYTES)
    if k in (L.OP_DOT_TRI_FWD, L.OP_DOT_TRI_BWD):
        P4 = (d.k1 * (d.k1 - 1) // 2 + 3) & ~3
        if d.k1 < 2 or 4 * (d.k1 * 20 + P4) > WL_LDS_FLOATS:
            return None
    if k in (L.OP_MHA_FWD, L.OP_MHA_BWD) and (d.N < 1 or d.N > 64 or (k == L.OP_MHA_BWD and not d.saved)):
        return None
    if k == L.OP_DEDUP_IDS and (d.B > 256 or d.cap != 256):
        return None
    if k in _PLAIN_KINDS:
        return C.string_at(C.addressof(d), C.sizeof(d))
    if k == L.OP_REDUCE_ROWS and 1 <= d.ndst <= L.WL_REDUCE_DST:
        r = L.WlReduce()
        r.kind, r.R, r.C, r.ld, r.in_, r.ndst = d.kind, d.R, d.C, d.ld, d.in_, d.ndst
        for q in range(d.ndst):
            r.dst[q], r.dst_off[q], r.dst_len[q] = d.dst[q], d.dst_off[q], d.dst_len[q]
        return C.string_at(C.addressof(r), C.sizeof(r))
    return None


_PART = {"whole": L.WL_WHOLE, "main": L.WL_MAIN, "epi": L.WL_EPI}


_ITEM_NS = {L.OP_MHA_BWD: 18000, L.OP_MHA_FWD: 11000, L.OP_DOT_TRI_BWD: 10000, L.OP_DOT_TRI_FWD: 6000, L.OP_REDUCE_ROWS: 4500,
            L.OP_FM_BWD: 3900, L.OP_FM_FWD: 3500, L.OP_FINAL_BWD: 7500, L.OP_DEDUP_IDS: 8000, L.OP_FINAL_FUSED: 4500}
_ITEM_NS_R4 = {L.OP_MHA_BWD: 18500, L.OP_MHA_FWD: 10500, L.OP_REDUCE_ROWS: 6000, L.OP_FM_BWD: 7000, L.OP_FM_FWD: 3500, L.OP_FINAL_BWD: 7000,
               L.OP_FINAL_FWD: 3400, L.OP_GATE_BWD: 3500, L.OP_DEDUP_IDS: 8000, L.OP_FINAL_FUSED: 4500}
_COST_MODEL = os.environ.get("NASREC_WL_COST", "time")
_MHA_NS = [int(v) for v in os.environ.get("NASREC_WL_MHA_NS", "10500,0,16000,0,4,4").split(",")]
TUNE_MHA_NS = [(f, 0, b, 0) for f in (8000, 10500) for b in (12000, 14000, 16000, 18500, 21000, 24000)] + [(6000, 0, 24000, 0), (3500, 95, 6400, 105)]


def _mha_ns(d):
    return _MHA_NS[0] + _MHA_NS[1] * d.N if d.kind == L.OP_MHA_FWD else _MHA_NS[2] + _MHA_NS[3] * d.N


def _cost(node):
    d = node.desc
    if _COST_MODEL == "size":
        if isinstance(d, L.GemmDesc):
            return 1 if node.part == "epi" else sum(d.seg[q].M * d.seg[q].N * max(d.seg[q].K, 1) for q in range(d.nseg) if d.seg[q].A)
        if d.kind in (L.OP_MHA_FWD, L.OP_MHA_BWD):
            return d.B * d.N * 16 * 4000 * (2 if d.kind == L.OP_MHA_BWD else 1)
        return 1000
    if isinstance(d, L.GemmDesc):
        if node.part == "epi":
            return 3600
        return 5000 + sum(d.seg[q].M * d.seg[q].N * max(d.seg[q].K, 1) for q in range(d.nseg) if d.seg[q].A) // 20000
    if d.kind == L.OP_FINAL_BWD and d.dseg_done:
        return 5000
    if d.kind in (L.OP_MHA_FWD, L.OP_MHA_BWD):
        return _mha_ns(d)
    return _ITEM_NS.get(d.kind, 3000)


def _cost_r4(node):
    d = node.desc
    if isinstance(d, L.GemmDesc):
        if node.part == "epi":
            return 4000
        live = [q for q in range(d.nseg) if d.seg[q].A]
        extra = 0 if d.zmode else 900 * max(len(live) - 1, 0)
        return 5200 + extra + sum(d.seg[q].M * d.seg[q].N * max(d.seg[q].K, 1) for q in live) // _GEMM_DIV
# ... 246 lines not shown
```

Baseline: 1.158 million.

## Apply ReLU gradient mask at the final-layer producer instead of in GEMM consumers

When a ReLU linear's output gradient is written by the final-layer backward kernel, that kernel now also writes a ReLU-masked copy of the gradient using the saved activation as the mask. The downstream dx and dW GEMMs then read the pre-masked buffer instead of applying the Aaux mask inside the GEMM. The aim is to stop re-reading the activation and masking in every consumer GEMM. In exchange it allocates an extra gradient buffer, adds mask reads and writes in the final kernel, and marks those segments pmask, which excludes them from the fast, kslice, skinny and token GEMM paths. It is on by default for B<=256 and can be turned off with NASREC_RELU_MASK=consumer.

```diff
diff --git a/include/nasrec_hip.h b/include/nasrec_hip.h
--- a/include/nasrec_hip.h
+++ b/include/nasrec_hip.h
@@ -81,7 +81,7 @@
   int32_t Mvalid;
   int32_t accumulate;
   int32_t ones_col;
-  int32_t _pad;
+  int32_t pmask;
 } nasrec_gemm_seg_t;
 
 typedef struct nasrec_gemm_desc {
@@ -242,6 +242,8 @@
   int32_t nsplit;
   int32_t dseg_done;
   int32_t tok_stride[NASREC_MAX_SEGS];
+  const float* dseg_mask[NASREC_MAX_SEGS];
+  float* dseg_masked[NASREC_MAX_SEGS];
 } nasrec_final_desc_t;
 
 typedef struct nasrec_bce_desc {
diff --git a/nasrec_amd/_lib.py b/nasrec_amd/_lib.py
--- a/nasrec_amd/_lib.py
+++ b/nasrec_amd/_lib.py
@@ -39,7 +39,7 @@
 
 class GemmSeg(C.Structure):
     _fields_ = [("A", vp), ("B", vp), ("C", vp), ("Aaux", vp), ("Baux", vp), ("rowsum", vp), ("M", i32), ("N", i32), ("K", i32),
-                ("lda", i32), ("ldb", i32), ("ldc", i32), ("Mvalid", i32), ("accumulate", i32), ("ones_col", i32), ("_pad", i32)]
+                ("lda", i32), ("ldb", i32), ("ldc", i32), ("Mvalid", i32), ("accumulate", i32), ("ones_col", i32), ("pmask", i32)]
 
 
 class GemmDesc(C.Structure):
@@ -107,7 +107,8 @@
     _fields_ = [("kind", i32), ("B", i32), ("nseg", i32), ("grad_scale", f32), ("w", vp), ("bias", vp), ("logits", vp), ("dlogits", vp),
                 ("dw", vp), ("dbias", vp), ("seg", vp * MAX_SEGS), ("dseg", vp * MAX_SEGS), ("width", i32 * MAX_SEGS),
                 ("ld", i32 * MAX_SEGS), ("off", i32 * MAX_SEGS), ("dseg_accumulate", i32 * MAX_SEGS), ("y", vp), ("loss", vp),
-                ("dlogits_out", vp), ("nsplit", i32), ("dseg_done", i32), ("tok_stride", i32 * MAX_SEGS)]
+                ("dlogits_out", vp), ("nsplit", i32), ("dseg_done", i32), ("tok_stride", i32 * MAX_SEGS),
+                ("dseg_mask", vp * MAX_SEGS), ("dseg_masked", vp * MAX_SEGS)]
 
 
 class BceDesc(C.Structure):
diff --git a/nasrec_amd/csrc/common.h b/nasrec_amd/csrc/common.h
--- a/nasrec_amd/csrc/common.h
+++ b/nasrec_amd/csrc/common.h
@@ -101,6 +101,7 @@
 int launch_rowsum(hipStream_t s, const nasrec_rowsum_desc_t* d);
 int launch_final(hipStream_t s, const nasrec_final_desc_t* d);
 int final_fused_check(const nasrec_final_desc_t* d);
+int final_mask_check(const nasrec_final_desc_t* d);
 int launch_bce(hipStream_t s, const nasrec_bce_desc_t* d);
 int launch_sumsq(hipStream_t s, const nasrec_sumsq_desc_t* d);
 int launch_clip_coef(hipStream_t s, const nasrec_clip_coef_desc_t* d);
diff --git a/nasrec_amd/csrc/final_bodies.h b/nasrec_amd/csrc/final_bodies.h
--- a/nasrec_amd/csrc/final_bodies.h
+++ b/nasrec_amd/csrc/final_bodies.h
@@ -59,10 +59,19 @@
   const int b = vb;
   if (b >= d.B) return;
   const float yb = d.y[b];
+  const int tid = threadIdx.x;
+  int qm = -1;
+  for (int q = 0; q < d.nseg; ++q)
+    if (qm < 0 && d.dseg_masked[q] && d.dseg[q] && d.seg[q]) qm = q;
+  float mpre[4] = {0.f, 0.f, 0.f, 0.f};
+  if (qm >= 0) {
+    const float* mk = d.dseg_mask[qm] + (long)b * d.ld[qm];
+#pragma unroll
+    for (int u = 0; u < 4; ++u) mpre[u] = mk[min(tid + 256 * u, d.width[qm] - 1)];
+  }
   const float z = final_logit(d, b, red);
   if (threadIdx.x == 0) d.logits[b] = z;
   const float g = bce_grad(z, yb, d.grad_scale);
-  const int tid = threadIdx.x;
   for (int q = 0; q < d.nseg; ++q) {
     float* p = d.dseg[q];
     if (!p || !d.seg[q]) continue;
@@ -70,18 +79,26 @@
     const float* w = d.w + d.off[q];
     const int W = d.width[q], ts = d.tok_stride[q];
     const bool acc = d.dseg_accumulate[q] != 0;
+    float* pm = d.dseg_masked[q];
+    const float* mk = pm ? d.dseg_mask[q] + (long)b * d.ld[q] : nullptr;
+    if (pm) pm += (long)b * d.ld[q];
     for (int j0 = tid; j0 < W; j0 += 256 * 4) {
-      float wv[4], cv[4];
+      float wv[4], cv[4], mv[4];
 #pragma unroll
       for (int u = 0; u < 4; ++u) {
         const int j = min(j0 + 256 * u, W - 1);
         wv[u] = w[ts ? (j >> 4) * ts + (j & 15) : j];
         cv[u] = acc ? p[j] : 0.f;
+        mv[u] = pm ? ((q == qm && j0 == tid) ? mpre[u] : mk[j]) : 0.f;
       }
 #pragma unroll
       for (int u = 0; u < 4; ++u) {
         const float v = g * wv[u];
-        if (j0 + 256 * u < W) p[j0 + 256 * u] = acc ? cv[u] + v : v;
+        const float o = acc ? cv[u] + v : v;
+        if (j0 + 256 * u < W) {
+          p[j0 + 256 * u] = o;
+          if (pm) pm[j0 + 256 * u] = mv[u] > 0.f ? o : 0.f;
+        }
       }
     }
   }
@@ -107,6 +124,8 @@
     const int rblk = vb / kblocks, k = (vb - rblk * kblocks) * 256 + (int)threadIdx.x;
     if (k >= K) return;
     float* p0 = nullptr;
+    float* pm = nullptr;
+    const float* mk = nullptr;
     long ldq = 0;
     bool accq = false;
     for (int q = 0; q < d.nseg; ++q) {
@@ -116,6 +135,10 @@
           p0 = d.dseg[q] + jj;
           ldq = d.ld[q];
           accq = d.dseg_accumulate[q] != 0;
+          if (d.dseg_masked[q]) {
+            pm = d.dseg_masked[q] + jj;
+            mk = d.dseg_mask[q] + jj;
+          }
         }
         break;
       }
@@ -123,17 +146,22 @@
     if (!p0) return;
     const float wk = d.w[k];
     const int r0 = rblk * RB;
-    float z[RB], y[RB], c[RB], g[RB];
+    float z[RB], y[RB], c[RB], g[RB], m[RB];
 #pragma unroll
     for (int u = 0; u < RB; ++u) {
       const int b = min(r0 + u, d.B - 1);
       z[u] = dl_a[b];
       y[u] = dl_b[b];
       c[u] = 0.f;
+      m[u] = 0.f;
     }
     if (accq) {
 #pragma unroll
       for (int u = 0; u < RB; ++u) c[u] = p0[(long)min(r0 + u, d.B - 1) * ldq];
+    }
+    if (pm) {
+#pragma unroll
+      for (int u = 0; u < RB; ++u) m[u] = mk[(long)min(r0 + u, d.B - 1) * ldq];
     }
     if (fused) {
 #pragma unroll
@@ -147,7 +175,9 @@
     for (int u = 0; u < RB; ++u) {
       if (r0 + u >= d.B) break;
       const float v = g[u] * wk;
-      p0[(long)(r0 + u) * ldq] = accq ? c[u] + v : v;
+      const float o = accq ? c[u] + v : v;
+      p0[(long)(r0 + u) * ldq] = o;
+      if (pm) pm[(long)(r0 + u) * ldq] = m[u] > 0.f ? o : 0.f;
     }
     return;
   }
@@ -159,9 +189,12 @@
       const int jj = final_feat(d, q, k);
       if (jj >= 0) {
         if (d.dseg[q]) {
-          float* p = d.dseg[q] + (long)b * d.ld[q] + jj;
+          const long e = (long)b * d.ld[q] + jj;
+          float* p = d.dseg[q] + e;
           const float v = dl(b) * d.w[k];
-          *p = d.dseg_accumulate[q] ? *p + v : v;
+          const float o = d.dseg_accumulate[q] ? *p + v : v;
+          *p = o;
+          if (d.dseg_masked[q]) d.dseg_masked[q][e] = d.dseg_mask[q][e] > 0.f ? o : 0.f;
         }
         break;
       }
diff --git a/nasrec_amd/csrc/gemm_fast.hip b/nasrec_amd/csrc/gemm_fast.hip
--- a/nasrec_amd/csrc/gemm_fast.hip
+++ b/nasrec_amd/csrc/gemm_fast.hip
@@ -650,7 +650,7 @@
   long tiles = 0, kmax = 0;
   for (int q = 0; q < d->nseg; ++q) {
     const nasrec_gemm_seg_t& s = d->seg[q];
-    if (s.Aaux || s.Baux) return false;
+    if (s.Aaux || s.Baux || s.pmask) return false;
     if (s.A && s.K > kmax) kmax = s.K;
     const long r = s.M > s.N ? s.M : s.N, ld = s.lda > s.ldb ? s.lda : s.ldb;
     if (s.A && (r * ld + s.K >= (1L << 29) || (long)s.K * ld + r >= (1L << 29))) return false;
diff --git a/nasrec_amd/csrc/gemm_kslice.hip b/nasrec_amd/csrc/gemm_kslice.hip
--- a/nasrec_amd/csrc/gemm_kslice.hip
+++ b/nasrec_amd/csrc/gemm_kslice.hip
@@ -327,7 +327,7 @@
   long K = 0;
   for (int q = 0; q < d->nseg; ++q) {
     const nasrec_gemm_seg_t& s = d->seg[q];
-    if (s.Aaux || s.Baux || s.ones_col || (s.Mvalid > 0 && s.Mvalid < s0.M)) return false;
+    if (s.Aaux || s.Baux || s.pmask || s.ones_col || (s.Mvalid > 0 && s.Mvalid < s0.M)) return false;
     if (s.A && s.K > 0) {
       K += s.K;
       if ((long)s0.M * s.lda >= (1L << 29) || (long)s0.N * s.ldb >= (1L << 29)) return false;
diff --git a/nasrec_amd/csrc/gemm_skinny.hip b/nasrec_amd/csrc/gemm_skinny.hip
--- a/nasrec_amd/csrc/gemm_skinny.hip
+++ b/nasrec_amd/csrc/gemm_skinny.hip
@@ -104,7 +104,7 @@
   long K = 0;
   for (int q = 0; q < d->nseg; ++q) {
     const nasrec_gemm_seg_t& s = d->seg[q];
-    if (s.Aaux || s.Baux || s.ones_col || (s.Mvalid > 0 && s.Mvalid < s0.M)) return false;
+    if (s.Aaux || s.Baux || s.pmask || s.ones_col || (s.Mvalid > 0 && s.Mvalid < s0.M)) return false;
     if (s.A && s.K > 0) {
       K += s.K;
       if ((long)s0.M * s.lda >= (1L << 29) || (long)(d->bmode == NASREC_AM_RC ? s.K : s0.N) * s.ldb >= (1L << 29)) return false;
@@ -210,7 +210,7 @@
   if (!d->zmode && d->nseg != 1) return false;
   for (int q = 0; q < d->nseg; ++q) {
     const nasrec_gemm_seg_t& s = d->seg[q];
-    if (s.Aaux || s.Baux || s.ones_col || (s.Mvalid > 0 && s.Mvalid < s.M)) return false;
+    if (s.Aaux || s.Baux || s.pmask || s.ones_col || (s.Mvalid > 0 && s.Mvalid < s.M)) return false;
     if (s.M < 1024 || s.N < 256 || s.K < 0 || s.K > TK_MAXK) return false;
   }
   return true;
diff --git a/nasrec_amd/csrc/norm_loss_opt.hip b/nasrec_amd/csrc/norm_loss_opt.hip
--- a/nasrec_amd/csrc/norm_loss_opt.hip
+++ b/nasrec_amd/csrc/norm_loss_opt.hip
@@ -16,6 +16,15 @@
 __global__ __launch_bounds__(256) void final_fused_kernel(const nasrec_final_desc_t d) {
   __shared__ float red[4];
   final_fused_block(d, blockIdx.x, red);
+}
+
+int final_mask_check(const nasrec_final_desc_t* d) {
+  for (int q = 0; q < NASREC_MAX_SEGS; ++q) {
+    const bool live = q < d->nseg && d->dseg[q];
+    if (d->dseg_masked[q] && (!live || !d->dseg_mask[q] || d->kind == NASREC_OP_FINAL_FWD))
+      return nasrec_set_error(-2, "final: segment %d has a masked gradient copy without a gradient destination / mask source in kind %d", q, d->kind);
+  }
+  return 0;
 }
 
 int final_fused_check(const nasrec_final_desc_t* d) {
@@ -23,11 +32,12 @@
   if (d->nsplit > 1) return nasrec_set_error(-2, "final_fused: nsplit=%d (the batch-sliced backward keeps its own launch)", d->nsplit);
   for (int q = 0; q < d->nseg; ++q)
     if (d->dseg[q] && !d->seg[q]) return nasrec_set_error(-2, "final_fused: segment %d has a gradient destination and no input", q);
-  return 0;
+  return final_mask_check(d);
 }
 
 int launch_final(hipStream_t st, const nasrec_final_desc_t* d) {
   if (d->B == 0) return 0;
+  if (const int rc = final_mask_check(d)) return rc;
   if (d->kind == NASREC_OP_FINAL_FUSED) {
     const int rc = final_fused_check(d);
     if (rc) return rc;
diff --git a/nasrec_amd/csrc/token_linear.hip b/nasrec_amd/csrc/token_linear.hip
--- a/nasrec_amd/csrc/token_linear.hip
+++ b/nasrec_amd/csrc/token_linear.hip
@@ -125,7 +125,7 @@
     long kp = 0;
     for (int q = d->zmode ? p : 0; q < (d->zmode ? p + 1 : d->nseg); ++q) {
       const nasrec_gemm_seg_t& s = d->seg[q];
-      if (s.Aaux || s.Baux) return false;
+      if (s.Aaux || s.Baux || s.pmask) return false;
       if (!d->zmode && (s.M != s0.M || s.N != s0.N)) return false;
       if (s.A && s.K > 0) kp += (s.K + 3) & ~3;
       if ((long)s.K * 64 > 0x7fffffffL) return false;
@@ -250,7 +250,7 @@
   if (d->splitk < 2 || !d->workspace) return false;
   for (int q = 0; q < d->nseg; ++q) {
     const nasrec_gemm_seg_t& s = d->seg[q];
-    if (s.Aaux || s.Baux) return false;
+    if (s.Aaux || s.Baux || s.pmask) return false;
     if (s.M < 1 || s.M > 80 || s.N < 1 || s.N > 80) return false;
     if ((s.K & 15) || (s.K >> 4) < 1024) return false;
   }
diff --git a/nasrec_amd/csrc/worklist.hip b/nasrec_amd/csrc/worklist.hip
--- a/nasrec_amd/csrc/worklist.hip
+++ b/nasrec_amd/csrc/worklist.hip
@@ -186,6 +186,7 @@
       }
       case NASREC_OP_FINAL_FWD:
         WL_NEED(nasrec_final_desc_t);
+        if (const int rc = final_mask_check(reinterpret_cast<const nasrec_final_desc_t*>(blob))) return rc;
         it.nblk = reinterpret_cast<const nasrec_final_desc_t*>(blob)->B;
         break;
       case NASREC_OP_FINAL_FUSED: {
@@ -199,6 +200,7 @@
         WL_NEED(nasrec_final_desc_t);
         const nasrec_final_desc_t* d = reinterpret_cast<const nasrec_final_desc_t*>(blob);
         if (d->y != nullptr && d->logits == nullptr) return nasrec_set_error(-2, "worklist: final_bwd with the fused loss needs desc.logits");
+        if (const int rc = final_mask_check(d)) return rc;
         int K, nA, nB;
         final_bwd_geometry(*d, K, nA, nB);
         it.geom[0] = K, it.geom[1] = nA, it.geom[2] = nB;
diff --git a/nasrec_amd/engine.py b/nasrec_amd/engine.py
--- a/nasrec_amd/engine.py
+++ b/nasrec_amd/engine.py
@@ -474,7 +474,7 @@
                 cp.bwd_core = Program(pre[1:] + ctx.bwd)
                 last = L.FinalDesc.from_buffer_copy(plain)
                 for q in range(L.MAX_SEGS):
-                    last.dseg[q] = None
+                    last.dseg[q] = last.dseg_masked[q] = last.dseg_mask[q] = None
                 tail = [ctx.bwd[fi + 1]] if plain.nsplit > 1 else []
                 cp.bwd_final_only = Program(pre[1:] + [last] + tail)
                 cp.opt = Program(odescs)
@@ -570,6 +570,7 @@
                 gp, acc = ctx.gtarget(s.view)
                 e.seg[q], e.dseg[q], e.width[q], e.ld[q], e.off[q], e.dseg_accumulate[q] = s.view.ptr, gp, s.width, s.view.ld, s.koff, acc
                 e.tok_stride[q] = ts
+                P.note_final_producer(ctx, e, q)
             if B > 256:
                 e.nsplit = max(2, min(32, B // 128))
                 part = ctx.alloc(e.nsplit * (K + 1))
diff --git a/nasrec_amd/plan.py b/nasrec_amd/plan.py
--- a/nasrec_amd/plan.py
+++ b/nasrec_amd/plan.py
@@ -1,5 +1,6 @@
 import ctypes as C
 import math
+import os as _os
 from typing import Dict, List, Optional
 
 import torch
@@ -155,6 +156,8 @@
         self.sk_workspace = None
         self.mha_bwd_form = 0
         self.block_marks: List = []
+        self.gwrites: List = []
+        self.relu_at_producer = relu_mask_at_producer() and B <= 256
 
     def alloc(self, numel):
         if self.shape_only:
@@ -240,7 +243,10 @@
             self.emit(memset_desc(buf.grad_tensor()))
             acc = True
         buf.mark(*view.cols())
-        return view.gptr, int(acc)
+        gp = view.gptr
+        c0, c1 = view.cols()
+        self.gwrites.append([gp, gp + 4 * ((self.B - 1) * view.ld + (c1 - c0)), None])
+        return gp, int(acc)
 
     def live(self, view):
         return view.buf.overlaps(*view.cols())
@@ -328,7 +334,7 @@
     kt_max = kt_sum = 0
     any_live = False
     for sd in segs:
-        if sd.get("Aaux") or sd.get("Baux"):
+        if sd.get("Aaux") or sd.get("Baux") or sd.get("pmask"):
             return None
         if not sd.get("A"):
             continue
@@ -365,7 +371,7 @@
     M, N = segs[0]["M"], segs[0]["N"]
     K = 0
     for sd in segs:
-        if sd.get("Aaux") or sd.get("Baux") or sd.get("ones_col") or (0 < sd.get("Mvalid", M) < M):
+        if sd.get("Aaux") or sd.get("Baux") or sd.get("pmask") or sd.get("ones_col") or (0 < sd.get("Mvalid", M) < M):
             return False
         if sd.get("A") and sd["K"] > 0:
             K += sd["K"]
@@ -385,7 +391,7 @@
         return False
     K = 0
     for sd in segs:
-        if sd.get("Aaux") or sd.get("Baux") or sd.get("ones_col") or (0 < sd.get("Mvalid", M) < M):
+        if sd.get("Aaux") or sd.get("Baux") or sd.get("pmask") or sd.get("ones_col") or (0 < sd.get("Mvalid", M) < M):
             return False
         if sd.get("A") and sd["K"] > 0:
             K += sd["K"]
@@ -432,7 +438,7 @@
         return False
     for q in range(d.nseg):
         s = d.seg[q]
-        if s.Aaux or s.Baux or s.ones_col or (0 < s.Mvalid < s.M):
+        if s.Aaux or s.Baux or s.pmask or s.ones_col or (0 < s.Mvalid < s.M):
             return False
         if s.M < 1024 or s.N < 256 or s.K < 0 or s.K > 16:
             return False
@@ -440,7 +446,7 @@
 
 
 def gemm_kernel_name(d) -> str:
-    segs = [dict(A=d.seg[q].A, Aaux=d.seg[q].Aaux, Baux=d.seg[q].Baux, M=d.seg[q].M, N=d.seg[q].N, K=d.seg[q].K) for q in range(d.nseg)]
+    segs = [dict(A=d.seg[q].A, Aaux=d.seg[q].Aaux or d.seg[q].pmask, Baux=d.seg[q].Baux, M=d.seg[q].M, N=d.seg[q].N, K=d.seg[q].K) for q in range(d.nseg)]
     live = [sd for sd in segs if sd["A"]]
     if d.splitk <= 1 and kslice_eligible(d.amode, d.bmode, d.cmode, [dict(sd, ones_col=d.seg[q].ones_col, Mvalid=d.seg[q].Mvalid, lda=d.seg[q].lda,
                                                                           ldb=d.seg[q].ldb) for q, sd in enumerate(segs)], d.zmode):
@@ -528,7 +534,7 @@
     if amode == L.AM_TOKK and zmode and B >= 1024:
         ok = True
         for sd in segs:
-            if sd["M"] > 80 or sd["N"] > 80 or sd.get("Aaux") or sd.get("Baux"):
+            if sd["M"] > 80 or sd["N"] > 80 or sd.get("Aaux") or sd.get("Baux") or sd.get("pmask"):
                 ok = False
                 break
         if ok:
@@ -807,6 +813,33 @@
     if mode == L.AM_KC:
         return R * ld
     return (R // 16) * ld
+
+
+def relu_mask_at_producer():
+    return _os.environ.get("NASREC_RELU_MASK", "producer") != "consumer"
+
+
+def note_final_producer(ctx, e, q):
+    if ctx.relu_at_producer and ctx.gwrites and ctx.gwrites[-1][0] == e.dseg[q]:
+        ctx.gwrites[-1][2] = (e, q)
+
+
+def _producer_masked(ctx, out: DV, mask_ptr):
+    if not ctx.relu_at_producer or not isinstance(out, DV):
+        return None
+    lo = out.gptr
+    hi = lo + 4 * ((ctx.B - 1) * out.ld + out.width)
+    hits = [w for w in ctx.gwrites if w[0] < hi and lo < w[1]]
+    if len(hits) != 1 or hits[0][2] is None:
+        return None
+    e, q = hits[0][2]
+    if e.dseg[q] != lo or e.ld[q] != out.ld or e.width[q] != out.width or e.tok_stride[q]:
+        return None
+    if e.dseg_masked[q]:
+        return e.dseg_masked[q] if e.dseg_mask[q] == mask_ptr else None
+    e.dseg_mask[q] = mask_ptr
+    e.dseg_masked[q] = ctx.alloc(ctx.B * out.ld).data_ptr()
+    return e.dseg_masked[q]
 
 
 def linear_dense(ctx, segs: List[Seg], Ktot, wname, nout, bias: bool, out: DV, act=L.ACT_NONE, dims=-1, beta=0, ln=None,
@@ -849,14 +882,15 @@
                             mul=mul_list, pre_add=pre_add.ptr if (pre_add is not None and c0 == 0) else None):
             ctx.emit(d)
 
-    def backward_products(dz_ptr, dz_ld, aux_ptr, kdims):
+    def backward_products(dz_ptr, dz_ld, aux_ptr, kdims, pm=0):
         kd = nout if kdims < 0 else min(kdims, nout)
         _emit_z_groups(ctx, L.AM_KC, L.AM_RC, L.CM_PLAIN, _dx_groups(ctx, live, lambda s, gp, acc: dict(
-            A=dz_ptr, Aaux=aux_ptr, B=W + 4 * s.koff, C=gp, M=B, N=s.width, K=kd, lda=dz_ld, ldb=Ktot, ldc=s.view.ld, accumulate=acc)))
+            A=dz_ptr, Aaux=aux_ptr, B=W + 4 * s.koff, C=gp, M=B, N=s.width, K=kd, lda=dz_ld, ldb=Ktot, ldc=s.view.ld, accumulate=acc,
+            pmask=pm)))
         gW = ctx.gparam(wname + ".weight")
         _weight_grad_products(ctx, L.AM_RC, L.AM_RC, L.CM_PLAIN, [(rank, dict(
             A=dz_ptr, Aaux=aux_ptr, B=s.view.ptr + 4 * (a - s.koff), C=gW + 4 * a, M=nout, N=b - a, K=B, lda=dz_ld, ldb=s.view.ld, ldc=Ktot,
-            Mvalid=kd, accumulate=int(rank > 0))) for s, a, b, rank in _cover_pieces(live)],
+            Mvalid=kd, accumulate=int(rank > 0), pmask=pm)) for s, a, b, rank in _cover_pieces(live)],
             rowsum_out=ctx.gparam(wname + ".bias") if (bias and live) else None)
         if bias and not live:
             r = L.RowsumDesc()
@@ -881,7 +915,11 @@
         if not ctx.live(out):
             return
         if act == L.ACT_RELU:
-            backward_products(out.gptr, out.ld, out.ptr, dims)
+            masked = _producer_masked(ctx, out, out.ptr)
+            if masked is not None:
+                backward_products(masked, out.ld, None, dims, 1)
+            else:
+                backward_products(out.gptr, out.ld, out.ptr, dims)
         elif act == L.ACT_SILU:
             dz = ctx.alloc(B * nout)
             a = L.ActBwdDesc()
@@ -1242,6 +1280,7 @@
         e.x, e.dout = x.ptr, out.gptr
         e.dx = xbuf.grad_tensor().data_ptr()
         xbuf.mark()
+        ctx.gwrites.append([e.dx, e.dx + 4 * xbuf.numel, None])
         e.saved = saved.data_ptr() if saved is not None else None
         e.bwd_form = ctx.mha_bwd_form
         for q in range(12):
diff --git a/nasrec_amd/schedule.py b/nasrec_amd/schedule.py
--- a/nasrec_amd/schedule.py
+++ b/nasrec_amd/schedule.py
@@ -213,6 +213,9 @@
                     W.append(a)
                     if d.dseg_accumulate[q]:
                         R.append(a)
+                    if d.dseg_masked[q]:
+                        R.append(Acc(d.dseg_mask[q], d.B, d.width[q], d.ld[q]))
+                        W.append(Acc(d.dseg_masked[q], d.B, d.width[q], d.ld[q]))
         if k == L.OP_FINAL_BWD:
             W.append(_flat(d.dw, (K + 1) * max(d.nsplit, 1)))
             for ptr, n in ((d.dbias, 1), (d.loss, 1), (d.dlogits_out, d.B)):
@@ -492,7 +495,7 @@
     if nprob == 1 and ((d.seg[0].M + 63) // 64) * ((d.seg[0].N + 63) // 64) * S >= SOLO_TILES:
         return False
     from . import plan as P
-    if not getattr(d, "_wl_force", False) and P.kslice_eligible(d.amode, d.bmode, d.cmode, [dict(A=d.seg[q].A, Aaux=d.seg[q].Aaux, Baux=d.seg[q].Baux, ones_col=d.seg[q].ones_col,
+    if not getattr(d, "_wl_force", False) and P.kslice_eligible(d.amode, d.bmode, d.cmode, [dict(A=d.seg[q].A, Aaux=d.seg[q].Aaux, Baux=d.seg[q].Baux, pmask=d.seg[q].pmask, ones_col=d.seg[q].ones_col,
                                                            Mvalid=d.seg[q].Mvalid, M=d.seg[q].M, N=d.seg[q].N, K=d.seg[q].K, lda=d.seg[q].lda,
                                                            ldb=d.seg[q].ldb) for q in range(d.nseg)], d.zmode):
         return False
```

After: 1.149 million (median of 2 runs). No clear change (-0.8%).
